# ghy1228/LDPC_Error_Floor

Hardware: AMD Instinct MI355X
Metric: decoded codewords/sec, wman N576 R3/4, 20 NMS iters (higher is better)
Workload: dtype i32

## Files before the change

include/ldpc_nms.h:

```cpp
#ifndef LDPC_NMS_H
#define LDPC_NMS_H

#include <stdint.h>

#ifdef __cplusplus
extern "C" {
#endif

#define LDPC_NMS_ABI_VERSION 3

typedef struct ldpc_graph ldpc_graph;
typedef struct ldpc_ctx ldpc_ctx;

enum ldpc_status {
    LDPC_OK = 0,
    LDPC_ERR_ARG = -1,
    LDPC_ERR_HIP = -2,
    LDPC_ERR_OOM = -3,
    LDPC_ERR_STATE = -4,
    LDPC_ERR_UNSUPPORTED = -5
};

enum ldpc_decoding_type {
    LDPC_DEC_SP = 0,
    LDPC_DEC_MS = 1,
    LDPC_DEC_QMS = 2,
    LDPC_DEC_MS_NONUDGE = 3
};

enum ldpc_kernel {
    LDPC_KERNEL_AUTO = 0,
    LDPC_KERNEL_FLOOD = 1,
    LDPC_KERNEL_FUSED = 2
};

typedef struct ldpc_decode_params {
    int32_t T;
    int32_t decoding_type;
    int32_t q_bit;
    int32_t target_bits;
    float clip_llr;
    int32_t kernel;
    int32_t outputs_size;
    int32_t reserved;
} ldpc_decode_params;

typedef struct ldpc_decode_outputs {
    float* app_all;
    uint32_t* hard_bits;
    uint32_t* synd_bits;
    int64_t* counters;
    uint8_t* frame_flags;
    uint32_t* iter_wrong;
} ldpc_decode_outputs;

int ldpc_abi_version(void);
const char* ldpc_status_string(int status);

int ldpc_graph_create(const int32_t* proto, int32_t M, int32_t N, int32_t z, int32_t device,
                      ldpc_graph** out);
int ldpc_graph_destroy(ldpc_graph* g);
int ldpc_graph_query(const ldpc_graph* g, int32_t* dims);

int ldpc_weights_set(ldpc_graph* g, int32_t T, const float* alpha, const float* alpha_ucn,
                     const float* beta);

int ldpc_ctx_create(ldpc_graph* g, int64_t B_max, int32_t T_max, ldpc_ctx** out);
int ldpc_ctx_destroy(ldpc_ctx* c);

int ldpc_decode(ldpc_ctx* c, const float* llr_dev, int64_t B, const ldpc_decode_params* p,
                const ldpc_decode_outputs* o, void* stream);

int ldpc_kernel_info(const ldpc_ctx* c, const ldpc_decode_params* p, int64_t* bytes_per_cw,
                     char* name, int32_t name_len);

int ldpc_ctx_last_kernel(const ldpc_ctx* c, char* name, int32_t name_len);

int ldpc_ctx_last_frozen(const ldpc_ctx* c);

int ldpc_ctx_last_afix(const ldpc_ctx* c);

int ldpc_channel_awgn(float* llr_dev, int64_t B, int32_t n_vars, double sigma, uint64_t seed,
                      int64_t offset, int32_t decoding_type, int32_t q_bit, int32_t punct_start,
                      int32_t punct_end, int32_t short_start, int32_t short_end, float clip_llr,
                      void* stream);

typedef struct ldpc_channel_params {
    double sigma;
    uint64_t seed;
    int64_t offset;
    int32_t punct_start, punct_end, short_start, short_end;
    int32_t reserved[4];
} ldpc_channel_params;

int ldpc_decode_awgn(ldpc_ctx* ctx, int64_t B, const ldpc_decode_params* params,
                     const ldpc_channel_params* channel, const ldpc_decode_outputs* outputs,
                     void* stream);

int ldpc_awgn_in_kernel(const ldpc_ctx* ctx, const ldpc_decode_params* params, int32_t has_short,
                        int32_t app);

typedef struct ldpc_es_outputs {
    int32_t size;
    int32_t reserved;
    int64_t* counters;
    uint8_t* frame_flags;
    uint8_t* n_iter;
    int64_t* iter_hist;
} ldpc_es_outputs;

int ldpc_decode_es(ldpc_ctx* ctx, const float* llr_dev, int64_t B, const ldpc_decode_params* params,
                   const ldpc_es_outputs* es_outputs, void* stream);
int ldpc_decode_awgn_es(ldpc_ctx* ctx, int64_t B, const ldpc_decode_params* params,
                        const ldpc_channel_params* channel, const ldpc_es_outputs* es_outputs,
                        void* stream);
int ldpc_es_supported(const ldpc_ctx* ctx, const ldpc_decode_params* params);

typedef struct ldpc_word_outputs {
    int32_t size;
    int32_t reserved;
    uint32_t* hard_last;
    uint8_t* word_flags;
    int64_t* counters;
    uint8_t* frame_flags;
} ldpc_word_outputs;

int ldpc_decode_word(ldpc_ctx* ctx, const float* llr_dev, int64_t B, const ldpc_decode_params* params,
                     const ldpc_word_outputs* word_outputs, void* stream);
int ldpc_word_supported(const ldpc_ctx* ctx, const ldpc_decode_params* params);

typedef struct ldpc_es_word_outputs {
    int32_t size;
    int32_t reserved;
    uint32_t* hard_stop;
    uint8_t* word_flags;
    int64_t* counters;
    uint8_t* frame_flags;
    uint8_t* n_iter;
    int64_t* iter_hist;
    uint64_t reserved1;
} ldpc_es_word_outputs;

int ldpc_decode_es_word(ldpc_ctx* ctx, const float* llr_dev, int64_t B, const ldpc_decode_params* params,
                        const ldpc_es_word_outputs* outputs, void* stream);
int ldpc_decode_awgn_es_word(ldpc_ctx* ctx, int64_t B, const ldpc_decode_params* params,
                             const ldpc_channel_params* channel, const ldpc_es_word_outputs* outputs,
                             void* stream);
int ldpc_es_word_supported(const ldpc_ctx* ctx, const ldpc_decode_params* params);

typedef struct ldpc_event_outputs {
    int32_t size;
    int32_t early_stop;
    int64_t frame_base;
    int64_t cap;
    int64_t* ev_count;
    int64_t* ev_frame;
    int32_t* ev_info;
    uint32_t* ev_word;
    int64_t* counters;
    uint8_t* frame_flags;
    uint8_t* n_iter;
    int64_t* iter_hist;
    uint64_t reserved1;
} ldpc_event_outputs;

int ldpc_decode_events(ldpc_ctx* ctx, const float* llr_dev, int64_t B, const ldpc_decode_params* params,
                       const ldpc_event_outputs* outputs, void* stream);
int ldpc_decode_awgn_events(ldpc_ctx* ctx, int64_t B, const ldpc_decode_params* params,
                            const ldpc_channel_params* channel, const ldpc_event_outputs* outputs,
                            void* stream);
int ldpc_events_supported(const ldpc_ctx* ctx, const ldpc_decode_params* params, int32_t early_stop);

int ldpc_decode_q8(ldpc_ctx* ctx, const int8_t* q8_dev, int64_t B, const ldpc_decode_params* params,
                   const ldpc_decode_outputs* outputs, void* stream);
int ldpc_decode_q8_word(ldpc_ctx* ctx, const int8_t* q8_dev, int64_t B, const ldpc_decode_params* params,
                        const ldpc_word_outputs* word_outputs, void* stream);
int ldpc_q8_supported(const ldpc_ctx* ctx, const ldpc_decode_params* params, int32_t has_short,
                      int32_t word);
int ldpc_channel_awgn_q8(int8_t* q8_dev, int64_t B, int32_t n_vars, double sigma, uint64_t seed,
                         int64_t offset, int32_t q_bit, int32_t punct_start, int32_t punct_end,
                         int32_t short_start, int32_t short_end, void* stream);
int ldpc_llr_to_q8(const float* llr_dev, int64_t n, int32_t q_bit, float clip_llr, int8_t* q8_dev,
                   int64_t* n_invalid_dev, void* stream);

int ldpc_channel_awgn_rows(float* rows_dev, const int64_t* idx_dev, int64_t n, int32_t n_vars,
                           double sigma, uint64_t seed, int64_t offset, int32_t decoding_type,
                           int32_t q_bit, int32_t punct_start, int32_t punct_end,
                           int32_t short_start, int32_t short_end, float clip_llr, void* stream);

int ldpc_collect_frames(const uint8_t* flags_dev, int64_t B, uint32_t mask, uint32_t want,
                        int64_t* idx_dev, int64_t cap, int64_t* count_dev, void* stream);

int ldpc_gather_rows(const float* src_dev, int64_t n_cols, const int64_t* idx_dev, int64_t n,
                     float* dst_dev, void* stream);

#define LDPC_UNCOR_ROW_BOUND(n_cols) (13 + 48 * (int64_t)(n_cols))
int ldpc_format_uncor_rows(const float* rows, int64_t n, int64_t n_cols, char* out, int64_t cap,
                           int64_t* len);

#ifdef __cplusplus
}
#endif
#endif
```

include/ldpc_nms_debug.h:

```cpp
#ifndef LDPC_NMS_DEBUG_H
#define LDPC_NMS_DEBUG_H

#include <stdint.h>

#include "ldpc_nms.h"

#ifdef __cplusplus
extern "C" {
#endif

int ldpc_debug_bs_bounds(const int32_t* proto, int32_t M, int32_t N, int32_t z, int32_t T,
                         int32_t mode, int32_t alpha_uniform, int32_t beta_uniform, float clip,
                         int32_t flags, int32_t* violations, char* msg, int32_t msg_len);

int ldpc_debug_bs_frozen(const int32_t* proto, int32_t M, int32_t N, int32_t z, int32_t T, int32_t mode,
                         int32_t alpha_uniform, int32_t beta_uniform, int32_t ucn, int32_t kind,
                         float clip, int32_t* plan, int32_t* frozen, int32_t n, char* names,
                         int32_t names_len);

int ldpc_debug_alpha_tid(float alpha, int32_t mode, int32_t* out_id, uint8_t* table);

int ldpc_debug_alpha_tids(const int32_t* proto, int32_t M, int32_t N, int32_t z, int32_t T,
                          const float* alpha, const float* alpha_ucn, int32_t* ids);

int ldpc_debug_events_out(ldpc_ctx* ctx, const uint32_t* planes_dev, const uint32_t* bad_dev, int64_t B,
                          int32_t target_bits, const uint8_t* n_iter_dev, int32_t T,
                          const ldpc_event_outputs* outputs, void* stream);

#ifdef __cplusplus
}
#endif

#endif
```

ldpc_error_floor_amd/csrc/ldpc_bs.hip:

```cpp
#include <algorithm>
#include <array>
#include <cmath>
#include <cstdio>
#include <cstdlib>
#include <cstring>
#include <functional>
#include <string>
#include <utility>
#include <vector>

#include "ldpc_bs_host.h"

namespace ldpc {
namespace bs {

__global__ void k_bs_tables(const float* __restrict__ alpha, const float* __restrict__ alpha_ucn,
                            const float* __restrict__ beta, const int32_t* __restrict__ row_ptr,
                            int T, int E, int N, int arows, int ar, int bcols, float step, float inv,
                            int qmax, float cu, uint32_t* alut, uint32_t* blut) {
    const int f = blockIdx.x * blockDim.x + threadIdx.x;
    const int na = T * ar, nbt = T * bcols;
    if (f >= na + nbt) return;
    int g[16];
    uint32_t* out;
// ... 71 lines not shown
        if (i > 0) first += (size_t)((((int64_t)lay[2 * (i - 1)] + h.z - (int64_t)cur) % 32 + 32) % 32);
        int A = ((deg + LPC - 1) / LPC) * h.z;
        while (!ok(A)) ++A;
        const int last_rows = (deg - (LPC - 1) + LPC - 1) / LPC;
        cur = first + (size_t)(LPC - 1) * A + (size_t)std::max(last_rows, 0) * h.z;
        lay[2 * i] = (int32_t)first;
        lay[2 * i + 1] = A;
    }
    *nslot = cur;
    return lay;
}
std::vector<int32_t> slot_layout(const host::GraphTables& h, int LPC, size_t* nslot) {
    return slot_layout_rows(h, std::vector<int>((size_t)h.M, LPC), nslot);
}

bool bs_mode(int mode) { return mode == MODE_Q5 || mode == MODE_QM5 || mode == MODE_Q4 || mode == MODE_Q3; }
float bs_step(int mode) { return mode == MODE_Q5 ? 0.5f : mode == MODE_Q3 ? 2.0f : 1.0f; }
int bs_qmax(int mode) { return mode == MODE_Q4 ? 7 : mode == MODE_Q3 ? 3 : QMAX; }
static float mode_step_bs(int mode) { return bs_step(mode); }

static BsPlan plan_inst(const DevGraph& g, int i, bool ucn, float clip, int min_cdeg, int mode, int T) {
    BsPlan p;
    const BsInst& k = kBsInst[i];
    const host::GraphTables& h = *g.host;
    if (h.max_cdeg > k.D || h.max_vdeg > k.DV || (ucn && !k.UCN)) return p;
    p.inst = i;
    p.ucn = ucn;
    const int nv = g.n_vars, nc = g.n_checks;
    p.cn_lanes = 64 * ((k.LPC * nc + 63) / 64);
    int vch = (nv + 63) / 64;
    const int cch = p.cn_lanes / 64;
    if (k.VPL == 1 && k.CPL == 1) {
        static const int eca = [] { const char* e = getenv("LDPC_BS_COLALIGN"); return e ? atoi(e) : 1; }();
        p.colalign = eca != 0 && colalign_fits(h, std::max(vch, cch));
        if (p.colalign) vch = (32 * h.N + 63) / 64;
    }
    if (k.VPL == 1 && k.CPL == 1) p.nw = std::max(vch, cch);
    else p.nw = std::max((vch + k.VPL - 1) / k.VPL, (cch + k.CPL - 1) / k.CPL);
    if (p.nw > 16) return p;
    if (k.VPL > 1 || k.CPL > 1) {
        p.nw = 16;
        if (vch > k.VPL * p.nw || cch > k.CPL * p.nw) return p;
    }
    const char* eap = getenv("LDPC_BS_AROWS");
    p.arows = ((g.w_alpha_uniform && !ucn) || (g.w_alpha_pair_uniform && !(eap && atoi(eap) == 0))) ? 1 : h.M;
    p.bcols = g.w_beta_uniform ? 1 : h.N;
    p.cn_dmin = (p.cn_lanes == k.LPC * nc) ? min_cdeg : 0;
    if (k.BIG) {
        const float cu = clip / mode_step_bs(mode);
        if (cu > (float)bs_qmax(mode)) p.cu = cu;
    }
    size_t nslot = 0;
    p.lay = slot_layout(h, k.LPC, &nslot);
    size_t o = 0;
    if (k.UCN) {
        p.off_hdz = (uint32_t)(4 * (size_t)nv);
        o = ((size_t)4 * (nv + 1) + 127) & ~(size_t)127;
    }
    p.off_slots = (uint32_t)o;
    p.off_pad = (uint32_t)(o + nslot * SLOT_B);
    p.off_zero = p.off_pad + SLOT_B;
    const size_t slot_end = (size_t)p.off_zero + SLOT_B;
    if (k.PK && slot_end > 65535) return p;
    if (k.UCN && p.off_hdz > 65535) return p;
    o = (slot_end + 15) & ~(size_t)15;
    p.off_red = (uint32_t)o;
    o += 64 + (((size_t)4 * T + 15) & ~(size_t)15) + 4 * FLORW;
    if (k.ES) {
        p.off_esu = (uint32_t)o;
        o += ((size_t)4 * T + 15) & ~(size_t)15;
    }
    p.off_alut = (uint32_t)o;
    o += (size_t)2 * (k.UCN ? 2 : 1) * p.arows * LUT_W * 4;
    p.off_blut = (uint32_t)o;
    o += (size_t)2 * p.bcols * BLUT_W * 4;
    const bool first_buffer = k.ES || i == kBsInstUcn1;
    if (k.PK && k.CPL == 1 && (first_buffer ? (size_t)p.off_alut + (size_t)p.arows * LUT_W * 4 : o) > 65535) return p;
    if (k.CPL == 1) {
        p.off_ch = (uint32_t)o;
        o += (size_t)4 * 64 * p.nw;
    }
    if (k.UCN && k.CPL == 1) {
        const int EPL = (k.D + k.LPC - 1) / k.LPC, HDW = (EPL + 1) / 2;
        p.off_hdl = (uint32_t)o;
        o += (size_t)4 * HDW * 64 * p.nw;
    }
    p.lds = (o + 15) & ~(size_t)15;
    if (p.lds > BS_LDS_MAX) return p;
    p.ok = true;
    return p;
}

BsPlan bs_plan(const DevGraph& g, int mode, bool ucn, bool per_edge_w, float clip, int T, bool es = false) {
    BsPlan p;
    const char* e = getenv("LDPC_BS");
    if (e && atoi(e) == 0) return p;
    const char* el = getenv("LDPC_BS_LPC");
    const int want_lpc = el ? atoi(el) : 0;
    const char* ei = getenv("LDPC_BS_INST");
    const int want_inst = ei ? atoi(ei) : -1;
    if (!bs_mode(mode)) return p;
    if (per_edge_w || !g.host || !g.w_beta_nonneg) return p;
    const host::GraphTables& h = *g.host;
    int min_cdeg = 1 << 30;
    for (int i = 0; i < h.M; ++i) min_cdeg = std::min(min_cdeg, h.row_ptr[i + 1] - h.row_ptr[i]);
    if (min_cdeg < 2) return p;
    for (int i = 0; i < kBsNInst; ++i) {
        if (kBsInst[i].ES != es) continue;
        if (es) {
            BsPlan q = plan_inst(g, i, ucn, clip, min_cdeg, mode, T);
            if (q.ok) return q;
            continue;
        }
        if (want_lpc != 0 && want_lpc != kBsInst[i].LPC) continue;
        if (want_inst >= 0 && want_inst != i) continue;
        if (i == kBsInstUcn1 && !ucn) continue;
        BsPlan q = plan_inst(g, i, ucn, clip, min_cdeg, mode, T);
        if (q.ok) return q;
    }
    return p;
}

typedef std::array<int32_t, kBsFrozenFields> BsGeoFields;
static const char* const bs_frozen_names[kBsFrozenFields] = {
    "inst", "n_vars", "n_checks", "z", "N", "cn_lanes", "cn_dmin", "NT", "nw", "arows", "bcols", "AL", "BL",
    "cstride", "off_slots", "off_pad", "off_zero", "off_red", "off_alut", "off_blut", "off_ch", "lds"};
static BsGeoFields bs_plan_fields(const DevGraph& g, const BsPlan& p) {
    const int ar = (p.inst >= 0 && kBsInst[p.inst].UCN ? 2 : 1) * p.arows;
    return {p.inst, g.n_vars, g.n_checks, g.z, g.N, p.cn_lanes, p.cn_dmin, 64 * p.nw, p.nw, p.arows, p.bcols,
            ar * LUT_W, p.bcols * BLUT_W, g.z * SLOT_B, (int32_t)p.off_slots, (int32_t)p.off_pad,
            (int32_t)p.off_zero, (int32_t)p.off_red, (int32_t)p.off_alut, (int32_t)p.off_blut,
            (int32_t)p.off_ch, (int32_t)p.lds};
}
static BsGeoFields bs_frozen_fields() {
    typedef BsFrozenWman W;
    return {W::inst, W::n_vars, W::n_checks, W::z, W::N, W::cn_lanes, W::cn_dmin, W::NT, W::nw, W::arows,
            W::bcols, W::AL, W::BL, (int32_t)W::cstride, (int32_t)W::off_slots, (int32_t)W::off_pad,
            (int32_t)W::off_zero, (int32_t)W::off_red, (int32_t)W::off_alut, (int32_t)W::off_blut,
            (int32_t)W::off_ch, (int32_t)W::lds};
}
static bool bs_frozen_fit(const DevGraph& g, BsPlan& p, const BsReq& r, bool exports) {
    const char* e = getenv("LDPC_BS_FROZEN");
    if (e && atoi(e) == 0) return false;
    if (!p.ok || p.inst != BsFrozenWman::inst || p.ucn || r.es || r.l8 || exports || r.T > BsFrozenWman::T_CAP) return false;
    BsPlan q = p;
    const uint32_t d = (uint32_t)(((4 * BsFrozenWman::T_CAP + 15) & ~15) - ((4 * r.T + 15) & ~15));
    q.off_alut += d;
    q.off_blut += d;
    q.off_ch += d;
    q.lds += d;
    if (bs_plan_fields(g, q) != bs_frozen_fields()) return false;
    p = q;
    return true;
}

#ifndef BS_DEAL_DEFAULT
#define BS_DEAL_DEFAULT 2
#endif
std::vector<int> deal_chunks(const std::vector<int>& cost, int nw, int cap) {
    const int n = (int)cost.size();
    std::vector<int> order(n), slot((size_t)nw * cap, -1);
    for (int c = 0; c < n; ++c) order[c] = c;
    std::stable_sort(order.begin(), order.end(), [&](int x, int y) { return cost[x] > cost[y]; });
    const char* e = getenv("LDPC_BS_DEAL");
    if (e && atoi(e) == 0) {
        std::vector<int> used(nw, 0), load(4, 0);
        for (int c : order) {
            int best = -1, bw = -1;
            for (int sm = 0; sm < 4; ++sm) {
                int w_s = -1;
                for (int w = sm; w < nw; w += 4)
                    if (used[w] < cap && (w_s < 0 || used[w] < used[w_s])) w_s = w;
                if (w_s >= 0 && (best < 0 || load[sm] < load[best])) { best = sm; bw = w_s; }
            }
            slot[(size_t)bw * cap + used[bw]] = c;
            ++used[bw];
            load[best] += cost[c];
        }
        return slot;
    }
    const int deal_mode = e ? atoi(e) : BS_DEAL_DEFAULT;
    if (deal_mode == 2 && cap == 1 && n <= nw && nw <= 16) {
        int slots[4] = {0, 0, 0, 0};
        for (int w = 0; w < nw; ++w) ++slots[w % 4];
        std::vector<int> cur(n, -1), best(n, -1);
        int load[4] = {0, 0, 0, 0}, used[4] = {0, 0, 0, 0};
        long long best_key = -1;
        std::function<void(int)> rec = [&](int i) {
            const int mx = std::max(std::max(load[0], load[1]), std::max(load[2], load[3]));
            if (best_key >= 0 && (long long)mx * 1000000 > best_key) return;
            if (i == n) {
                const long long key = (long long)mx * 1000000 + (long long)load[0] * load[0] + (long long)load[1] * load[1] +
                                      (long long)load[2] * load[2] + (long long)load[3] * load[3];
                if (best_key < 0 || key < best_key) { best_key = key; best = cur; }
                return;
            }
            for (int sm = 0; sm < 4; ++sm) {
                if (used[sm] >= slots[sm]) continue;
                bool dup = false;
                for (int q = 0; q < sm; ++q)
                    if (used[q] < slots[q] && load[q] == load[sm] && slots[q] - used[q] == slots[sm] - used[sm]) dup = true;
                if (dup) continue;
                load[sm] += cost[order[i]];
                ++used[sm];
                cur[i] = sm;
                rec(i + 1);
                load[sm] -= cost[order[i]];
                --used[sm];
            }
        };
        rec(0);
        int next[4] = {0, 1, 2, 3};
        for (int i = 0; i < n; ++i) {
            const int sm = best[i];
            slot[(size_t)next[sm]] = order[i];
            next[sm] += 4;
        }
        return slot;
    }
    std::vector<std::vector<int>> vch(nw);
    std::vector<int> vload(nw, 0);
    for (int c : order) {
        int best = -1;
        for (int w = 0; w < nw; ++w)
            if ((int)vch[w].size() < cap &&
                (best < 0 || vload[w] < vload[best] || (vload[w] == vload[best] && vch[w].size() < vch[best].size())))
                best = w;
        vch[best].push_back(c);
        vload[best] += cost[c];
    }
    std::vector<int> vorder(nw), sload(4, 0), next(4);
    for (int w = 0; w < nw; ++w) vorder[w] = w;
    std::stable_sort(vorder.begin(), vorder.end(), [&](int x, int y) { return vload[x] > vload[y]; });
    for (int sm = 0; sm < 4; ++sm) next[sm] = sm;
    for (int v : vorder) {
        int sm = -1;
        for (int q = 0; q < 4; ++q)
            if (next[q] < nw && (sm < 0 || sload[q] < sload[sm])) sm = q;
        const int w = next[sm];
        next[sm] += 4;
        sload[sm] += vload[v];
        for (size_t u = 0; u < vch[v].size(); ++u) slot[(size_t)w * cap + u] = vch[v][u];
    }
    return slot;
}

std::vector<int32_t> uniform_lanes(const host::GraphTables& h, int LPC, int cn_lanes) {
    std::vector<int32_t> lanes((size_t)cn_lanes, -1);
    const int nc = h.M * h.z;
    for (int ql = 0; ql < cn_lanes; ++ql)
        if (ql / LPC < nc) lanes[(size_t)ql] = (ql / LPC) | ((ql % LPC) << 16) | (LPC << 20);
    return lanes;
}

std::vector<int> check_chunk_cost_lanes(const host::GraphTables& h, const std::vector<int32_t>& lanes) {
    const int cch = (int)(lanes.size() / 64);
    std::vector<int> cost(cch, 2);
    for (int ch = 0; ch < cch; ++ch) {
        int pos = 0;
        for (int l = 0; l < 64; ++l) {
            const int32_t d = lanes[(size_t)64 * ch + l];
            if (d < 0) continue;
            const int i = (d & 0xFFFF) / h.z, L = (d >> 20) & 15;
            pos = std::max(pos, (h.row_ptr[i + 1] - h.row_ptr[i] + L - 1) / L);
        }
        cost[ch] += pos;
    }
    return cost;
}
std::vector<int> check_chunk_cost(const host::GraphTables& h, int LPC, int cch) {
    return check_chunk_cost_lanes(h, uniform_lanes(h, LPC, 64 * cch));
}

std::vector<int> column_rotation_lanes(const host::GraphTables& h, int EPL, const std::vector<int32_t>& lanes) {
    const int z = h.z, cn_lanes = (int)lanes.size();
    std::vector<int> toff(h.N, 0);
    {
        std::vector<std::vector<std::pair<int, int>>> grp;
        std::vector<std::vector<int>> bycol(h.N);
        for (int h0 = 0; h0 < cn_lanes; h0 += 32)
            for (int m = 0; m < EPL; ++m) {
                std::vector<std::pair<int, int>> gl;
                for (int ql = h0; ql < h0 + 32 && ql < cn_lanes; ++ql) {
                    const int32_t d = lanes[(size_t)ql];
                    if (d < 0) continue;
                    const int cc = d & 0xFFFF, cj = (d >> 16) & 15, LPC = (d >> 20) & 15;
                    const int i = cc / z, hc = cc - i * z, kk = LPC * m + cj;
                    if (kk >= h.row_ptr[i + 1] - h.row_ptr[i]) continue;
                    const int pe = h.row_ptr[i] + kk;
                    gl.emplace_back(h.pe_col[pe], (hc + h.pe_shift[pe]) % z);
                }
                if (gl.empty()) continue;
                for (const auto& x : gl)
                    if (bycol[x.first].empty() || bycol[x.first].back() != (int)grp.size())
                        bycol[x.first].push_back((int)grp.size());
                grp.push_back(std::move(gl));
            }
        auto gcost = [&](const std::vector<std::pair<int, int>>& gl) {
            int cnt[32] = {0}, mx = 0, sq = 0;
            uint32_t seen[32];
            int ns = 0;
            for (const auto& x : gl) {
                const uint32_t t = (uint32_t)(x.first * z + (x.second + toff[x.first]) % z);
                bool dup = false;
                for (int q = 0; q < ns && !dup; ++q) dup = seen[q] == t;
                if (dup) continue;
// ... 191 lines not shown
        for (size_t x = 0; x < cs.size(); ++x) cchunk[x] = cs[x];
    }
    std::vector<uint32_t> chd;
    if (k.UCN) {
        chd.assign((size_t)p.cn_lanes * HDW, 0u);
        for (int ql = 0; ql < p.cn_lanes; ++ql) {
            const int cc = ql / LPC, cj = ql % LPC;
            for (int m = 0; m < EPL; ++m) {
                uint32_t addr = p.off_hdz;
                const int kk = LPC * m + cj;
                if (cc < g.n_checks) {
                    const int i = cc / z, hc = cc - i * z;
                    if (kk < h.row_ptr[i + 1] - h.row_ptr[i]) {
                        const int pe = h.row_ptr[i] + kk;
                        const int v = h.pe_col[pe] * z + (hc + h.pe_shift[pe]) % z;
                        addr = 4 * hd_index(v);
                    }
                }
                chd[(size_t)ql * HDW + (m >> 1)] |= addr << (16 * (m & 1));
            }
        }
    }
    BsHostTables t;
    t.vn.swap(vn);
    t.wdeg.swap(wdeg);
    t.cchunk.swap(cchunk);
    t.chd.swap(chd);
    return t;
}
static int bs_graph_tables(const DevGraph& g, const BsPlan& p, void*& graph, int& inst, hipStream_t s) {
    if (graph && inst != p.inst) {
        (void)hipFree(graph);
        graph = nullptr;
    }
    if (graph) return LDPC_OK;
    BsHostTables t = bs_host_tables(g, p);
    const std::vector<uint32_t>& vn = t.vn;
    const std::vector<int32_t>& wdeg = t.wdeg;
    const std::vector<int32_t>& cchunk = t.cchunk;
    const std::vector<uint32_t>& chd = t.chd;
    const size_t nwords = vn.size() + wdeg.size() + p.lay.size() + cchunk.size() + chd.size();
    void* d = nullptr;
    if (hipMalloc(&d, nwords * 4) != hipSuccess) { (void)hipGetLastError(); return LDPC_ERR_OOM; }
    uint32_t* dp = reinterpret_cast<uint32_t*>(d);
    size_t at = 0;
    bool ok = true;
    auto up = [&](const void* src, size_t n) {
        if (n) ok = ok && hipMemcpyAsync(dp + at, src, n * 4, hipMemcpyHostToDevice, s) == hipSuccess;
        at += n;
    };
    up(vn.data(), vn.size());
    up(wdeg.data(), wdeg.size());
    up(p.lay.data(), p.lay.size());
    up(cchunk.data(), cchunk.size());
    up(chd.data(), chd.size());
    if (!ok || hipStreamSynchronize(s) != hipSuccess) {
        (void)hipFree(d);
        return LDPC_ERR_HIP;
    }
    graph = d;
    inst = p.inst;
    return LDPC_OK;
}

static BsPlan bs_route(const DevGraph& g, const BsReq& r, bool* to_bsc) {
    BsPlan p = bs_plan(g, r.mode, r.ucn, r.per_edge_w, r.clip, r.T, r.es);
    *to_bsc = !p.ok && (!r.es || !bs_plan(g, r.mode, r.ucn, r.per_edge_w, r.clip, r.T).ok);
    return p;
}

bool bs_supported(const DevGraph& g, const BsReq& r) {
    bool to_bsc;
    return bs_route(g, r, &to_bsc).ok || (to_bsc && bsc_supported(g, r));
}

bool bs_q8_ok(const DevGraph& g, const BsReq& r, bool has_short) {
    bool to_bsc;
    const BsPlan p = bs_route(g, r, &to_bsc);
    if (!p.ok) return to_bsc && bsc_q8_ok(g, r, has_short);
    return (!has_short || p.cu > 0.f) && q8_tab_fits(p);
}

bool bs_l8_ok(const DevGraph& g, const BsReq& r, bool has_short) {
    bool to_bsc;
    if (r.es) return false;
    const BsPlan p = bs_route(g, r, &to_bsc);
    if (!p.ok) return to_bsc && bsc_l8_ok(g, r, has_short);
    return bs_l8_inst(p.inst) && (!has_short || (kBsInst[p.inst].BIG && p.cu > 0.f));
}

const char* bs_kernel_name(const DevGraph& g, const BsReq& r) {
    static thread_local char buf[64];
    bool to_bsc;
    const BsPlan p = bs_route(g, r, &to_bsc);
    if (!p.ok) return to_bsc ? bsc_kernel_name(g, r) : "";
    const BsInst& k = kBsInst[p.inst];
    char x[16] = "";
    if (k.VPL > 1 || k.CPL > 1) snprintf(x, sizeof(x), ",x%d/%d", k.VPL, k.CPL);
    snprintf(buf, sizeof(buf), "bsl[p32,w%d,d%d,v%d,l%d%s%s%s]", p.nw, k.D, k.DV, k.LPC, x, p.ucn ? ",ucn" : "",
             r.es ? ",es" : "");
    return buf;
}

static int bs_run(const DevGraph& g, const Bufs& b, FusedWorkspace& ws, const BsPlan& p, const float* llr,
                  const BsReq& r, const BsOut& o, bool frozen, hipStream_t s) {
    ws.bs_frozen = frozen;
    void*& graph = r.es ? ws.bs_es_graph : ws.bs_graph;
    int st = bs_graph_tables(g, p, graph, r.es ? ws.bs_es_graph_inst : ws.bs_graph_inst, s);
    if (st != LDPC_OK) return st;
    const BsInst& k = kBsInst[p.inst];
    const float step = mode_step_bs(r.mode);
    const int ar = (k.UCN ? 2 : 1) * p.arows;
    uint32_t *alut = nullptr, *blut = nullptr;
    st = bs_make_tables(b, g, p.arows, ar, p.bcols, step, bs_qmax(r.mode), p.cu, r.ucn, ws, &alut, &blut, s);
    if (st != LDPC_OK) return st;
    const int DV = k.DV;
    const int VNW = (k.PK ? (DV + 1) / 2 : DV) + 1;
    const uint32_t* gt = reinterpret_cast<const uint32_t*>(graph);
    BsLaunch a{};
    a.n_iter = o.n_iter;
    a.iter_hist = o.iter_hist;
    a.hdw = o.hdw;
    a.word = o.word ? 1 : 0;
    a.frozen = frozen;
    a.llr = r.l8 ? reinterpret_cast<const float*>(r.l8) : llr;
    const int src = r.l8 ? BS_SRC_L8 : b.q8 ? BS_SRC_GEN : BS_SRC_LLR;
    a.gen = bs_gen(b, q8_tab_lds(p));
    a.B = b.B;
    a.n_vars = g.n_vars;
    a.n_checks = g.n_checks;
    a.T = b.T;
    a.target_bits = b.target_bits;
    a.cn_lanes = p.cn_lanes;
    a.cn_dmin = p.cn_dmin;
    a.fold_wave = p.cn_lanes < 64 * p.nw ? (uint32_t)(p.nw - 1) : (p.nw > 1 ? 1u : 0u);
    a.inv = 1.0f / step;
    a.cu = p.cu > 0.f ? p.cu : -1.f;
    a.qmax = bs_qmax(r.mode);
    a.ucn = p.ucn ? 1 : 0;
    a.ucn_iter = g.w_ucn_iter;
    a.beta_id = g.w_beta_id_mask;
    a.row_ptr = g.row_ptr;
    a.z = g.z;
    a.vn_tab = gt;
    const size_t nvt = (size_t)k.VPL * 64 * p.nw * VNW;
    a.vn_wdeg = reinterpret_cast<const int32_t*>(gt + nvt);
    a.row_lay = a.vn_wdeg + 3 * (size_t)k.VPL * p.nw;
    a.cn_chunk = a.row_lay + 2 * (size_t)g.M;
    a.cn_hd = reinterpret_cast<const uint32_t*>(a.cn_chunk + (size_t)p.nw * k.CPL);
    a.alut = alut;
    a.blut = blut;
    a.arows = p.arows;
    a.bcols = p.bcols;
    a.btid = (bs_qmax(r.mode) == QMAX && !getenv("LDPC_BS_NOBFIX")) ? g.beta_tid : nullptr;
    a.btid_n = g.N;
    a.atid = nullptr;
    if (bs_loops(k) && !p.ucn && p.arows == 1 && (r.mode == MODE_Q5 || r.mode == MODE_QM5)) {
        const char* e = getenv("LDPC_BS_AFIX");
        if (e ? atoi(e) != 0 : true) a.atid = g.host->w_alpha_tid_dev;
    }
    ws.bs_afix = a.atid != nullptr;
    a.counters = o.counters;
    a.flags = o.flags;
    a.bad = o.bad;
    a.iter_wrong = r.es ? nullptr : b.iter_wrong;
    a.hdx = o.hdx;
    bs_stagger(k.VPL > 1 || k.CPL > 1, &a.stagger, &a.stagger_n);
    a.off_slots = p.off_slots;
    a.off_pad = p.off_pad;
    a.off_zero = p.off_zero;
    a.off_red = p.off_red;
    a.off_alut = p.off_alut;
    a.off_blut = p.off_blut;
    a.off_hdz = p.off_hdz;
    a.off_hdl = p.off_hdl;
    a.off_ch = p.off_ch;
    if (const char* e = getenv("LDPC_DIAG_ABLATE")) a.ablate = atoi(e);
    const int npacks = (int)((b.B + PACK - 1) / PACK);
    int grid = -1;
    if (const char* e = getenv("LDPC_BS_GRID")) grid = std::max(atoi(e), 0);
    a.ticket = nullptr;
    if (bs_loops(k)) {
        const char* e = getenv("LDPC_BS_TICKETS");
        if (e ? atoi(e) != 0 : true) {
            if (!ws.bs_ticket && hipMalloc(reinterpret_cast<void**>(&ws.bs_ticket), sizeof(uint32_t)) != hipSuccess)
                return LDPC_ERR_OOM;
            a.ticket = ws.bs_ticket;
        }
    }
    static const auto kLaunch = launch_table(std::make_integer_sequence<int, kBsNInst>{});
    static const size_t lds_min = [] { const char* e = getenv("LDPC_BS_LDS_MIN"); return e ? (size_t)atol(e) : 0; }();
    const size_t lds = std::min(std::max(p.lds, lds_min), (size_t)BS_LDS_MAX);
    const uint64_t rkey = (uint64_t)p.inst << 48 | (uint64_t)p.nw << 32 | (uint64_t)lds;
    if (ws.bs_resident_key != rkey) {
        ws.bs_resident_key = rkey;
        std::fill(ws.bs_resident, ws.bs_resident + 7, 0);
    }
#ifdef BS_STAMP
    static unsigned long long* dst = nullptr;
    static size_t dst_words = 0;
    const size_t st_words = BS_WG_BASE + (size_t)BS_WG_REC * npacks;
    if (dst_words < st_words) {
        if (dst && (hipStreamSynchronize(s) != hipSuccess || hipFree(dst) != hipSuccess)) return LDPC_ERR_HIP;
        dst = nullptr;
        dst_words = 0;
        if (hipMalloc(reinterpret_cast<void**>(&dst), st_words * 8) != hipSuccess) return LDPC_ERR_OOM;
        dst_words = st_words;
    }
    if (hipMemsetAsync(dst, 0, st_words * 8, s) != hipSuccess) return LDPC_ERR_HIP;
    a.stamps = dst;
    st = kLaunch[p.inst](a, npacks, p.nw, lds, s, src, grid, ws.bs_resident);
    unsigned long long hst[256];
    if (st != LDPC_OK || hipMemcpyAsync(hst, dst, sizeof(hst), hipMemcpyDeviceToHost, s) != hipSuccess ||
        hipStreamSynchronize(s) != hipSuccess)
        return st != LDPC_OK ? st : LDPC_ERR_HIP;
    fprintf(stderr, "bs_stamp inst %d T %d q8 %d frozen %d: per pack, shader clocks [check, check-barrier, var, var-barrier | "
            "entry, channel, ch-barrier, tables, first-var, check-setup | epilogue]\n", p.inst, b.T, b.q8 != nullptr,
            (int)frozen);
    static const int order[] = {0, 1, 2, 3, 8, 9, 10, 11, 12, 4, 5};
    for (int w = 0; w < p.nw && w < 16; ++w) {
        const double n = (double)(hst[16 * w + 15] ? hst[16 * w + 15] : 1);
        fprintf(stderr, "  wave %2d:", w);
        for (const int i : order) fprintf(stderr, " %8.0f", hst[16 * w + i] / n);
        fprintf(stderr, "  | SIMD %5.3f %5.3f %5.3f %5.3f\n", (hst[16 * w + 13] & 0xFFFFFFFFull) / n,
                (hst[16 * w + 13] >> 32) / n, (hst[16 * w + 14] & 0xFFFFFFFFull) / n, (hst[16 * w + 14] >> 32) / n);
    }
    if (const char* path = getenv("LDPC_BS_WG_DUMP")) {
        std::vector<unsigned long long> rec((size_t)BS_WG_REC * npacks);
        if (hipMemcpy(rec.data(), dst + BS_WG_BASE, rec.size() * 8, hipMemcpyDeviceToHost) != hipSuccess)
            return LDPC_ERR_HIP;
        int nwg = 0;
        for (int w = 0; w < npacks; ++w) nwg += rec[(size_t)BS_WG_REC * w] != 0;
        const int tickets = a.ticket != nullptr && nwg < npacks;
        if (FILE* f = fopen(path, "a")) {
            fprintf(f, "bs_wg_launch inst %d T %d B %lld packs %d q8 %d frozen %d tickets %d\n"
                    "# bs_wg wg packs rt_entry rt_exit clk_entry clk_exit hw_id xcc_id   (rt: 100 MHz ticks, clk: shader clocks)\n",
                    p.inst, b.T, (long long)b.B, npacks, b.q8 != nullptr, (int)frozen, tickets);
            for (int w = 0; w < npacks; ++w) {
                const unsigned long long* r = rec.data() + (size_t)BS_WG_REC * w;
                if (!r[0]) continue;
                fprintf(f, "bs_wg %d %llu %llu %llu %llu %llu %08llx %llu\n", w, r[0], r[1], r[2], r[3], r[4],
                        r[5] & 0xFFFFFFFFull, r[5] >> 32);
            }
            fclose(f);
        }
    }
    return st;
#else
    return kLaunch[p.inst](a, npacks, p.nw, lds, s, src, grid, ws.bs_resident);
#endif
}

int bs_decode(const DevGraph& g, const Bufs& b, FusedWorkspace& ws, const float* llr, const BsReq& r,
              const BsOut& o, hipStream_t s) {
    bool to_bsc;
    BsPlan p = bs_route(g, r, &to_bsc);
    ws.bs_frozen = false;
    ws.bs_afix = false;
    if (!p.ok) return to_bsc ? bsc_decode(g, b, ws, llr, r, o, s) : LDPC_ERR_UNSUPPORTED;
    const bool frozen = bs_frozen_fit(g, p, r, o.hdx != nullptr || o.hdw != nullptr);
    return bs_run(g, b, ws, p, llr, r, o, frozen, s);
}

}

namespace ldpc {
namespace bs {
struct BoundsReport {
    int violations = 0;
    std::string first;
    void fail(const char* what, long long idx, long long lim) {
        if (violations++ == 0) {
            char buf[160];
            snprintf(buf, sizeof(buf), "%s: index %lld outside [0, %lld)", what, idx, lim);
            first = buf;
        }
    }
    void in(const char* what, long long idx, long long lim) {
        if (idx < 0 || idx >= lim) fail(what, idx, lim);
    }
    void lds(const char* what, long long a, long long n, long long lo, long long hi) {
        if (a < lo || a + n > hi) fail(what, a, hi);
    }
    void apart(const char* what, long long a, long long n, long long b, long long m) {
        if (a < b + m && b < a + n) fail(what, a + n, b);
    }
};

static int bs_bounds_check(const DevGraph& g, const BsPlan& p, const BsHostTables& t, int T, int flags,
                           BoundsReport& r) {
    const BsInst& k = kBsInst[p.inst];
    const host::GraphTables& h = *g.host;
    const int LPC = k.LPC, VPL = k.VPL, CPL = k.CPL, DV = k.DV;
    const int EPL = (k.D + LPC - 1) / LPC, HDW = (EPL + 1) / 2, OB = 4 / LPC;
    const int VNA = k.PK ? (DV + 1) / 2 : DV, VNW = VNA + 1;
    const int NT = 64 * p.nw, nwv = p.nw, nv = g.n_vars, z = h.z;
    const bool UCN = k.UCN, ucn = UCN && (p.ucn || k.ES);
    const int AR = UCN ? 2 * p.arows : p.arows;
    const long long AL = (long long)AR * LUT_W, BL = (long long)p.bcols * BLUT_W;
    const long long lds = (long long)p.lds;
    const bool SKIPM = CPL > 1;
    const bool GBL = CPL == 1;
    const bool HDL = UCN && CPL == 1;
    if (getenv("LDPC_BOUNDS_VERBOSE"))
        fprintf(stderr, "bs plan: inst %d nw %d ucn %d lds %lld (slots %u..%u, alut %u, blut %u, ch %u, hdl %u)\n",
                p.inst, p.nw, (int)p.ucn, lds, p.off_slots, p.off_pad, p.off_alut, p.off_blut, p.off_ch, p.off_hdl);
    r.in("lds size", lds, (long long)BS_LDS_MAX + 1);
    if ((long long)t.vn.size() != (long long)VPL * NT * VNW) r.fail("vn_tab size", (long long)t.vn.size(), (long long)VPL * NT * VNW);
    r.lds("RED", p.off_red, 4LL * (16 + ((T + 3) & ~3) + FLORW), 0, k.ES ? p.off_esu : p.off_alut);
    if (k.ES) {
        r.lds("syndrome words", p.off_esu, 4LL * T, p.off_red, p.off_alut);
        r.apart("syndrome words / RED", p.off_esu, 4LL * T, p.off_red, 4LL * (16 + ((T + 3) & ~3) + FLORW));
        if (p.off_esu != p.off_red + 4u * (uint32_t)(16 + ((T + 3) & ~3) + FLORW)) r.fail("syndrome words' offset", p.off_esu, p.off_red);
        if (p.off_alut & 15) r.fail("alpha tables off 16 B", p.off_alut & 15, 1);
    }
    r.lds("ALUT", p.off_alut, 4 * 2 * AL, 0, p.off_blut);
    r.lds("BLUT", p.off_blut, 4 * 2 * BL, 0, lds);
    r.lds("PAD+ZERO", p.off_pad, 2 * SLOT_B, p.off_slots, p.off_red);
    if (UCN) r.lds("HD", 0, 4LL * (nv + 1), 0, p.off_slots);
    if (q8_tab_fits(p)) {
        const long long tb = q8_tab_lds(p);
        const long long tn = (flags & LDPC_BOUNDS_BIG_TABLES) ? (long long)(p.off_pad - p.off_slots) + 4
                                                              : 4LL * AWGN_TAB_W;
        r.lds("channel tables", tb, tn, p.off_slots, p.off_pad);
        if (UCN) r.apart("channel tables / HD", tb, tn, 0, 4LL * (nv + 1));
        r.apart("channel tables / PAD+ZERO", tb, tn, p.off_pad, 2 * SLOT_B);
        r.apart("channel tables / RED", tb, tn, p.off_red, (long long)p.off_alut - p.off_red);
        r.apart("channel tables / ALUT", tb, tn, p.off_alut, 4 * 2 * AL);
        r.apart("channel tables / BLUT", tb, tn, p.off_blut, 4 * 2 * BL);
    }
    for (int u = 0; u < VPL; ++u)
        for (int w = 0; w < nwv; ++w) {
            const long long wi = 3LL * (u * nwv + w);
            r.in("vn_wdeg", wi + 2, (long long)t.wdeg.size());
            if (wi + 2 >= (long long)t.wdeg.size()) continue;
            const int dw = t.wdeg[(size_t)wi], pcol = t.wdeg[(size_t)wi + 2];
            if (pcol >= 0) r.in("btid column", pcol, h.N);
            if (dw >= 0 && T > 1) {
                const long long col = p.bcols == 1 ? 0 : pcol;
                if (col >= 0) r.in("btid", (long long)(T - 1) * h.N + col, (long long)T * h.N);
            }
            for (int l = 0; l < 64; ++l) {
                const long long ti = ((long long)u * NT + 64LL * w + l) * VNW;
                r.in("vn_tab", ti + VNA, (long long)t.vn.size());
                if (ti + VNA >= (long long)t.vn.size()) continue;
                const uint32_t* q = &t.vn[(size_t)ti];
                const int vv = (int)q[VNA];
                const int v = (UCN && vv >= 0) ? (vv & 0xFFFF) : vv;
                if (v >= nv) r.fail("variable", v, nv);
                if (vv >= 0 && UCN) r.in("HD index", (long long)((uint32_t)vv >> 16), nv);
                if (vv >= 0 && p.bcols > 1) r.in("beta table", v / (nv / p.bcols), p.bcols);
                for (int f = 0; f < DV && f < dw; ++f) {
                    const uint32_t a = k.PK ? ((f & 1) ? (q[f >> 1] >> 16) : (q[f >> 1] & 0xFFFFu)) : q[f];
                    if (a != p.off_zero) r.lds("variable slot", a, SLOT_B, p.off_slots, p.off_pad);
                }
            }
        }
    for (int w = 0; w < nwv; ++w)
        for (int c = 0; c < CPL; ++c) {
            r.in("cn_chunk", (long long)w * CPL + c, (long long)t.cchunk.size());
            const int gchunk = CPL == 1 ? w : t.cchunk[(size_t)w * CPL + c];
            const bool active = CPL == 1 ? w * 64 < p.cn_lanes : gchunk >= 0;
            int gm = EPL;
            if (SKIPM) {
                uint32_t any = 0u;
                for (int l = 0; l < 64; ++l) {
                    const int ql = std::max(gchunk, 0) * 64 + l, cc = ql / LPC;
                    const int ci = std::min(cc / z, g.n_checks / z - 1);
                    const int gdeg = cc < g.n_checks ? h.row_ptr[ci + 1] - h.row_ptr[ci] : 0;
                    any |= (1u << ((gdeg + LPC - 1) / LPC)) - 1u;
                }
                gm = __builtin_popcount(any);
                if (active) r.in("real positions - 1 (the min2 switch)", gm - 1, EPL);
            }
            for (int l = 0; l < 64; ++l) {
                const int ql = std::max(gchunk, 0) * 64 + l, cc = ql / LPC, cj = l % LPC;
                const int ci = std::min(cc / z, g.n_checks / z - 1);
                r.in("row_ptr", ci + 1, h.M + 1);
                r.in("row_lay", 2LL * ci + 1, (long long)p.lay.size());
                const int gdeg = cc < g.n_checks ? h.row_ptr[ci + 1] - h.row_ptr[ci] : 0;
                if (UCN) {
                    const bool guard = (flags & LDPC_BOUNDS_PRE_GUARD) ? true : ql < p.cn_lanes;
                    if (ucn && gchunk >= 0 && guard)
                        for (int pp = 0; pp < HDW; ++pp) r.in("cn_hd", (long long)ql * HDW + pp, (long long)t.chd.size());
                }
                if (GBL) r.lds("per-lane words", p.off_ch + 4LL * (64 * w + l), 4, p.off_ch, lds);
                if (HDL)
                    for (int pp = 0; pp < HDW; ++pp) r.lds("HD addresses", p.off_hdl + 4LL * (pp * NT + 64 * w + l), 4, p.off_hdl, lds);
                if (!active) continue;
                const long long gbase = p.off_slots +
                    ((long long)p.lay[2 * ci] + (long long)cj * p.lay[2 * ci + 1] + (cc - ci * z)) * SLOT_B;
                for (int m = 0; m < EPL; ++m) {
                    if (SKIPM && m >= gm) continue;
                    const bool re = LPC * m + LPC - 1 < p.cn_dmin || LPC * m + cj < gdeg;
                    const long long a = re ? gbase + (long long)m * z * SLOT_B : p.off_pad;
                    r.lds("check slot", a, SLOT_B, p.off_slots, p.off_red);
                    if (re && a + SLOT_B > p.off_pad) r.fail("check slot past the slot region", a, p.off_pad);
                    if (ucn && cc < g.n_checks && ql < p.cn_lanes && (size_t)ql * HDW + (m >> 1) < t.chd.size()) {
                        const uint32_t hw = t.chd[(size_t)ql * HDW + (m >> 1)];
                        const uint32_t ha = (m & 1) ? (hw >> 16) : (hw & 0xFFFFu);
                        r.lds("HD read", ha, 4, 0, (long long)p.off_hdz + 4);
                    }
                }
                const long long ctab = p.off_alut + (long long)(p.arows > 1 ? ci : 0) * LUT_W * 4 + (long long)cj * OB * 64;
                const long long last = ctab + 4LL * AL + (UCN ? (long long)p.arows * LUT_W * 4 : 0) + (OB - 1) * 64 + 3 * 16;
                r.lds("alpha table", ctab, 16, p.off_alut, p.off_alut + 4 * 2 * AL);
                if (k.PK && CPL == 1) r.in("packed alpha-table address", ctab, 65536);
                r.lds("alpha table (odd t, alpha')", last, 16, p.off_alut, p.off_alut + 4 * 2 * AL);
            }
        }
    return r.violations;
}
}
}

extern "C" int ldpc_debug_bs_frozen(const int32_t* proto, int32_t M, int32_t N, int32_t z, int32_t T,
                                    int32_t mode, int32_t alpha_uniform, int32_t beta_uniform, int32_t ucn,
                                    int32_t kind, float clip, int32_t* plan, int32_t* frozen, int32_t n,
                                    char* names, int32_t names_len) {
    using namespace ldpc;
    using namespace ldpc::bs;
    if (!proto || T <= 0 || kind < 0 || kind > 2 || n < 0) return LDPC_ERR_ARG;
    host::GraphTables h;
    const int st = host::build_graph(proto, M, N, z, h);
    if (st != LDPC_OK) return st;
    DevGraph g{};
    g.M = h.M; g.N = h.N; g.z = h.z; g.E = h.E;
    g.n_checks = h.M * h.z; g.n_vars = h.N * h.z; g.n_edges = h.E * h.z; g.max_cdeg = h.max_cdeg;
    g.h_row_ptr = h.row_ptr.data();
    g.host = &h;
    g.w_alpha_uniform = alpha_uniform;
    g.w_alpha_pair_uniform = alpha_uniform;
    g.w_beta_uniform = beta_uniform;
    g.w_beta_nonneg = 1;
    const BsReq r{mode, ucn != 0, false, clip, T, kind == 1};
    bool to_bsc;
    BsPlan p = bs_route(g, r, &to_bsc);
    const bool fz = bs_frozen_fit(g, p, r, kind == 2);
    const BsGeoFields pf = bs_plan_fields(g, p), ff = bs_frozen_fields();
    for (int i = 0; i < n && i < kBsFrozenFields; ++i) {
        if (plan) plan[i] = p.ok ? pf[(size_t)i] : -1;
        if (frozen) frozen[i] = ff[(size_t)i];
    }
    if (names && names_len > 0) {
        std::string all;
        for (int i = 0; i < kBsFrozenFields; ++i) all += std::string(i ? "," : "") + bs_frozen_names[i];
        std::strncpy(names, all.c_str(), (size_t)names_len - 1);
        names[names_len - 1] = 0;
    }
    return fz ? 1 : 0;
}

extern "C" int ldpc_debug_bs_bounds(const int32_t* proto, int32_t M, int32_t N, int32_t z, int32_t T,
                                    int32_t mode, int32_t alpha_uniform, int32_t beta_uniform,
                                    float clip, int32_t flags, int32_t* violations, char* msg,
                                    int32_t msg_len) {
    using namespace ldpc;
    using namespace ldpc::bs;
    if (!proto || !violations || T <= 0) return LDPC_ERR_ARG;
    host::GraphTables h;
    const int st = host::build_graph(proto, M, N, z, h);
    if (st != LDPC_OK) return st;
    DevGraph g{};
    g.M = h.M; g.N = h.N; g.z = h.z; g.E = h.E;
    g.n_checks = h.M * h.z; g.n_vars = h.N * h.z; g.n_edges = h.E * h.z; g.max_cdeg = h.max_cdeg;
    g.h_row_ptr = h.row_ptr.data();
    g.host = &h;
    g.w_alpha_uniform = alpha_uniform;
    g.w_alpha_pair_uniform = alpha_uniform;
    g.w_beta_uniform = beta_uniform;
    g.w_beta_nonneg = 1;
    int min_cdeg = 1 << 30;
    for (int i = 0; i < h.M; ++i) min_cdeg = std::min(min_cdeg, h.row_ptr[i + 1] - h.row_ptr[i]);
    int checked = 0;
    *violations = 0;
    std::string first;
    for (int i = 0; i < kBsNInst; ++i)
        for (int u = 0; u < 2; ++u) {
            if (kBsInst[i].ES && !(flags & LDPC_BOUNDS_ES)) continue;
            if (i == kBsInstUcn1 && (!(flags & LDPC_BOUNDS_UCN1) || u == 0)) continue;
            const BsPlan p = plan_inst(g, i, u != 0, clip, min_cdeg, mode, T);
            if (!p.ok) continue;
            const BsHostTables t = bs_host_tables(g, p);
            BoundsReport r;
            bs_bounds_check(g, p, t, T, flags, r);
            ++checked;
            if (r.violations && first.empty()) {
                char buf[64];
                snprintf(buf, sizeof(buf), "instance %d%s: ", i, u ? " ucn" : "");
                first = std::string(buf) + r.first;
            }
            *violations += r.violations;
        }
    for (int b1 = 0; b1 < 2; ++b1) {
        if (b1 && !beta_uniform) continue;
        g.w_beta_one = b1;
        BoundsReport r;
        const int n = bsc_debug_bounds(g, mode, clip, T, flags, r.violations, r.first);
        if (n <= 0) continue;
        ++checked;
        if (r.violations && first.empty()) first = std::string(b1 ? "bsc beta=1: " : "bsc: ") + r.first;
        *violations += r.violations;
    }
    g.w_beta_one = 1;
    if ((flags & LDPC_BOUNDS_ES_BSC) && beta_uniform && !bs_plan(g, mode, false, false, clip, T).ok) {
        BoundsReport r;
        if (bsc_debug_bounds(g, mode, clip, T, flags, r.violations, r.first, true) > 0) {
            ++checked;
            if (r.violations && first.empty()) first = std::string("bsc early stop: ") + r.first;
            *violations += r.violations;
        }
    }
    if (msg && msg_len > 0) {
        std::strncpy(msg, first.c_str(), (size_t)msg_len - 1);
        msg[msg_len - 1] = 0;
    }
    return checked;
}
```

ldpc_error_floor_amd/csrc/ldpc_bs_kernel.h:

```cpp
#pragma once
#include <type_traits>
#include <cstdint>

#include "ldpc_beta_tabs.h"
#include "ldpc_fused.h"
#include "ldpc_fused5_kernel.h"
#include "ldpc_bitplane.h"
#include "ldpc_bs_frozen.h"

namespace ldpc {
namespace bs {

constexpr int PACK = 32;
constexpr int SLOT_W = 5;
constexpr int SLOT_B = SLOT_W * 4;
constexpr int LUT_W = 64;
constexpr int BLUT_W = LUT_W + 4;
constexpr int QMAX = 15;
constexpr size_t BS_LDS_MAX = 160 * 1024;

struct BsInst { int D, DV, LPC, VPL, CPL; bool UCN, BIG, PK; int WPE; bool ES = false; };
constexpr BsInst kBsInst[] = {
    {15, 6, 4, 1, 1, false, false, true, 8},
    {16, 8, 4, 1, 1, false, false, true, 8},
// ... 280 lines not shown
    a = grp_and<LPC>(a);
    m2[3] = a;
#pragma unroll
    for (int m = 0; m < K; ++m) c2[m] = B3(T_NANDEQ, cand[m], X[m][3], a);
#pragma unroll
    for (int i = 2; i >= 0; --i) {
        a = X[0][i] | ~c2[0];
#pragma unroll
        for (int m = 1; m < K; ++m) a = B3(T_ANDORN, a, X[m][i], c2[m]);
        a = grp_and<LPC>(a);
        m2[i] = a;
        if (i > 0) {
#pragma unroll
            for (int m = 0; m < K; ++m) c2[m] = B3(T_ANDEQ, c2[m], X[m][i], a);
        }
    }
#pragma unroll
    for (int i = 0; i < 4; ++i) m2[i] = mux(two, m1[i], m2[i]);
}

#ifdef BS_DIAG
#define ABL(bit) (a.ablate & (bit))
#else
#define ABL(bit) 0
#endif
#ifdef BS_MARK
#define PH(name, k) asm volatile(";@ph " name ".%0" ::"i"(k))
#define PH4(name, k, x) asm volatile(";@ph " name ".%4" : "+v"(x[0]), "+v"(x[1]), "+v"(x[2]), "+v"(x[3]) : "i"(k))
#define PH8(name, k, x, y)                                                                        \
    asm volatile(";@ph " name ".%8" : "+v"(x[0]), "+v"(x[1]), "+v"(x[2]), "+v"(x[3]), "+v"(y[0]),  \
                 "+v"(y[1]), "+v"(y[2]), "+v"(y[3]) : "i"(k))
#define PH9(name, k, x, y, z)                                                                     \
    asm volatile(";@ph " name ".%9" : "+v"(x[0]), "+v"(x[1]), "+v"(x[2]), "+v"(x[3]), "+v"(y[0]),  \
                 "+v"(y[1]), "+v"(y[2]), "+v"(y[3]), "+v"(z) : "i"(k))
#else
#define PH(name, k) ((void)0)
#define PH4(name, k, x) ((void)0)
#define PH8(name, k, x, y) ((void)0)
#define PH9(name, k, x, y, z) ((void)0)
#endif
__device__ __forceinline__ void t8x8(uint32_t& lo, uint32_t& hi) {
    uint32_t t;
    t = B3((TA ^ TB) & TC, lo, lo >> 7, 0x00AA00AAu);
    lo = B3(T_XOR3, lo, t, t << 7);
    t = B3((TA ^ TB) & TC, hi, hi >> 7, 0x00AA00AAu);
    hi = B3(T_XOR3, hi, t, t << 7);
    t = B3((TA ^ TB) & TC, lo, lo >> 14, 0x0000CCCCu);
    lo = B3(T_XOR3, lo, t, t << 14);
    t = B3((TA ^ TB) & TC, hi, hi >> 14, 0x0000CCCCu);
    hi = B3(T_XOR3, hi, t, t << 14);
    t = B3((TA ^ TB) & TC, lo, hi << 4, 0xF0F0F0F0u);
    lo ^= t;
    hi ^= t >> 4;
}
template <bool BIG>
__device__ __forceinline__ void pack_bytes(const uint32_t (&D)[8], uint32_t valid, uint32_t& cs,
                                           uint32_t (&cm)[4], uint32_t& bg) {
    uint32_t lo[4], hi[4];
#pragma unroll
    for (int g = 0; g < 4; ++g) {
        lo[g] = D[2 * g];
        hi[g] = D[2 * g + 1];
        t8x8(lo[g], hi[g]);
    }
    const uint32_t a = __builtin_amdgcn_perm(lo[1], lo[0], 0x06020400u), b = __builtin_amdgcn_perm(lo[1], lo[0], 0x07030501u);
    const uint32_t c = __builtin_amdgcn_perm(lo[3], lo[2], 0x06020400u), d = __builtin_amdgcn_perm(lo[3], lo[2], 0x07030501u);
    const uint32_t L0 = __builtin_amdgcn_perm(c, a, 0x05040100u) & valid, L2 = __builtin_amdgcn_perm(c, a, 0x07060302u) & valid;
    const uint32_t L1 = __builtin_amdgcn_perm(d, b, 0x05040100u) & valid, L3 = __builtin_amdgcn_perm(d, b, 0x07060302u) & valid;
    const uint32_t e = __builtin_amdgcn_perm(hi[1], hi[0], 0x05010400u), f = __builtin_amdgcn_perm(hi[3], hi[2], 0x05010400u);
    const uint32_t n = ~__builtin_amdgcn_perm(f, e, 0x05040100u) & valid;
    bg = BIG ? (__builtin_amdgcn_perm(f, e, 0x07060302u) & valid) : 0u;
    cs = n;
    cm[0] = L0;
    cm[1] = B3(T_XAND, L1, n, L0);
    cm[2] = B3(T_XAND, L2, n, L0 | L1);
    cm[3] = B3(T_XAND, L3, n, L0 | L1 | L2);
}
template <bool BIG>
__device__ __forceinline__ int pack_channel(const float (&xv)[PACK], float inv, int qmax, float cu,
                                            uint32_t valid, uint32_t& cs, uint32_t (&cm)[4], uint32_t& bg) {
    const float qf = (float)qmax;
    uint32_t D[8];
    int off = 0;
#pragma unroll
    for (int k = 0; k < 8; ++k) D[k] = 0u;
#pragma unroll
    for (int r = 0; r < PACK; ++r) {
        const float x = xv[r] * inv;
        const float q = __builtin_amdgcn_fmed3f(rintf(x), -qf, qf);
        const bool big = BIG && fabsf(x) == cu;
        off |= (q != x && !big) ? 1 : 0;
        D[r >> 2] = __builtin_amdgcn_cvt_pk_u8_f32(q + (big ? 48.f : 16.f), r & 3, D[r >> 2]);
    }
    pack_bytes<BIG>(D, valid, cs, cm, bg);
    return off;
}
typedef unsigned int v2u_g __attribute__((ext_vector_type(2)));
typedef __attribute__((address_space(3))) const v2u_g LdsU2;
__device__ __forceinline__ void gen_bytes(const BsGen& g, int64_t pk, int v, int qmax, uint32_t (&D)[8]) {
    const int bit = v + 1;
    if (g.ss > 0 && bit >= g.ss && bit <= g.se) {
#pragma unroll
        for (int i = 0; i < 8; ++i) D[i] = (uint32_t)(48 - qmax) * 0x01010101u;
        return;
    }
    if (g.ps > 0 && bit >= g.ps && bit <= g.pe) {
#pragma unroll
        for (int i = 0; i < 8; ++i) D[i] = 0x10101010u;
        return;
    }
    LdsU2* bucket = reinterpret_cast<LdsU2*>((uintptr_t)g.lds);
    const LdsW* thi = reinterpret_cast<const LdsW*>((uintptr_t)(g.lds + 8u * (1u << AWGN_KB)));
    const LdsW* tlo = thi + AWGN_NB_MAX;
    const uint64_t g0 = (uint64_t)g.offset + (uint64_t)pk * 32u;
    const int sh = (int)(g.offset & 3);
    const uint32_t boff = (uint32_t)(16 + g.kmin);
    auto word = [&](const int (&l)[4]) __attribute__((always_inline)) -> uint32_t {
        return ((uint32_t)l[0] + boff) | ((uint32_t)l[1] + boff) << 8 | ((uint32_t)l[2] + boff) << 16 |
               ((uint32_t)l[3] + boff) << 24;
    };
#pragma unroll
    for (int i = 0; i < 8; ++i) {
        const uint64_t gq = (g0 + 4u * (uint32_t)i) >> 2;
        int la[4];
        awgn_levels4b(g, bucket, thi, tlo, (uint32_t)v, gq, la);
        uint32_t w = word(la);
        if (sh) {
            int lb[4];
            awgn_levels4b(g, bucket, thi, tlo, (uint32_t)v, gq + 1, lb);
            w = __builtin_amdgcn_alignbyte(word(lb), w, (uint32_t)sh);
        }
        D[i] = w;
    }
}
__device__ __forceinline__ void gen_tables(const BsGen& g, int tid, int NT) {
    copy_async(g.lds, g.tab, AWGN_TAB_W, __builtin_amdgcn_readfirstlane(tid >> 6), NT);
}

constexpr double STAGGER_US = 60.0;
constexpr int FLORW = 32;
constexpr bool bs_loops(const BsInst& k) { return k.VPL == 1 && k.CPL == 1 && !k.UCN; }
#if defined(BS_INST) && BS_INST <= 2
#define BS_LOOP_TU 1
#else
#define BS_LOOP_TU 0
#endif
template <class K>
struct BsArgsAf : K {
    const int32_t* atid;
};
template <class K>
using BsKernArgs = std::conditional_t<BS_LOOP_TU != 0, BsArgsAf<K>, K>;
constexpr int BS_RED_NEXT = 8;
#define BS_PACK_SETUP(pk)                                                                          \
    const int64_t b0 = (int64_t)(pk) * PACK;                                                       \
    const int nvalid = (int)min<int64_t>(PACK, a.B - b0);                                          \
    const uint32_t valid = (nvalid >= 32) ? 0xFFFFFFFFu : ((1u << nvalid) - 1u);                   \
    uint32_t* RED = reinterpret_cast<uint32_t*>(smem + (FZ ? W::off_red : a.off_red));             \
    const int flor = 16 + ((a.T + 3) & ~3);                                                        \
    const int AR = UCN ? 2 * (FZ ? W::arows : a.arows) : (FZ ? W::arows : a.arows);                \
    const int AL = AR * LUT_W, BL = (FZ ? W::bcols : a.bcols) * BLUT_W;                            \
    uint32_t* ALUT = reinterpret_cast<uint32_t*>(smem + (FZ ? W::off_alut : a.off_alut));          \
    uint32_t* BLUT = reinterpret_cast<uint32_t*>(smem + (FZ ? W::off_blut : a.off_blut));          \
    const bool ucn = UCN && a.ucn;                                                                 \
    auto ucn_on = [&](int t) __attribute__((always_inline)) -> bool {                              \
        return ucn && (t >= 64 || ((a.ucn_iter >> t) & 1));                                        \
    };

template <int D, int DV, int LPC, int VPL, int CPL, bool UCN, bool BIG, bool PK, int WPE, bool XP, int LB, bool Q8,
          bool ES = false, bool EW = false, bool FZ = false, bool L8 = false>
__global__ void __launch_bounds__(LB) __attribute__((amdgpu_waves_per_eu(WPE)))
k_bs(BsKernArgs<std::conditional_t<ES, std::conditional_t<EW, BsArgsEw, BsArgsEs>, std::conditional_t<XP, BsArgsXp, BsArgs>>> a) {
    static_assert(LPC == 2 || LPC == 4, "lanes per check");
    using KArgs = std::conditional_t<ES, std::conditional_t<EW, BsArgsEw, BsArgsEs>, std::conditional_t<XP, BsArgsXp, BsArgs>>;
    static_assert(!ES || (UCN && VPL == 1 && CPL == 1 && !XP), "early stop: one-chunk UCN-compiled instances");
    static_assert(!EW || ES, "the stop-iteration word: early-stop builds");
    static_assert(!L8 || (!Q8 && !ES && !FZ), "int8 LLRs: the decode and export builds");
    static_assert(!FZ || (BS_LOOP_TU && !UCN && !XP && !ES && VPL == 1 && CPL == 1 && D == 15 && DV == 6 && LPC == 4),
                  "frozen geometry: the wman pack-loop builds");
    using W = BsFrozenWman;
    static_assert(W::cstride == W::z * SLOT_B && W::AL == W::arows * LUT_W && W::BL == W::bcols * BLUT_W &&
                  W::NT == 64 * W::nw && W::off_zero == W::off_pad + SLOT_B, "BsFrozenWman is consistent");
    constexpr int SB = (DV * QMAX + QMAX <= 127) ? 8 : 9;
    constexpr int EPL = (D + LPC - 1) / LPC;
    constexpr bool SKIPM = CPL > 1;
    constexpr int OB = 4 / LPC;
    constexpr int VNA = PK ? (DV + 1) / 2 : DV;
    constexpr int VNW = VNA + 1;
    constexpr int HDW = (EPL + 1) / 2;
    constexpr bool PKG = PK && CPL == 1;
    constexpr bool ONE = VPL == 1 && CPL == 1;
    constexpr int PRIO = ONE ? (DV >= 6 ? 4 : 2) : 0;
    constexpr int PROPRIO = PRIO == 4 ? 3 : 0;
    constexpr bool T0A = ONE;
    constexpr bool EBR = T0A;
    constexpr int SBSET = ONE ? 3 : 2;
    constexpr int KEEP0 = ONE ? 3 : (UCN ? 4 : 7);
    constexpr int KEEP = DV <= 4 ? DV : (KEEP0 < DV ? KEEP0 : DV - 1);
    constexpr bool BKPF = !XP && VPL > 1;
    constexpr bool AFX = BS_LOOP_TU != 0;
    static_assert(!AFX || (ONE && !UCN), "fixed-set check tables: the one-chunk instances without UCN");
    extern __shared__ __attribute__((aligned(16))) unsigned char smem[];
    if ((uint32_t)(uintptr_t)smem != 0u) __builtin_trap();
#ifdef BS_STAMP
    uint64_t sacc[13] = {};
    uint64_t sts = __builtin_amdgcn_s_memtime();
    if (a.stamps && threadIdx.x == 0) {
        unsigned long long* rec = a.stamps + BS_WG_BASE + (size_t)BS_WG_REC * blockIdx.x;
        rec[1] = __builtin_amdgcn_s_memrealtime();
        rec[3] = sts;
    }
#define BS_ST(i)                                                                                   \
    do {                                                                                           \
        const uint64_t tn_ = __builtin_amdgcn_s_memtime();                                         \
        sacc[i] += tn_ - sts;                                                                      \
        sts = tn_;                                                                                 \
    } while (0)
#else
#define BS_ST(i) ((void)0)
#endif
    const int tid = threadIdx.x;
    const int NT = FZ ? W::NT : (int)blockDim.x;
    const int lane = tid & 63;
    const int wave = __builtin_amdgcn_readfirstlane(tid >> 6);
    const int nwv = NT >> 6;
    const int nv = (FZ ? W::n_vars : a.n_vars);
#if !BS_LOOP_TU
    BS_PACK_SETUP(blockIdx.x)
#endif

    if (PROPRIO > 0) __builtin_amdgcn_s_setprio(PROPRIO);
    uint32_t va[VPL][VNA];
    int vv[VPL], dw[VPL], dwmin[VPL], pcol[VPL];
    uint32_t tab_b[VPL];
#pragma unroll
    for (int u = 0; u < VPL; ++u) {
        const uint32_t* vt = a.vn_tab + ((size_t)u * NT + tid) * VNW;
#pragma unroll
        for (int p = 0; p < VNA; ++p) va[u][p] = vt[p];
        vv[u] = (int)vt[VNA];
        dw[u] = __builtin_amdgcn_readfirstlane(a.vn_wdeg[3 * (u * nwv + wave)]);
        dwmin[u] = __builtin_amdgcn_readfirstlane(a.vn_wdeg[3 * (u * nwv + wave) + 1]);
        pcol[u] = __builtin_amdgcn_readfirstlane(a.vn_wdeg[3 * (u * nwv + wave) + 2]);
        tab_b[u] = ((FZ ? W::bcols : a.bcols) > 1 && vv[u] >= 0) ? (uint32_t)(((UCN ? (vv[u] & 0xFFFF) : vv[u]) / (nv / (FZ ? W::bcols : a.bcols))) * BLUT_W * 4) : 0u;
    }
    constexpr int FOLDB = BS_LOOP_TU ? 0x100 : 0;
    int cn_dmin = (FZ ? W::cn_dmin : a.cn_dmin) | ((FOLDB && (uint32_t)wave == a.fold_wave) ? FOLDB : 0);

    if (a.stagger > 0 && (int)blockIdx.x < a.stagger_n) {
        const int n = (int)(((uint32_t)blockIdx.x * 97u % (uint32_t)a.stagger_n) * (uint32_t)a.stagger /
                            (uint32_t)a.stagger_n);
        for (int i = 0; i < n; ++i) __builtin_amdgcn_s_sleep(8);
    }
#if BS_LOOP_TU
    auto lane_now = [&]() __attribute__((always_inline)) -> int {
        uint32_t all = ~0u;
        asm volatile("" : "+s"(all));
        return (int)__builtin_amdgcn_mbcnt_hi(all, __builtin_amdgcn_mbcnt_lo(all, 0u));
    };
    unsigned pack = blockIdx.x;
#ifdef BS_STAMP
    unsigned long long npk = 0ull;
#endif
    do {
    if (pack != blockIdx.x) {
        __syncthreads();
        if (PROPRIO > 0) __builtin_amdgcn_s_setprio(PROPRIO);
    }
    typedef __attribute__((address_space(4))) const BsArgs PackArgs;
    PackArgs* kap = (PackArgs*)__builtin_amdgcn_kernarg_segment_ptr();
    asm volatile("" : "+s"(kap));
    PackArgs& a = *kap;
    const int tid = wave * 64 + lane_now(), lane = tid & 63;
    BS_PACK_SETUP(pack)
    [[maybe_unused]] const int pack_tbits = FZ ? a.target_bits : 0;
#define BS_TBITS (FZ ? pack_tbits : a.target_bits)
#define BS_PK pack
#define BS_NEXT_PACK continue
#define BS_LANE_IS0 (lane_now() == 0)
#else
#define BS_TBITS a.target_bits
#define BS_PK blockIdx.x
#define BS_NEXT_PACK return
#define BS_LANE_IS0 (lane == 0)
#endif
    if (tid < SLOT_W) {
        reinterpret_cast<uint32_t*>(smem + (FZ ? W::off_pad : a.off_pad))[tid] = 0xFFFFFFFFu;
        reinterpret_cast<uint32_t*>(smem + (FZ ? W::off_zero : a.off_zero))[tid] = 0u;
    }
    if (UCN && tid == 0) lds_put(a.off_hdz, 0u);
    if (tid < 8) RED[tid] = (tid == 1) ? 0xFFFFFFFFu : 0u;
#ifdef BS_STAMP
    if (tid == 0) {
        uint32_t hw0;
        asm volatile("s_getreg_b32 %0, hwreg(HW_REG_HW_ID)" : "=s"(hw0));
        RED[12] = (hw0 >> 4) & 3u;
    }
#endif
    if (tid < FLORW) RED[flor + tid] = 0u;
    [[maybe_unused]] uint32_t es_done = ~valid;
    if constexpr (ES) {
        for (int w = tid; w < a.T; w += NT) RED[flor + FLORW + w] = 0u;
    }
    [[maybe_unused]] uint32_t es_hd = 0u;
#if BS_LOOP_TU
    BsGen gen{};
    if constexpr (Q8) {
        gen.tab = a.gen.tab;
        gen.k0 = a.gen.k0;
        gen.k1 = a.gen.k1;
        gen.offset = a.gen.offset;
        gen.nb = a.gen.nb;
        gen.kmin = a.gen.kmin;
        gen.ps = a.gen.ps;
        gen.pe = a.gen.pe;
        gen.ss = a.gen.ss;
        gen.se = a.gen.se;
        gen.lds = a.gen.lds;
    }
#define BS_GEN gen
#else
#define BS_GEN a.gen
#endif
#if BS_LOOP_TU
    unsigned next_pack = pack + gridDim.x;
    auto take_ticket = [&]() __attribute__((always_inline)) {
        typedef __attribute__((address_space(1))) uint32_t GlobalW;
        GlobalW* tk = (GlobalW*)(uintptr_t)a.cn_hd;
        if (tid == 0 && tk)
            next_pack = gridDim.x + __hip_atomic_fetch_add(tk, 1u, __ATOMIC_RELAXED, __HIP_MEMORY_SCOPE_AGENT);
    };
    if constexpr (Q8) take_ticket();
#endif
    if constexpr (Q8) gen_tables(BS_GEN, tid, NT);
    if (Q8 || !EBR) __syncthreads();
#if BS_LOOP_TU
    if constexpr (Q8) {
        if (tid == 0) RED[BS_RED_NEXT] = next_pack;
    }
#endif
    BS_ST(8);
    uint32_t cs[VPL], cm[VPL][4], bg[VPL];
    int off = 0;
    if (T0A) {
        copy_async((FZ ? W::off_alut : a.off_alut), a.alut, AL, wave, NT);
        copy_async((FZ ? W::off_blut : a.off_blut), a.blut, BL, wave, NT);
    }
    const __amdgpu_buffer_rsrc_t llr_rs = __builtin_amdgcn_make_buffer_rsrc(
        (void*)(a.llr + b0 * nv), 0, nvalid * nv * 4, 0x00020000);
    auto llr_at = [&](int r, int v) __attribute__((always_inline)) -> float {
        return __builtin_bit_cast(float, __builtin_amdgcn_raw_buffer_load_b32(llr_rs, 4 * v, 4 * r * nv, 0));
    };
    auto var_of = [&](int u) __attribute__((always_inline)) -> int {
        return (UCN && vv[u] >= 0) ? (vv[u] & 0xFFFF) : vv[u];
    };
    float xv[VPL][PACK];
#if BS_LOOP_TU
#pragma unroll
    for (int r = 0; r < PACK; ++r) xv[0][r] = 0.f;
#endif
    if constexpr (Q8) {
#pragma unroll
        for (int u = 0; u < VPL; ++u) {
            cs[u] = 0u;
            bg[u] = 0u;
#pragma unroll
            for (int p = 0; p < 4; ++p) cm[u][p] = 0u;
            const int v = var_of(u);
            if (v >= 0 && !ABL(32)) {
                uint32_t Dq[8];
                gen_bytes(BS_GEN, BS_PK, v, a.qmax, Dq);
                pack_bytes<BIG>(Dq, valid, cs[u], cm[u], bg[u]);
            }
        }
    } else if constexpr (L8) {
#if BS_LOOP_TU
        take_ticket();
#endif
        const __amdgpu_buffer_rsrc_t l8_rs = __builtin_amdgcn_make_buffer_rsrc(
            (void*)(reinterpret_cast<const uint8_t*>(a.llr) + b0 * nv), 0, nvalid * nv, 0x00020000);
        auto l8_load = [&](uint32_t (&Dw)[8], int v) __attribute__((always_inline)) {
            uint32_t by[PACK];
#pragma unroll
            for (int r = 0; r < PACK; ++r)
                by[r] = (uint32_t)__builtin_amdgcn_raw_buffer_load_b8(l8_rs, v, min(r, nvalid - 1) * nv, 0);
#pragma unroll
            for (int i = 0; i < 8; ++i)
                Dw[i] = by[4 * i] | by[4 * i + 1] << 8 | by[4 * i + 2] << 16 | by[4 * i + 3] << 24;
        };
        uint32_t Dw[VPL][8];
#pragma unroll
        for (int i = 0; i < 8; ++i) Dw[0][i] = 0u;
        if (var_of(0) >= 0 && !ABL(32)) l8_load(Dw[0], var_of(0));
        if (EBR) {
            asm volatile("" ::: "memory");
            __builtin_amdgcn_s_waitcnt(0xC07F);
            __builtin_amdgcn_s_barrier();
            asm volatile("" ::: "memory");
        }
        const bool l8_big = BIG && a.cu > 0.f;
        uint32_t l8_bad = 0u;
#pragma unroll
        for (int u = 0; u < VPL; ++u) {
            cs[u] = 0u;
            bg[u] = 0u;
#pragma unroll
            for (int p = 0; p < 4; ++p) cm[u][p] = 0u;
            const int v = var_of(u);
            const int u1 = u + 1 < VPL ? u + 1 : u;
            const int vn = (u + 1 < VPL && !ABL(32)) ? var_of(u1) : -1;
            if (v >= 0 && !ABL(32)) {
                uint32_t Dk[8];
#pragma unroll
                for (int i = 0; i < 8; ++i) {
                    uint32_t iv;
                    Dk[i] = l8_bytes(Dw[u][i], a.qmax, l8_big, iv);
                    l8_bad |= l8_invalid(iv, valid >> (4 * i));
                }
                pack_bytes<BIG>(Dk, valid, cs[u], cm[u], bg[u]);
            }
            if (vn >= 0) l8_load(Dw[u1], vn);
        }
        off = l8_bad != 0u;
#if BS_LOOP_TU
        if (tid == 0) RED[BS_RED_NEXT] = next_pack;
#endif
    } else {
#if BS_LOOP_TU
    take_ticket();
#endif
    if (var_of(0) >= 0 && !ABL(32)) {
#pragma unroll
        for (int r = 0; r < PACK; ++r) xv[0][r] = llr_at(r, var_of(0));
    }
    if (EBR) {
        asm volatile("" ::: "memory");
        __builtin_amdgcn_s_waitcnt(0xC07F);
        __builtin_amdgcn_s_barrier();
        asm volatile("" ::: "memory");
    }
#pragma unroll
    for (int u = 0; u < VPL; ++u) {
        cs[u] = 0u;
        bg[u] = 0u;
#pragma unroll
        for (int p = 0; p < 4; ++p) cm[u][p] = 0u;
        const int v = var_of(u);
        const int u1 = u + 1 < VPL ? u + 1 : u;
        const int vn = (u + 1 < VPL && !ABL(32)) ? var_of(u1) : -1;
        if (v >= 0 && !ABL(32))
            off |= pack_channel<BIG>(xv[u], a.inv, a.qmax, a.cu, valid, cs[u], cm[u], bg[u]);
        if (vn >= 0) {
#pragma unroll
            for (int r = 0; r < PACK; ++r) xv[u1][r] = llr_at(r, vn);
        }
    }
#if BS_LOOP_TU
    if (tid == 0) RED[BS_RED_NEXT] = next_pack;
#endif
    }
    if (off) atomicOr(&RED[7], 1u);
    BS_ST(9);
    __syncthreads();
    BS_ST(10);
    if (RED[7]) {
        if constexpr (ES) {
            if (tid < nvalid) {
                if (a.flags) a.flags[b0 + tid] = 0x80;
                if (kern_args<KArgs>().n_iter) kern_args<KArgs>().n_iter[b0 + tid] = 0;
            }
        }
        if constexpr (L8) {
            if (tid < nvalid && a.flags) a.flags[b0 + tid] = 0x80;
        }
        if (tid == 0) a.bad[BS_PK] = 1u;
        BS_NEXT_PACK;
    }
    if (tid == 0) a.bad[BS_PK] = 0u;
    if (!T0A) {
        for (int w = tid; w < AL; w += NT) ALUT[w] = a.alut[w];
        for (int w = tid; w < BL; w += NT) BLUT[w] = a.blut[w];
        __syncthreads();
    }
    BS_ST(11);

    int bkp[VPL];
#pragma unroll
    for (int u = 0; u < VPL; ++u) bkp[u] = -1;
    auto beta_lw = [&](const int u, const uint32_t bslice, const int tb, const uint32_t (&cmu)[4],
                       uint32_t (&lw)[4], const bool use_bk) __attribute__((always_inline)) {
        int bk = -1;
        if constexpr (!XP) {
            if (use_bk && a.btid) {
                const int col = ((FZ ? W::bcols : a.bcols) == 1) ? 0 : pcol[u];
                if (BKPF) bk = __builtin_amdgcn_readfirstlane(bkp[u]);
                else if (col >= 0)
                    bk = __builtin_amdgcn_readfirstlane((int)((const ConstW*)a.btid)[(size_t)tb * (FZ ? W::btid_n : a.btid_n) + col]);
            }
        }
        if (ABL(2) || (tb < 64 && ((a.beta_id >> tb) & 1))) {
            PH("vn_beta_id", u);
#pragma unroll
            for (int i = 0; i < 4; ++i) lw[i] = cmu[i];
        } else if (bk >= 0 && bk < kNBetaTab) {
            PH("vn_beta_fix", u);
            beta_asm(lw, cmu, bk);
            if constexpr (BIG) {
                if ((FZ ? W::bcols : a.bcols) == 1) {
                    const ConstW* tg = (const ConstW*)(a.blut) + (size_t)tb * BLUT_W;
#pragma unroll
                    for (int i = 0; i < 4; ++i) lw[i] = mux(bg[u], tg[LUT_W + i], lw[i]);
                } else {
                    const v4u gb = lds_q(bslice + tab_b[u] + LUT_W * 4);
                    lw[0] = mux(bg[u], gb.x, lw[0]);
                    lw[1] = mux(bg[u], gb.y, lw[1]);
                    lw[2] = mux(bg[u], gb.z, lw[2]);
                    lw[3] = mux(bg[u], gb.w, lw[3]);
                }
            }
        } else if ((FZ ? W::bcols : a.bcols) == 1) {
            PH("vn_beta_sg", u);
            const ConstW* tg = (const ConstW*)(a.blut) + (size_t)tb * BLUT_W;
            lut_s(lw, cmu, tg);
            if constexpr (BIG) {
#pragma unroll
                for (int i = 0; i < 4; ++i) lw[i] = mux(bg[u], tg[LUT_W + i], lw[i]);
            }
        } else {
            PH("vn_beta_lds", u);
            const uint32_t btab = bslice + tab_b[u];
            const uint32_t cmi[1][4] = {{cmu[0], cmu[1], cmu[2], cmu[3]}};
            uint32_t lo[1][4];
            lut<1>(lo, cmi, btab);
#pragma unroll
            for (int i = 0; i < 4; ++i) lw[i] = lo[0][i];
            if constexpr (BIG) {
                const v4u gb = lds_q(btab + LUT_W * 4);
                lw[0] = mux(bg[u], gb.x, lw[0]);
                lw[1] = mux(bg[u], gb.y, lw[1]);
                lw[2] = mux(bg[u], gb.z, lw[2]);
                lw[3] = mux(bg[u], gb.w, lw[3]);
            }
        }
    };
    auto vn_phase = [&](const bool first, const bool last, const uint32_t bslice, const int tb)
                        __attribute__((always_inline)) {
        (void)tid;
        uint32_t wr = 0u, apos = 0u, nb = 0u;
#pragma unroll
        for (int u = 0; u < VPL; ++u) {
            if (VPL > 1 && dw[u] < 0) continue;
            PH("vn_setup", (last ? 100 : 0) + u);
#pragma unroll
            for (int p = 0; p < VNA; ++p) asm volatile("" : "+v"(va[u][p]));
            auto vaddr = [&](int f) __attribute__((always_inline)) -> uint32_t {
                if constexpr (PK) return (f & 1) ? (va[u][f >> 1] >> 16) : (va[u][f >> 1] & 0xFFFFu);
                else return va[u][f];
            };
            const int v = (UCN && vv[u] >= 0) ? (vv[u] & 0xFFFF) : vv[u];
            const uint32_t hda = UCN ? 4u * ((uint32_t)vv[u] >> 16) : 0u;
            const uint32_t cmu[4] = {cm[u][0], cm[u][1], cm[u][2], cm[u][3]};
            const bool counted = v >= 0 && v < BS_TBITS;
            uint32_t lw[1][4];
            PH("vn_beta", (last ? 100 : 0) + u);
            if (!last) beta_lw(u, bslice, tb, cmu, lw[0], !first);
            const int dwu = dw[u];
            auto vbody = [&](auto sbc) __attribute__((always_inline)) {
                constexpr int SB = decltype(sbc)::value;
                uint32_t mn[KEEP > 0 ? KEEP : 1], mb[KEEP > 0 ? KEEP : 1][4];
                uint32_t S[SB];
#pragma unroll
                for (int i = 0; i < SB; ++i) S[i] = 0u;
                if (!first) {
#pragma unroll
                    for (int f = 0; f < DV; ++f) {
                        if (f < dwu) {
                            PH("vn_sum", 1000 * (SB - 6) + (last ? 100 : 0) + 10 * u + f);
                            uint32_t M[4], n, b[4];
                            read_slot(n, M, vaddr(f));
#pragma unroll
                            for (int i = 0; i < 4; ++i) b[i] = M[i] ^ n;
                            if (f == 0) set_b<SB>(S, b, n);
                            else add_b<SB>(S, b, n);
                            if (f < KEEP) {
                                mn[f < KEEP ? f : 0] = n;
#pragma unroll
                                for (int i = 0; i < 4; ++i) mb[f < KEEP ? f : 0][i] = b[i];
                            }
                        }
                    }
                    if constexpr (SB == 8) PH8("vn_app", 1000 * (SB - 6) + (last ? 100 : 0) + u, S, (S + 4));
                    else PH("vn_app", 1000 * (SB - 6) + (last ? 100 : 0) + u);
                    uint32_t hd, nz = 0u;
                    const uint32_t c_s = cs[u];
                    if (last) {
                        uint32_t A[SB];
#pragma unroll
                        for (int i = 0; i < SB; ++i) A[i] = S[i];
                        const uint32_t cb[4] = {cmu[0] ^ c_s, cmu[1] ^ c_s, cmu[2] ^ c_s, cmu[3] ^ c_s};
                        add_b<SB>(A, cb, c_s);
                        hd = ~A[SB - 1];
#pragma unroll
                        for (int i = 0; i < SB; ++i) nz |= A[i];
                    } else {
                        uint32_t c = c_s;
#pragma unroll
                        for (int i = 0; i < SB - 1; ++i) c = B3(T_MAJ, S[i], i < 4 ? (cmu[i] ^ c_s) : c_s, c);
                        hd = B3(T_XNOR3, S[SB - 1], c_s, c);
                    }
                    if (UCN && !last && v >= 0 && (ES || ucn_on(tb))) lds_put(hda, hd);
                    hd &= valid;
                    if constexpr (XP) {
                        const bool word = kern_args<KArgs>().word != 0;
                        const size_t row = word ? (size_t)BS_PK : (size_t)(tb - 1) * (size_t)((a.B + 31) >> 5) + BS_PK;
                        if (v >= 0 && (last || !word)) a.hdx[row * nv + v] = hd;
                    }
                    if (ABL(8)) hd = 0u;
                    if (counted) {
                        wr |= hd;
                        if (last) {
                            apos |= hd & nz;
                            if constexpr (ES) nb += (uint32_t)__popc(hd & ~es_done);
                            else
                            nb += (uint32_t)__popc(hd);
                        }
                    }
                    if constexpr (EW) {
                        if (last) es_hd |= hd & ~es_done;
                    }
                }
                if (last) return;
                if constexpr (SB == 8) PH8("vn_tv", 1000 * (SB - 6) + (last ? 100 : 0) + u, S, (S + 4));
                else PH("vn_tv", 1000 * (SB - 6) + (last ? 100 : 0) + u);
                uint32_t lb[4];
#pragma unroll
                for (int i = 0; i < 4; ++i) lb[i] = lw[0][i] ^ cs[u];
                add_b<SB>(S, lb, cs[u]);
                uint32_t Tv[6];
                clamp6<SB>(Tv, S);
                const int dwm = dwmin[u];
                if (first) {
                    if (UCN && v >= 0 && ucn_on(0)) lds_put(hda, ~Tv[5]);
                    uint32_t x[7], X[4];
#pragma unroll
                    for (int i = 0; i < 7; ++i) x[i] = Tv[i < 6 ? i : 5];
                    abs_sat(X, x);
#pragma unroll
                    for (int f = 0; f < DV; ++f)
                        if (f < dwu && (f < dwm || vaddr(f) != (FZ ? W::off_zero : a.off_zero))) write_slot(vaddr(f), x[6], X);
                } else {
#pragma unroll
                    for (int f = 0; f < DV; ++f) {
                        if (f < dwu) {
                            if (ABL(4)) continue;
                            PH("vn_vc", 1000 * (SB - 6) + (last ? 100 : 0) + 10 * u + f);
                            uint32_t x[7], X[4], n, b[4];
                            if (f < KEEP) {
                                n = mn[f < KEEP ? f : 0];
#pragma unroll
                                for (int i = 0; i < 4; ++i) b[i] = mb[f < KEEP ? f : 0][i];
                            } else {
                                uint32_t M[4];
                                read_slot(n, M, vaddr(f));
#pragma unroll
                                for (int i = 0; i < 4; ++i) b[i] = M[i] ^ n;
                            }
                            sub_tv(x, Tv, b, n);
                            abs_sat(X, x);
                            if (f < dwm || vaddr(f) != (FZ ? W::off_zero : a.off_zero)) write_slot(vaddr(f), x[6], X);
                        }
                    }
                }
            };
            if constexpr (SB >= 8) {
                if ((SBSET & 1) && dwu * QMAX + QMAX <= 63) vbody(std::integral_constant<int, 7>{});
                else if ((SBSET & 2) && SB == 9 && dwu * QMAX + QMAX <= 127) vbody(std::integral_constant<int, (SB == 9 ? 8 : SB)>{});
                else vbody(std::integral_constant<int, SB>{});
            } else {
                vbody(std::integral_constant<int, SB>{});
            }
        }
        if (!first && !last) {
            PH("vn_flags", 0);
            if (!ABL(8)) {
                const uint32_t la = __builtin_amdgcn_mbcnt_hi(~0u, __builtin_amdgcn_mbcnt_lo(~0u, 0u)) & 31u;
                __hip_atomic_fetch_or(RED + flor + la, wr, __ATOMIC_RELAXED, __HIP_MEMORY_SCOPE_WORKGROUP);
            }
        } else if (!first) {
            PH("vn_flags", last ? 100 : 0);
            if (!ABL(8)) wr = wave_or(wr);
            if (last) {
                apos = wave_or(apos);
                nb = wave_add(nb);
            }
            if (BS_LANE_IS0) {
                if (wr) atomicOr(&RED[0], wr);
                if (last) {
                    if (apos) atomicOr(&RED[2], apos);
                    if (nb) atomicAdd(&RED[3], nb);
                }
            }
        }
    };

    vn_phase(true, false, (FZ ? W::off_blut : a.off_blut), 0);
    BS_ST(12);
    const int cj = lane % LPC;
    int gchunk[CPL], gdeg[CPL], gm[CPL];
    uint32_t gbase[CPL], gtab[CPL], ghd[CPL][UCN ? HDW : 1];
#pragma unroll
    for (int c = 0; c < CPL; ++c) {
        gchunk[c] = (CPL == 1) ? wave : __builtin_amdgcn_readfirstlane(a.cn_chunk[wave * CPL + c]);
        const int ql = max(gchunk[c], 0) * 64 + lane;
        const int cc = ql / LPC;
        const int ci = min(cc / (FZ ? W::z : a.z), (FZ ? W::n_checks : a.n_checks) / (FZ ? W::z : a.z) - 1);
        gdeg[c] = (cc < (FZ ? W::n_checks : a.n_checks)) ? a.row_ptr[ci + 1] - a.row_ptr[ci] : 0;
        gm[c] = SKIPM ? (int)__popc(wave_or((1u << ((gdeg[c] + LPC - 1) / LPC)) - 1u)) : EPL;
        gbase[c] = (FZ ? W::off_slots : a.off_slots) + (uint32_t)((a.row_lay[2 * ci] + cj * a.row_lay[2 * ci + 1] + (cc - ci * (FZ ? W::z : a.z))) * SLOT_B);
        gtab[c] = (FZ ? W::off_alut : a.off_alut) + (uint32_t)(((FZ ? W::arows : a.arows) > 1 ? ci : 0) * LUT_W * 4) + (uint32_t)(cj * OB * 64);
        if constexpr (PKG) gbase[c] |= gtab[c] << 16;
        if constexpr (UCN) {
#pragma unroll
            for (int p = 0; p < HDW; ++p) ghd[c][p] = ((ES || ucn) && gchunk[c] >= 0 && ql < (FZ ? W::cn_lanes : a.cn_lanes)) ? a.cn_hd[(size_t)ql * HDW + p] : 0u;
        }
    }
    constexpr bool RPW = CPL > 1;
    constexpr int RB = EPL;
    static_assert(CPL * RB <= 32, "real-position word");
    static_assert(!SKIPM || EPL <= 8, "BS_MIN2_CASE covers 1..8");
    uint32_t rpk = 0u;
#pragma unroll
    for (int c = 0; c < CPL; ++c)
#pragma unroll
        for (int m = 0; m < EPL; ++m)
            if (RPW && (LPC * m + LPC - 1 < cn_dmin || LPC * m + cj < gdeg[c])) rpk |= 1u << (RB * c + m);
    const uint32_t cstride = (uint32_t)((FZ ? W::z : a.z) * SLOT_B);
    const uint32_t tabu = (uint32_t)((FZ ? W::arows : a.arows) * LUT_W * 4);
    constexpr bool GBL = CPL == 1;
    if constexpr (GBL) lds_put((FZ ? W::off_ch : a.off_ch) + 4u * (uint32_t)tid, gbase[0]);
    constexpr bool HDL = UCN && CPL == 1;
    if constexpr (HDL) {
#pragma unroll
        for (int p = 0; p < HDW; ++p) lds_put(a.off_hdl + 4u * (uint32_t)(p * NT + tid), ghd[0][p]);
    }
    __syncthreads();

    BS_ST(4);
    for (int t = 0; t < (ABL(16) ? 0 : a.T); ++t) {
        PH("top", 0);
        if (!ONE && wave == 0 && t > 0) {
            const uint32_t ln = __builtin_amdgcn_mbcnt_hi(~0u, __builtin_amdgcn_mbcnt_lo(~0u, 0u));
            uint32_t x = ln < 32u ? RED[flor + ln] : 0u;
            if (ln < 32u) RED[flor + ln] = 0u;
            const uint32_t w0 = wave_or(x);
            RED[16 + t - 1] = w0;
            RED[1] &= w0;
        }
        const int nx = (t + 1) & 1;
        int ak = 0;
        bool afx = false;
        if constexpr (AFX) {
            typedef __attribute__((address_space(4))) const BsArgsAf<KArgs> ConstAf;
            ConstAf* kq = (ConstAf*)__builtin_amdgcn_kernarg_segment_ptr();
            asm volatile("" : "+s"(kq));
            const ConstW* at = (const ConstW*)kq->atid;
            afx = at != nullptr;
            if (afx) ak = (int)at[t];
        }
#pragma unroll
        for (int u = 0; u < VPL; ++u) asm volatile("" : "+s"(dw[u]), "+s"(dwmin[u]));
        if (!RPW) asm volatile("" : "+s"(cn_dmin));
        const int cdm = FZ ? W::cn_dmin : FOLDB ? (cn_dmin & (FOLDB - 1)) : cn_dmin;
        if (RPW) {
#pragma unroll
            for (int u = 0; u < VPL; ++u) asm volatile("" : "+v"(vv[u]));
        }
        if (t + 1 < a.T) {
            int cw = wave, al = AL, bl = BL, bcl = (FZ ? W::bcols : a.bcols);
            if (!FZ && !(Q8 && VPL == 1 && CPL == 1 && !UCN))
                asm volatile("" : "+s"(cw), "+s"(al), "+s"(bl), "+s"(bcl));
            const uint32_t* alut_p = a.alut;
            const uint32_t* blut_p = a.blut;
            uint32_t off_al = (FZ ? W::off_alut : a.off_alut), off_bl = (FZ ? W::off_blut : a.off_blut);
            if constexpr (VPL == 1 && CPL == 1 && !(Q8 && !UCN)) {
                typedef __attribute__((address_space(4))) const BsArgs ConstArgs;
                ConstArgs* ka = (ConstArgs*)__builtin_amdgcn_kernarg_segment_ptr();
                asm volatile("" : "+s"(ka));
                alut_p = ka->alut;
                blut_p = ka->blut;
                if constexpr (!FZ) {
                    off_al = ka->off_alut;
                    off_bl = ka->off_blut;
                }
            }
            if (!(AFX && afx))
                copy_async(off_al + 4u * (uint32_t)(nx * al), alut_p + (size_t)(t + 1) * al, al, cw, NT);
            if (bcl > 1)
                copy_async(off_bl + 4u * (uint32_t)(nx * bl), blut_p + (size_t)(t + 1) * bl, bl, cw, NT);
        }
        if constexpr (BKPF) {
            if (t + 1 < a.T && a.btid) {
#pragma unroll
                for (int u = 0; u < VPL; ++u) {
                    const int col = ((FZ ? W::bcols : a.bcols) == 1) ? 0 : pcol[u];
                    bkp[u] = col >= 0 ? a.btid[(size_t)(t + 1) * (FZ ? W::btid_n : a.btid_n) + col] : -1;
                }
            }
        }
        if (PRIO == 2) __builtin_amdgcn_s_setprio(1);
        if (PRIO == 4) __builtin_amdgcn_s_setprio(2);
#pragma unroll
        for (int c = 0; c < CPL; ++c) {
            const bool active = (CPL == 1) ? (FZ && W::cn_lanes >= W::NT) || wave * 64 < (FZ ? W::cn_lanes : a.cn_lanes) : (gchunk[c] >= 0);
            if (!active || ABL(1)) continue;
            PH("ck_addr", c);
            uint32_t cbase;
            if constexpr (GBL) {
                uint32_t all = ~0u;
                asm volatile("" : "+s"(all));
                const uint32_t ln = __builtin_amdgcn_mbcnt_hi(all, __builtin_amdgcn_mbcnt_lo(all, 0u));
                cbase = lds_w((FZ ? W::off_ch : a.off_ch) + ((uint32_t)wave << 8) + 4u * ln);
            } else {
                cbase = gbase[c];
                asm volatile("" : "+v"(cbase));
            }
            uint32_t ctab = PKG ? (cbase >> 16) : gtab[c];
            if constexpr (PKG) cbase &= 0xFFFFu;
            int gmc = gm[c];
            asm volatile("" : "+s"(gmc));
            uint32_t rp = rpk;
            if (RPW) asm volatile("" : "+v"(rp));
            const int cdeg = gdeg[c];
            auto real = [&](int m) __attribute__((always_inline)) -> bool {
                if constexpr (RPW) return ((rp >> (RB * c + m)) & 1u) != 0u;
                else return LPC * m + LPC - 1 < cdm || LPC * m + cj < cdeg;
            };
            auto caddr = [&](int m) __attribute__((always_inline)) -> uint32_t {
                return real(m) ? cbase + m * cstride : (FZ ? W::off_pad : a.off_pad);
            };
            uint32_t Xs[EPL][4], ns[EPL];
            PH("ck_read", c);
#pragma unroll
            for (int m = 0; m < EPL; ++m) read_slot(ns[m], Xs[m], caddr(m));
            uint32_t syn = 0u;
            PH("ck_syn", c);
            const bool ucn_t = ucn_on(t);
            if constexpr (UCN) {
                if (ucn_t || (ES && t > 0)) {
                    uint32_t hwv[HDW];
                    if constexpr (HDL) {
                        uint32_t all = ~0u;
                        asm volatile("" : "+s"(all));
                        const uint32_t ln = __builtin_amdgcn_mbcnt_hi(all, __builtin_amdgcn_mbcnt_lo(all, 0u));
#pragma unroll
                        for (int p = 0; p < HDW; ++p)
                            hwv[p] = lds_w(a.off_hdl + 4u * (uint32_t)(p * NT) + ((uint32_t)wave << 8) + 4u * ln);
                    } else {
#pragma unroll
                        for (int p = 0; p < HDW; ++p) {
                            asm volatile("" : "+v"(ghd[c][p]));
                            hwv[p] = ghd[c][p];
                        }
                    }
#pragma unroll
                    for (int m = 0; m < EPL; ++m) {
                        if (SKIPM && m >= gmc) continue;
                        const uint32_t hw = hwv[m >> 1];
                        syn ^= lds_w((m & 1) ? (hw >> 16) : (hw & 0xFFFFu));
                    }
                    syn ^= qperm<QP_X1>(syn);
                    if (LPC == 4) syn ^= qperm<QP_X2>(syn);
                    if constexpr (ES) {
                        if (t > 0) {
                            const uint32_t wu = wave_or(syn);
                            if (wu && BS_LANE_IS0)
                                __hip_atomic_fetch_or(RED + flor + FLORW + (t - 1), wu,
                                                      __ATOMIC_RELAXED, __HIP_MEMORY_SCOPE_WORKGROUP);
                        }
                    }
                }
            }
            PH4("ck_min", c, Xs[EPL - 1]);
            uint32_t m1[4] = {Xs[0][0], Xs[0][1], Xs[0][2], Xs[0][3]}, m2[4] = {~0u, ~0u, ~0u, ~0u};
            uint32_t par = ns[0];
            uint32_t cand[EPL];
#pragma unroll
            for (int m = 1; m < EPL; ++m) par ^= ns[m];
            if constexpr (SKIPM) {
                switch (gmc) {
#define BS_MIN2_CASE(k)                                                                            \
    case k:                                                                                        \
        if constexpr (k <= EPL) {                                                                  \
            PH("ck_mink", 16 * c + k);                                                             \
            min2_bits<k, LPC>(m1, m2, cand, Xs);                                                   \
            _Pragma("unroll") for (int m = k; m < EPL; ++m) cand[m] = 0u;                          \
        } else {                                                                                   \
            __builtin_unreachable();                                                               \
        }                                                                                          \
        break;
                    BS_MIN2_CASE(1) BS_MIN2_CASE(2) BS_MIN2_CASE(3) BS_MIN2_CASE(4) BS_MIN2_CASE(5)
                    BS_MIN2_CASE(6) BS_MIN2_CASE(7) BS_MIN2_CASE(8)
#undef BS_MIN2_CASE
                    default:
                        __builtin_unreachable();
                }
            } else {
                min2_bits<EPL, LPC>(m1, m2, cand, Xs);
            }
            PH9("ck_merge", c, m1, m2, par);
            par ^= qperm<QP_X1>(par);
            if (LPC == 4) par ^= qperm<QP_X2>(par);
            uint32_t q1[4], q2[4];
            PH9("ck_tab", c, m1, m2, par);
            if (AFX && afx) {
                beta_asm(q1, m1, ak);
                beta_asm(q2, m2, ak);
            } else {
                const uint32_t mm[2][4] = {{m1[0], m1[1], m1[2], m1[3]}, {m2[0], m2[1], m2[2], m2[3]}};
                const uint32_t tab = ctab + (uint32_t)((t & 1) * AL * 4);
                uint32_t qb[OB][2];
                bool any_unsat = false;
                if constexpr (UCN) any_unsat = ucn_t && (CPL == 1 || __builtin_amdgcn_ballot_w64(syn != 0u) != 0ull);
#pragma unroll
                for (int b = 0; b < OB; ++b) {
                    uint32_t o[2];
                    lut_bit<2>(o, mm, tab + (uint32_t)(b * 64));
                    if constexpr (UCN) {
                        if (any_unsat) {
                            uint32_t ou[2];
                            lut_bit<2>(ou, mm, tab + tabu + (uint32_t)(b * 64));
                            o[0] = mux(syn, ou[0], o[0]);
                            o[1] = mux(syn, ou[1], o[1]);
                        }
                    }
                    qb[b][0] = o[0];
                    qb[b][1] = o[1];
                }
                if (LPC == 4) {
                    q1[0] = qperm<0x00>(qb[0][0]); q1[1] = qperm<0x55>(qb[0][0]);
                    q1[2] = qperm<0xAA>(qb[0][0]); q1[3] = qperm<0xFF>(qb[0][0]);
                    q2[0] = qperm<0x00>(qb[0][1]); q2[1] = qperm<0x55>(qb[0][1]);
                    q2[2] = qperm<0xAA>(qb[0][1]); q2[3] = qperm<0xFF>(qb[0][1]);
                } else {
                    q1[0] = qperm<0xA0>(qb[0][0]); q1[1] = qperm<0xA0>(qb[OB - 1][0]);
                    q1[2] = qperm<0xF5>(qb[0][0]); q1[3] = qperm<0xF5>(qb[OB - 1][0]);
                    q2[0] = qperm<0xA0>(qb[0][1]); q2[1] = qperm<0xA0>(qb[OB - 1][1]);
                    q2[2] = qperm<0xF5>(qb[0][1]); q2[3] = qperm<0xF5>(qb[OB - 1][1]);
                }
            }
#pragma unroll
            for (int m = 0; m < EPL; ++m) {
                if (m == 0) PH8("ck_pass2", 16 * c, q1, q2);
                if (real(m)) {
                    if (m > 0) PH("ck_pass2", 16 * c + m);
                    uint32_t Mg[4];
#pragma unroll
                    for (int i = 0; i < 4; ++i) Mg[i] = mux(cand[m], q2[i], q1[i]);
                    write_slot(cbase + m * cstride, par ^ ns[m], Mg);
                }
            }
        }
        if constexpr (ONE) {
            const bool folds = FOLDB ? (cn_dmin & FOLDB) != 0 : (uint32_t)wave == a.fold_wave;
            if (folds && t > 0) {
                const uint32_t ln = __builtin_amdgcn_mbcnt_hi(~0u, __builtin_amdgcn_mbcnt_lo(~0u, 0u));
                uint32_t x = ln < 32u ? RED[flor + ln] : 0u;
                if (ln < 32u) RED[flor + ln] = 0u;
                const uint32_t w0 = wave_or(x);
                RED[16 + t - 1] = w0;
                RED[1] &= w0;
            }
        }
        BS_ST(0);
        __syncthreads();
        BS_ST(1);
        if constexpr (ES) {
            if (t > 0) {
                const uint32_t un = (uint32_t)__builtin_amdgcn_readfirstlane((int)RED[flor + FLORW + t - 1]);
                const uint32_t nn = ~un & ~es_done;
                es_done |= nn;
                if (nn) {
                    const int v = vv[0] >= 0 ? (vv[0] & 0xFFFF) : -1;
                    uint32_t nb = 0u;
                    if constexpr (EW) {
                        if (v >= 0) {
                            const uint32_t h = lds_w(4u * ((uint32_t)vv[0] >> 16)) & nn;
                            es_hd |= h;
                            if (v < a.target_bits) nb = (uint32_t)__popc(h);
                        }
                    } else
                    if (v >= 0 && v < a.target_bits)
                        nb = (uint32_t)__popc(lds_w(4u * ((uint32_t)vv[0] >> 16)) & nn);
                    nb = wave_add(nb);
                    if (nb && BS_LANE_IS0) atomicAdd(&RED[3], nb);
                }
                if (es_done == 0xFFFFFFFFu) break;
            }
        }
        if (PRIO == 2) __builtin_amdgcn_s_setprio(0);
        if (PRIO == 4) {
            if (dw[0] >= DV - 1) __builtin_amdgcn_s_setprio(1);
            else __builtin_amdgcn_s_setprio(0);
        }
        const uint32_t bslice = (FZ ? W::off_blut : a.off_blut) + (uint32_t)(nx * BL * 4);
        if (t == a.T - 1) vn_phase(false, true, bslice, t + 1);
        else vn_phase(false, false, bslice, t + 1);
        BS_ST(2);
        __syncthreads();
        BS_ST(3);
    }
    int64_t* e_counters = a.counters;
    uint8_t* e_flags = a.flags;
    uint32_t* e_iter_wrong = a.iter_wrong;
    int64_t e_B = a.B;
    if constexpr (Q8 || (VPL == 1 && CPL == 1 && UCN)) {
        typedef __attribute__((address_space(4))) const BsArgs ConstArgs;
        ConstArgs* ka = (ConstArgs*)__builtin_amdgcn_kernarg_segment_ptr();
        asm volatile("" : "+s"(ka));
        e_counters = ka->counters;
        e_flags = ka->flags;
        e_iter_wrong = ka->iter_wrong;
        e_B = ka->B;
    }
#if BS_LOOP_TU
    const int te = wave * 64 + lane_now();
#else
    const int te = tid;
#endif
    if constexpr (EW) {
        uint32_t* hdw = kern_args<KArgs>().hdw;
        const int v = vv[0] >= 0 ? (vv[0] & 0xFFFF) : -1;
        if (hdw && v >= 0) hdw[(size_t)BS_PK * nv + v] = es_hd;
    }
    if constexpr (ES) {
        __syncthreads();
        if (wave == 0) {
            const uint32_t* ESU = RED + flor + FLORW;
            const int r = te & 31;
            const bool on = te < nvalid;
            int stop = a.T - 1;
            uint32_t all = 1u, wl = 0u;
            bool open = true;
            for (int t = 0; t < a.T; ++t) {
                const bool lastt = t == a.T - 1;
                const uint32_t w = lastt ? RED[0] : RED[16 + t];
                const uint32_t u = lastt ? 0u : ESU[t];
                if (open) {
                    wl = (w >> r) & 1u;
                    all &= wl;
                    if (!((u >> r) & 1u)) {
                        stop = t;
                        open = false;
                    }
                }
            }
            const unsigned long long mw = __builtin_amdgcn_ballot_w64(on && wl != 0u);
            const unsigned long long ma = __builtin_amdgcn_ballot_w64(on && all != 0u);
            if (on) {
                if (e_flags) e_flags[b0 + te] = (uint8_t)(all | (wl << 1));
                if (kern_args<KArgs>().n_iter) kern_args<KArgs>().n_iter[b0 + te] = (uint8_t)(stop + 1);
            }
            if (te == 0 && e_counters) {
                unsigned long long* cc = reinterpret_cast<unsigned long long*>(e_counters);
                const unsigned long long c0 = RED[3], c1 = __popcll(mw), c2 = __popcll(ma);
                if (c0) atomicAdd(cc + 0, c0);
                if (c1) atomicAdd(cc + 1, c1);
                if (c2) atomicAdd(cc + 2, c2);
            }
            if (kern_args<KArgs>().iter_hist) {
                unsigned long long rem = __builtin_amdgcn_ballot_w64(on);
                while (rem) {
                    const int l = __builtin_ctzll(rem);
                    const int ts = __builtin_amdgcn_readlane(stop, l);
                    const unsigned long long m = __builtin_amdgcn_ballot_w64(on && stop == ts);
                    if (te == l)
                        atomicAdd(reinterpret_cast<unsigned long long*>(kern_args<KArgs>().iter_hist) + ts,
                                  (unsigned long long)__popcll(m));
                    rem &= ~m;
                }
            }
        }
    }
    if constexpr (!ES) {
    if (te == 0) {
        const uint32_t wl = RED[0] & valid;
        const uint32_t all = RED[1] & RED[0] & valid;
        const uint32_t ap = RED[2] & valid;
        RED[16 + a.T - 1] = RED[0];
        if (e_counters) {
            unsigned long long* cc = reinterpret_cast<unsigned long long*>(e_counters);
            const unsigned long long c0 = RED[3], c1 = __popc(wl), c2 = __popc(all),
                                     c3 = 2ull * __popc(ap) + __popc(wl & ~ap);
            if (c0) atomicAdd(cc + 0, c0);
            if (c1) atomicAdd(cc + 1, c1);
            if (c2) atomicAdd(cc + 2, c2);
            if (c3) atomicAdd(cc + 3, c3);
        }
        RED[5] = all;
        RED[6] = wl;
    }
    if (e_flags || e_iter_wrong) {
        __syncthreads();
        if (e_flags && te < nvalid)
            e_flags[b0 + te] = (uint8_t)(((RED[5] >> te) & 1) | (((RED[6] >> te) & 1) << 1));
        if (e_iter_wrong)
            for (int t = te; t < a.T; t += NT)
                e_iter_wrong[(size_t)t * (size_t)((e_B + 31) >> 5) + BS_PK] = RED[16 + t] & valid;
    }
    }
    BS_ST(5);
#if BS_LOOP_TU
#ifdef BS_STAMP
    ++npk;
#endif
    } while ((pack = (unsigned)__builtin_amdgcn_readfirstlane(
                  (int)reinterpret_cast<volatile uint32_t*>(smem + (FZ ? W::off_red : a.off_red))[BS_RED_NEXT])) <
             (unsigned)((a.B + PACK - 1) / PACK));
#elif defined(BS_STAMP)
    const unsigned long long npk = 1ull;
#endif
#undef BS_TBITS
#undef BS_PK
#undef BS_NEXT_PACK
#undef BS_LANE_IS0
#undef BS_GEN
#ifdef BS_STAMP
    if (a.stamps && lane == 0 && wave < 16) {
#pragma unroll
        for (int i = 0; i < 13; ++i) atomicAdd(a.stamps + 16 * wave + i, (unsigned long long)sacc[i]);
        atomicAdd(a.stamps + 16 * wave + 15, npk);
        uint32_t hw;
        asm volatile("s_getreg_b32 %0, hwreg(HW_REG_HW_ID)" : "=s"(hw));
        const uint32_t simd = (((hw >> 4) & 3u) - reinterpret_cast<uint32_t*>(smem + (FZ ? W::off_red : a.off_red))[12]) & 3u;
        atomicAdd(a.stamps + 16 * wave + 13 + (simd >> 1), npk << (32 * (simd & 1)));
        if (wave == 0) {
            uint32_t xcc;
            asm volatile("s_getreg_b32 %0, hwreg(HW_REG_XCC_ID)" : "=s"(xcc));
            unsigned long long* rec = a.stamps + BS_WG_BASE + (size_t)BS_WG_REC * blockIdx.x;
            rec[0] = npk;
            rec[2] = __builtin_amdgcn_s_memrealtime();
            rec[4] = __builtin_amdgcn_s_memtime();
            rec[5] = (unsigned long long)xcc << 32 | hw;
        }
    }
#endif
#undef BS_ST
}

struct BsLaunch : BsArgsEw {
    int word;
    const int32_t* atid;
    bool frozen;
    uint32_t* ticket;
};

template <class K>
K kernel_arg_of(void (*)(K));
template <class K>
struct BsAfBase { using type = void; };
template <class K>
struct BsAfBase<BsArgsAf<K>> { using type = K; };
template <class K, class L>
K bs_kernel_args(const L& a) {
    if constexpr (std::is_base_of_v<K, L>) return a;
    else if constexpr (!std::is_void_v<typename BsAfBase<K>::type>)
        return K{bs_kernel_args<typename BsAfBase<K>::type>(a), a.atid};
    else return K{a, a.word};
}
template <auto Fn>
void bs_max_lds() {
    static const hipError_t once = hipFuncSetAttribute(reinterpret_cast<const void*>(Fn),
                                                       hipFuncAttributeMaxDynamicSharedMemorySize, (int)BS_LDS_MAX);
    (void)once;
}
template <auto Fn, class L>
int bs_launch_kernel(const L& a, int nblocks, int nw, size_t lds, hipStream_t s) {
    bs_max_lds<Fn>();
    hipLaunchKernelGGL(Fn, dim3(nblocks), dim3(64 * nw), lds, s, bs_kernel_args<decltype(kernel_arg_of(Fn))>(a));
    return hipGetLastError() == hipSuccess ? LDPC_OK : LDPC_ERR_HIP;
}

template <int I, bool XP, bool Q8, bool FZ = false, bool L8 = false>
int launch_bs_x(const BsLaunch& a, int npacks, int nw, size_t lds, hipStream_t s, int grid, int* resident) {
    constexpr BsInst k = kBsInst[I];
    static_assert(bs_loops(k) == (BS_LOOP_TU != 0), "BS_LOOP_TU lists the instances of bs_loops");
    constexpr auto fn = &k_bs<k.D, k.DV, k.LPC, k.VPL, k.CPL, k.UCN, k.BIG, k.PK, k.WPE, XP, 1024, Q8, false, false, FZ, L8>;
    int nblocks = npacks;
    if constexpr (bs_loops(k)) {
        if (grid < 0) {
            if (*resident <= 0) {
                bs_max_lds<fn>();
                int dev = 0, ncu = 0, per_cu = 0;
                if (hipGetDevice(&dev) != hipSuccess ||
                    hipDeviceGetAttribute(&ncu, hipDeviceAttributeMultiprocessorCount, dev) != hipSuccess ||
                    hipOccupancyMaxActiveBlocksPerMultiprocessor(&per_cu, reinterpret_cast<const void*>(fn),
                                                                 64 * nw, lds) != hipSuccess ||
                    ncu <= 0 || per_cu <= 0) {
                    (void)hipGetLastError();
                    return LDPC_ERR_HIP;
                }
                *resident = ncu * per_cu;
            }
            grid = *resident;
        }
        if (grid > 0 && grid < npacks) nblocks = grid;
        BsLaunch t = a;
        t.cn_hd = nblocks < npacks ? a.ticket : nullptr;
        if (t.cn_hd && hipMemsetAsync(a.ticket, 0, sizeof(uint32_t), s) != hipSuccess) return LDPC_ERR_HIP;
        return bs_launch_kernel<fn>(t, nblocks, nw, lds, s);
    }
    return bs_launch_kernel<fn>(a, nblocks, nw, lds, s);
}

template <int I, bool Q8, bool EW>
int launch_bs_es_x(const BsLaunch& a, int npacks, int nw, size_t lds, hipStream_t s) {
    constexpr BsInst k = kBsInst[I];
    static_assert(k.ES && !bs_loops(k), "an early-stop instance");
    return bs_launch_kernel<&k_bs<k.D, k.DV, k.LPC, k.VPL, k.CPL, k.UCN, k.BIG, k.PK, k.WPE, false, 1024, Q8, true, EW>>(
        a, npacks, nw, lds, s);
}
constexpr bool bs_l8_inst(int i) { return i == 0 || i == 1 || i == 3 || i == 4 || i == 5 || i == kBsInstUcn1; }
enum BsSrc { BS_SRC_LLR = 0, BS_SRC_GEN = 1, BS_SRC_L8 = 2 };
template <int I>
int launch_bs_any(const BsLaunch& a, int npacks, int nw, size_t lds, hipStream_t s, int src, int grid, int* resident) {
    const bool q8 = src == BS_SRC_GEN;
    if (src == BS_SRC_L8) {
        if constexpr (bs_l8_inst(I)) {
            if (a.hdw || (a.hdx && !a.word)) return LDPC_ERR_UNSUPPORTED;
            return a.hdx ? launch_bs_x<I, true, false, false, true>(a, npacks, nw, lds, s, grid, resident + 6)
                         : launch_bs_x<I, false, false, false, true>(a, npacks, nw, lds, s, grid, resident + 5);
        }
        return LDPC_ERR_UNSUPPORTED;
    }
    if constexpr (kBsInst[I].ES) {
        if (a.hdx) return LDPC_ERR_UNSUPPORTED;
        if (a.hdw)
            return q8 ? launch_bs_es_x<I, true, true>(a, npacks, nw, lds, s)
                      : launch_bs_es_x<I, false, true>(a, npacks, nw, lds, s);
        return q8 ? launch_bs_es_x<I, true, false>(a, npacks, nw, lds, s)
                  : launch_bs_es_x<I, false, false>(a, npacks, nw, lds, s);
    } else {
        if constexpr (I == BsFrozenWman::inst) {
            if (a.frozen && !a.hdx)
                return q8 ? launch_bs_x<I, false, true, true>(a, npacks, nw, lds, s, grid, resident + 4)
                          : launch_bs_x<I, false, false, true>(a, npacks, nw, lds, s, grid, resident + 3);
        }
        if (a.hdx) return q8 ? LDPC_ERR_UNSUPPORTED : launch_bs_x<I, true, false>(a, npacks, nw, lds, s, grid, resident + 1);
        return q8 ? launch_bs_x<I, false, true>(a, npacks, nw, lds, s, grid, resident + 2)
                  : launch_bs_x<I, false, false>(a, npacks, nw, lds, s, grid, resident);
    }
}

template <int I>
int bs_launch(const BsLaunch& a, int npacks, int nw, size_t lds, hipStream_t s, int src, int grid, int* resident);

}
}
```

ldpc_error_floor_amd/csrc/ldpc_capi.hip:

```cpp
#include <algorithm>
#include <cstdio>
#include <cstring>
#include <functional>
#include <new>
#include <vector>

#include "ldpc_awgn.h"
#include "ldpc_beta_tabs.h"
#include "ldpc_internal.h"
#include "ldpc_fused.h"

using namespace ldpc;

struct ldpc_graph {
    int device = 0;
    host::GraphTables h;
    int32_t* d_tables = nullptr;
    DevGraph dev{};
    int T_w = 0;
    int per_edge_w = 0;
    std::vector<int32_t> row_merge;
    int32_t* d_row_merge = nullptr;
    float* d_alpha = nullptr;
    float* d_alpha_ucn = nullptr;
// ... 147 lines not shown
            for (int t = 0; t < p.T; ++t) a &= p.wrong[((size_t)t * p.ntiles + tile) * 4 + q];
            all[q] = a;
            ap[q] = p.anypos[(size_t)tile * 4 + q] & valid;
            c[1] += __popcll(wl[q]);
            c[2] += __popcll(all[q]);
            c[3] += 2 * __popcll(ap[q]) + __popcll(wl[q] & ~ap[q]);
        }
        c[0] += (unsigned long long)p.biterr[tile];
        if (flags) {
            for (int bl = 0; bl < TILE; ++bl) {
                const int64_t b = tile * TILE + bl;
                if (b >= p.B) break;
                const int lane = bl >> 2, q = bl & 3;
                flags[b] = (uint8_t)(((all[q] >> lane) & 1) | (((wl[q] >> lane) & 1) << 1));
            }
        }
    }
    for (int k = 0; k < 4; ++k) red[k][threadIdx.x] = c[k];
    __syncthreads();
    for (int s = 128; s > 0; s >>= 1) {
        if ((int)threadIdx.x < s)
            for (int k = 0; k < 4; ++k) red[k][threadIdx.x] += red[k][threadIdx.x + s];
        __syncthreads();
    }
    if (threadIdx.x == 0 && counters)
        for (int k = 0; k < 4; ++k)
            if (red[k][0]) atomicAdd(reinterpret_cast<unsigned long long*>(counters + k), red[k][0]);
}

int ensure_counters(ldpc_ctx* c) {
    if (c->wrong) return LDPC_OK;
    const size_t nt = (size_t)c->ntiles_max;
    int st = dev_alloc(&c->wrong, (size_t)c->T_max * nt * 4);
    if (st == LDPC_OK) st = dev_alloc(&c->anypos, nt * 4);
    if (st == LDPC_OK) st = dev_alloc(&c->biterr, nt);
    return st;
}

int ensure_flood(ldpc_ctx* c) {
    if (c->ch) return LDPC_OK;
    const ldpc_graph* g = c->g;
    const size_t nt = (size_t)c->ntiles_max;
    const size_t nv = (size_t)g->h.N * g->h.z, ne = (size_t)g->h.E * g->h.z;
    int st = dev_alloc(&c->ch, nt * nv * TILE);
    if (st == LDPC_OK) st = dev_alloc(&c->Tv, nt * nv * TILE);
    if (st == LDPC_OK) st = dev_alloc(&c->c2v, nt * ne * TILE);
    if (st == LDPC_OK) st = dev_alloc(&c->hd, (size_t)(c->T_max + 1) * nt * nv * 4);
    if (st != LDPC_OK) {
        dev_free(c->ch); dev_free(c->Tv); dev_free(c->c2v); dev_free(c->hd);
    }
    return st;
}

}

extern "C" {

int ldpc_abi_version(void) { return LDPC_NMS_ABI_VERSION; }

const char* ldpc_status_string(int status) {
    switch (status) {
        case LDPC_OK: return "ok";
        case LDPC_ERR_ARG: return "invalid argument";
        case LDPC_ERR_HIP: return "HIP runtime error";
        case LDPC_ERR_OOM: return "device out of memory";
        case LDPC_ERR_STATE: return "invalid state (weights not set or limits exceeded)";
        case LDPC_ERR_UNSUPPORTED: return "unsupported configuration";
        default: return "unknown status";
    }
}

int ldpc_graph_create(const int32_t* proto, int32_t M, int32_t N, int32_t z, int32_t device,
                      ldpc_graph** out) {
    if (!out) return LDPC_ERR_ARG;
    *out = nullptr;
    ldpc_graph* g = new (std::nothrow) ldpc_graph();
    if (!g) return LDPC_ERR_OOM;
    const int st = host::build_graph(proto, M, N, z, g->h);
    if (st != LDPC_OK) { delete g; return st; }
    g->device = device;
    const host::GraphTables& h = g->h;
    {
        DeviceGuard dg(device);
        if (dev_alloc(&g->d_tables, h.device_block.size()) != LDPC_OK) { delete g; return LDPC_ERR_OOM; }
        if (hipMemcpy(g->d_tables, h.device_block.data(), h.device_block.size() * sizeof(int32_t),
                      hipMemcpyHostToDevice) != hipSuccess) {
            dev_free(g->d_tables);
            delete g;
            return LDPC_ERR_HIP;
        }
    }
    DevGraph& d = g->dev;
    d.M = M; d.N = N; d.z = z; d.E = h.E;
    d.n_checks = M * z; d.n_vars = N * z; d.n_edges = h.E * z; d.max_cdeg = h.max_cdeg;
    const int32_t* p = g->d_tables;
    d.row_ptr = p; p += M + 1;
    d.pe_row = p; p += h.E;
    d.pe_col = p; p += h.E;
    d.pe_shift = p; p += h.E;
    d.col_ptr = p; p += N + 1;
    d.col_pe = p;
    d.vn_edge = reinterpret_cast<const int4*>(g->d_tables + h.off_vn);
    d.h_row_ptr = h.row_ptr.data();
    d.host = &g->h;
    *out = g;
    return LDPC_OK;
}

int ldpc_graph_destroy(ldpc_graph* g) {
    if (!g) return LDPC_ERR_ARG;
    DeviceGuard dg(g->device);
    dev_free(g->d_tables);
    dev_free(g->d_alpha);
    dev_free(g->d_alpha_ucn);
    dev_free(g->d_beta);
    dev_free(g->d_beta_tid);
    dev_free(g->d_alpha_tid);
    dev_free(g->d_row_merge);
    delete g;
    return LDPC_OK;
}

int ldpc_graph_query(const ldpc_graph* g, int32_t* dims) {
    if (!g || !dims) return LDPC_ERR_ARG;
    const host::GraphTables& h = g->h;
    const int32_t v[8] = {h.M, h.N, h.z, h.E, h.M * h.z, h.N * h.z, h.E * h.z, h.max_cdeg};
    std::memcpy(dims, v, sizeof(v));
    return LDPC_OK;
}

int ldpc_weights_set(ldpc_graph* g, int32_t T, const float* alpha, const float* alpha_ucn,
                     const float* beta) {
    if (!g) return LDPC_ERR_ARG;
    if (alpha && alpha_ucn && T > 0 && g->h.E > 0 &&
        std::memcmp(alpha, alpha_ucn, (size_t)T * g->h.E * sizeof(float)) == 0)
        alpha_ucn = nullptr;
    host::WeightInfo wi;
    const int sta = host::analyze_weights(g->h, T, alpha, alpha_ucn, beta, wi);
    if (sta != LDPC_OK) return sta;
    DeviceGuard dg(g->device);
    dev_free(g->d_alpha);
    dev_free(g->d_alpha_ucn);
    dev_free(g->d_beta);
    dev_free(g->d_beta_tid);
    dev_free(g->d_alpha_tid);
    g->dev.beta_tid = nullptr;
    g->h.w_alpha_tid_dev = nullptr;
    g->T_w = 0;
    const size_t ne = (size_t)T * g->h.E, nn = (size_t)T * g->h.N;
    int st = dev_alloc(&g->d_alpha, ne);
    if (st == LDPC_OK && alpha_ucn) st = dev_alloc(&g->d_alpha_ucn, ne);
    if (st == LDPC_OK) st = dev_alloc(&g->d_beta, nn);
    if (st == LDPC_OK) st = dev_alloc(&g->d_beta_tid, nn);
    const bool afix = !wi.alpha_tid.empty() &&
                      std::all_of(wi.alpha_tid.begin(), wi.alpha_tid.end(), [](int32_t k) { return k >= 0; });
    if (st == LDPC_OK && afix) st = dev_alloc(&g->d_alpha_tid, (size_t)T);
    if (st != LDPC_OK) return st;
    bool ok = hipMemcpy(g->d_alpha, alpha, ne * sizeof(float), hipMemcpyHostToDevice) == hipSuccess;
    if (alpha_ucn)
        ok = ok && hipMemcpy(g->d_alpha_ucn, alpha_ucn, ne * sizeof(float),
                             hipMemcpyHostToDevice) == hipSuccess;
    ok = ok && hipMemcpy(g->d_beta, beta, nn * sizeof(float), hipMemcpyHostToDevice) == hipSuccess;
    ok = ok && hipMemcpy(g->d_beta_tid, wi.beta_tid.data(), nn * sizeof(int32_t), hipMemcpyHostToDevice) == hipSuccess;
    if (afix)
        ok = ok && hipMemcpy(g->d_alpha_tid, wi.alpha_tid.data(), (size_t)T * sizeof(int32_t), hipMemcpyHostToDevice) == hipSuccess;
    if (!ok) return LDPC_ERR_HIP;
    g->dev.beta_tid = g->d_beta_tid;
    g->h.w_alpha_tid_dev = afix ? g->d_alpha_tid : nullptr;
    g->T_w = T;
    g->per_edge_w = wi.per_edge_w;
    g->row_merge = wi.row_merge;
    g->dev.h_row_merge = nullptr;
    g->dev.row_merge = nullptr;
    if (!g->d_row_merge) {
        const int st2 = dev_alloc(&g->d_row_merge, (size_t)g->h.M);
        if (st2 != LDPC_OK) return st2;
    }
    if (hipMemcpy(g->d_row_merge, g->row_merge.data(), (size_t)g->h.M * sizeof(int32_t),
                  hipMemcpyHostToDevice) != hipSuccess)
        return LDPC_ERR_HIP;
    g->dev.h_row_merge = g->row_merge.data();
    g->dev.row_merge = g->d_row_merge;
    g->dev.w_alpha_uniform = wi.alpha_uniform;
    g->dev.w_alpha_pair_uniform = wi.alpha_pair_uniform;
    g->dev.w_beta_uniform = wi.beta_uniform;
    g->dev.w_beta_nonneg = wi.beta_nonneg;
    g->dev.w_beta_one = wi.beta_one;
    g->dev.w_beta_id_mask = wi.beta_id_mask;
    g->dev.w_ucn_iter = wi.ucn_iter_mask;
    g->dev.w_version++;
    return LDPC_OK;
}

int ldpc_ctx_create(ldpc_graph* g, int64_t B_max, int32_t T_max, ldpc_ctx** out) {
    if (!out) return LDPC_ERR_ARG;
    *out = nullptr;
    if (!g || B_max <= 0 || T_max <= 0) return LDPC_ERR_ARG;
    ldpc_ctx* c = new (std::nothrow) ldpc_ctx();
    if (!c) return LDPC_ERR_OOM;
    c->g = g;
    c->B_max = B_max;
    c->T_max = T_max;
    c->ntiles_max = (int)((B_max + TILE - 1) / TILE);
    DeviceGuard dg(g->device);
    const int st = ensure_counters(c);
    if (st != LDPC_OK) { ldpc_ctx_destroy(c); return st; }
    *out = c;
    return LDPC_OK;
}

int ldpc_ctx_destroy(ldpc_ctx* c) {
    if (!c) return LDPC_ERR_ARG;
    DeviceGuard dg(c->g->device);
    dev_free(c->ch); dev_free(c->Tv); dev_free(c->c2v); dev_free(c->hd);
    dev_free(c->wrong); dev_free(c->anypos); dev_free(c->biterr);
    fused_free(c->fused);
    if (c->llr_scratch) (void)hipFree(c->llr_scratch);
    if (c->gen_done) (void)hipEventSynchronize(c->gen_done);
    if (c->gen_tab) (void)hipFree(c->gen_tab);
    if (c->gen_done) (void)hipEventDestroy(c->gen_done);
    delete c;
    return LDPC_OK;
}

static int decode_impl(ldpc_ctx* c, const float* llr_dev, int64_t B, const ldpc_decode_params* p,
                       const ldpc_decode_outputs* o, void* stream, const AwgnParams* gen,
                       const uint32_t* q8 = nullptr, const AwgnParams* gen8 = nullptr);

static bool auto_fused(int mode) { return mode != MODE_SP; }

int ldpc_decode(ldpc_ctx* c, const float* llr_dev, int64_t B, const ldpc_decode_params* p,
                const ldpc_decode_outputs* o, void* stream) {
    if (!llr_dev) return LDPC_ERR_ARG;
    return decode_impl(c, llr_dev, B, p, o, stream, nullptr);
}

static bool awgn_q8_on() {
    static const bool on = [] { const char* e = getenv("LDPC_AWGN_Q8"); return !(e && atoi(e) == 0); }();
    return on;
}

static bool q8_serves(const ldpc_ctx* c, const ldpc_decode_params* p, bool has_short) {
    const ldpc_graph* g = c->g;
    return awgn_q8_on() && p->decoding_type == LDPC_DEC_QMS && p->kernel != LDPC_KERNEL_FLOOD &&
           fused_q8_ok(g->dev, mode_of(p->decoding_type, p->q_bit), p->T, p->clip_llr,
                       g->d_alpha_ucn != nullptr, g->per_edge_w != 0, has_short);
}

static int ensure_gen_tab(ldpc_ctx* c, const AwgnParams& a, void* stream) {
    if (!c->gen_tab) {
        if (hipMalloc(reinterpret_cast<void**>(&c->gen_tab), sizeof(c->gen_host)) != hipSuccess) {
            (void)hipGetLastError();
            return LDPC_ERR_OOM;
        }
        c->gen_valid = false;
    }
    uint32_t tab[AWGN_TAB_W];
    awgn_gen_table(a, tab);
    if (!c->gen_done && hipEventCreateWithFlags(&c->gen_done, hipEventDisableTiming) != hipSuccess) {
        (void)hipGetLastError();
        c->gen_done = nullptr;
        return LDPC_ERR_HIP;
    }
    if (!c->gen_valid || std::memcmp(tab, c->gen_host, sizeof(tab)) != 0) {
        if (c->gen_pending && hipEventSynchronize(c->gen_done) != hipSuccess) return LDPC_ERR_HIP;
        c->gen_pending = false;
        std::memcpy(c->gen_host, tab, sizeof(tab));
        c->gen_valid = false;
        if (hipMemcpyAsync(c->gen_tab, c->gen_host, sizeof(tab), hipMemcpyHostToDevice,
                           reinterpret_cast<hipStream_t>(stream)) != hipSuccess ||
            hipStreamSynchronize(reinterpret_cast<hipStream_t>(stream)) != hipSuccess)
            return LDPC_ERR_HIP;
        c->gen_valid = true;
    }
    return LDPC_OK;
}
static int ensure_llr_scratch(ldpc_ctx* c) {
    const ldpc_graph* g = c->g;
    const int64_t n = c->B_max * (int64_t)g->h.N * g->h.z;
    if (c->llr_scratch_n >= n) return LDPC_OK;
    DeviceGuard dg(g->device);
    return dev_grow(c->llr_scratch, c->llr_scratch_n, (size_t)n);
}

static Bufs make_bufs(const ldpc_ctx* c, int64_t B, const ldpc_decode_params* p) {
    const ldpc_graph* g = c->g;
    Bufs b{};
    b.B = B;
    b.ntiles = (int)((B + TILE - 1) / TILE);
    b.T = p->T;
    b.n_vars = g->h.N * g->h.z;
    b.target_bits = p->target_bits;
    b.clip = p->clip_llr;
    b.alpha = g->d_alpha;
    b.alpha_ucn = g->d_alpha_ucn;
    b.beta = g->d_beta;
    b.count = 1;
    return b;
}

static void set_last_kernel(ldpc_ctx* c, const char* kernel, const char* mode, bool gen) {
    const size_t n = std::strlen(kernel);
    std::snprintf(c->last_kernel, sizeof(c->last_kernel), "%.*s%s%s%s", (int)(mode && n ? n - 1 : n), kernel,
                  mode ? mode : "", mode ? "]" : "", gen ? "+gen" : "");
}

int ldpc_awgn_in_kernel(const ldpc_ctx* c, const ldpc_decode_params* p, int32_t has_short, int32_t app) {
    if (!c || !p) return LDPC_ERR_ARG;
// ... 312 lines not shown
    if (!c || !llr_dev || !p) return LDPC_ERR_ARG;
    return decode_bs_impl(c, llr_dev, B, p, true, bs_outs(o), stream, nullptr, nullptr);
}

int ldpc_decode_awgn_es_word(ldpc_ctx* c, int64_t B, const ldpc_decode_params* p, const ldpc_channel_params* ch,
                             const ldpc_es_word_outputs* o, void* stream) {
    if (!o || o->size != (int32_t)sizeof(ldpc_es_word_outputs) || !o->hard_stop) return LDPC_ERR_ARG;
    if (!c || !p || !ch || !(ch->sigma > 0.0) || ch->offset < 0) return LDPC_ERR_ARG;
    return decode_awgn_es_impl(c, B, p, ch, bs_outs(o), stream);
}

int ldpc_decode_word(ldpc_ctx* c, const float* llr_dev, int64_t B, const ldpc_decode_params* p,
                     const ldpc_word_outputs* o, void* stream) {
    if (!c || !llr_dev || !p || !o || o->size != (int32_t)sizeof(ldpc_word_outputs) || !o->hard_last)
        return LDPC_ERR_ARG;
    return decode_bs_impl(c, llr_dev, B, p, false, bs_outs(o), stream, nullptr, nullptr);
}

static int q8_request(const ldpc_ctx* c, int64_t B, const ldpc_decode_params* p, bool has_short, BsReq* r) {
    const int rq = bs_request(c, B, p, false, r);
    if (rq != LDPC_OK) return rq;
    return bs_l8_ok(c->g->dev, *r, has_short) ? LDPC_OK : LDPC_ERR_UNSUPPORTED;
}

int ldpc_q8_supported(const ldpc_ctx* c, const ldpc_decode_params* p, int32_t has_short, int32_t word) {
    if (!c || !p) return LDPC_ERR_ARG;
    (void)word;
    BsReq r{};
    const int st = q8_request(c, 1, p, has_short != 0, &r);
    return st == LDPC_OK ? 1 : st == LDPC_ERR_UNSUPPORTED ? 0 : st;
}

static int decode_q8_impl(ldpc_ctx* c, const int8_t* q8_dev, int64_t B, const ldpc_decode_params* p, const BsOuts& o,
                          uint32_t* iter_wrong, void* stream) {
    BsReq r{};
    const int rq = q8_request(c, B, p, false, &r);
    if (rq != LDPC_OK) return rq;
    r.l8 = q8_dev;
    ldpc_graph* g = c->g;
    hipStream_t s = reinterpret_cast<hipStream_t>(stream);
    DeviceGuard dg(g->device);
    Bufs b = make_bufs(c, B, p);
    b.iter_wrong = iter_wrong;
    if (iter_wrong && hipMemsetAsync(iter_wrong, 0, (size_t)p->T * ((B + 31) / 32) * sizeof(uint32_t), s) != hipSuccess)
        return LDPC_ERR_HIP;
    BsOut bo{};
    bo.counters = o.counters;
    bo.flags = o.frame_flags;
    const int st = fused_decode_bs(g->dev, b, c->fused, nullptr, r, c->B_max, c->ntiles_max, bo, o.rows, o.word_flags, s);
    if (st != LDPC_OK) return st;
    set_last_kernel(c, bs_kernel_name(g->dev, r), o.rows ? ",word" : nullptr, false);
    std::strncat(c->last_kernel, "+q8", sizeof(c->last_kernel) - std::strlen(c->last_kernel) - 1);
    return hipGetLastError() == hipSuccess ? LDPC_OK : LDPC_ERR_HIP;
}

int ldpc_decode_q8(ldpc_ctx* c, const int8_t* q8_dev, int64_t B, const ldpc_decode_params* p,
                   const ldpc_decode_outputs* o, void* stream) {
    if (!q8_dev || !p) return LDPC_ERR_ARG;
    if (p->outputs_size != 0 && p->outputs_size != (int32_t)sizeof(ldpc_decode_outputs)) return LDPC_ERR_ARG;
    if (o && (o->app_all || o->hard_bits || o->synd_bits)) return LDPC_ERR_ARG;
    if (!c) return LDPC_ERR_ARG;
    const bool full = o && p->outputs_size == (int32_t)sizeof(ldpc_decode_outputs);
    const BsOuts bo{o ? o->counters : nullptr, o ? o->frame_flags : nullptr, nullptr, nullptr, nullptr, nullptr, nullptr};
    return decode_q8_impl(c, q8_dev, B, p, bo, full ? o->iter_wrong : nullptr, stream);
}

int ldpc_decode_q8_word(ldpc_ctx* c, const int8_t* q8_dev, int64_t B, const ldpc_decode_params* p,
                        const ldpc_word_outputs* o, void* stream) {
    if (!q8_dev || !o || o->size != (int32_t)sizeof(ldpc_word_outputs) || !o->hard_last) return LDPC_ERR_ARG;
    if (!c || !p) return LDPC_ERR_ARG;
    return decode_q8_impl(c, q8_dev, B, p, bs_outs(o), nullptr, stream);
}

static_assert(sizeof(ldpc_event_outputs) == 96, "ldpc_event_outputs is part of ABI 3");
static bool event_outputs_ok(const ldpc_event_outputs* o) {
    return o && o->size == (int32_t)sizeof(ldpc_event_outputs) && o->ev_count && o->ev_frame && o->ev_info &&
           o->cap >= 0;
}
static EventSink event_sink(const ldpc_event_outputs* o, int64_t frame_base, const ldpc_decode_params* p) {
    return EventSink{frame_base, o->cap, o->ev_count, o->ev_frame, o->ev_info, o->ev_word, p->target_bits};
}
static BsOuts bs_outs(const ldpc_event_outputs* o, const EventSink* ev) {
    const bool es = o->early_stop != 0;
    return BsOuts{o->counters, o->frame_flags, es ? o->n_iter : nullptr, es ? o->iter_hist : nullptr, nullptr, nullptr, ev};
}

int ldpc_events_supported(const ldpc_ctx* c, const ldpc_decode_params* p, int32_t early_stop) {
    return bs_request_supported(c, p, early_stop != 0);
}

int ldpc_decode_events(ldpc_ctx* c, const float* llr_dev, int64_t B, const ldpc_decode_params* p,
                       const ldpc_event_outputs* o, void* stream) {
    if (!event_outputs_ok(o)) return LDPC_ERR_ARG;
    if (!c || !llr_dev || !p) return LDPC_ERR_ARG;
    const EventSink ev = event_sink(o, o->frame_base, p);
    return decode_bs_impl(c, llr_dev, B, p, o->early_stop != 0, bs_outs(o, &ev), stream, nullptr, nullptr);
}

int ldpc_decode_awgn_events(ldpc_ctx* c, int64_t B, const ldpc_decode_params* p, const ldpc_channel_params* ch,
                            const ldpc_event_outputs* o, void* stream) {
    if (!event_outputs_ok(o)) return LDPC_ERR_ARG;
    if (!c || !p || !ch || !(ch->sigma > 0.0) || ch->offset < 0) return LDPC_ERR_ARG;
    if (!o->early_stop) return LDPC_ERR_UNSUPPORTED;
    const EventSink ev = event_sink(o, ch->offset, p);
    return decode_awgn_es_impl(c, B, p, ch, bs_outs(o, &ev), stream);
}

int ldpc_debug_events_out(ldpc_ctx* c, const uint32_t* planes_dev, const uint32_t* bad_dev, int64_t B,
                          int32_t target_bits, const uint8_t* n_iter_dev, int32_t T, const ldpc_event_outputs* o,
                          void* stream) {
    if (!event_outputs_ok(o)) return LDPC_ERR_ARG;
    if (!c || !planes_dev || !bad_dev || B <= 0 || target_bits < 0) return LDPC_ERR_ARG;
    ldpc_graph* g = c->g;
    if (target_bits > g->h.N * g->h.z) return LDPC_ERR_ARG;
    DeviceGuard dg(g->device);
    const EventSink ev{o->frame_base, o->cap, o->ev_count, o->ev_frame, o->ev_info, o->ev_word, target_bits};
    return events_out(g->dev, planes_dev, bad_dev, B, n_iter_dev, T, ev, o->frame_flags,
                      reinterpret_cast<hipStream_t>(stream));
}

int ldpc_ctx_last_frozen(const ldpc_ctx* c) {
    if (!c) return LDPC_ERR_ARG;
    return (c->fused.bs_frozen && std::strncmp(c->last_kernel, "bsl[", 4) == 0) ? 1 : 0;
}

extern "C" int ldpc_debug_alpha_tid(float alpha, int32_t mode, int32_t* out_id, uint8_t* table) {
    if (!out_id) return LDPC_ERR_ARG;
    const int k = host::alpha_table_id(alpha, mode);
    *out_id = k;
    if (k >= 0 && table) std::memcpy(table, kBetaTab[k], 16);
    return LDPC_OK;
}

extern "C" int ldpc_debug_alpha_tids(const int32_t* proto, int32_t M, int32_t N, int32_t z, int32_t T, const float* alpha,
                          const float* alpha_ucn, int32_t* ids) {
    if (!proto || !alpha || !ids || T <= 0) return LDPC_ERR_ARG;
    host::GraphTables h;
    int st = host::build_graph(proto, M, N, z, h);
    if (st != LDPC_OK) return st;
    const std::vector<float> beta((size_t)T * h.N, 1.0f);
    host::WeightInfo wi;
    st = host::analyze_weights(h, T, alpha, alpha_ucn, beta.data(), wi);
    if (st != LDPC_OK) return st;
    if (wi.alpha_tid.empty()) return 0;
    std::copy(wi.alpha_tid.begin(), wi.alpha_tid.end(), ids);
    return 1;
}

int ldpc_ctx_last_afix(const ldpc_ctx* c) {
    if (!c) return LDPC_ERR_ARG;
    return (c->fused.bs_afix && std::strncmp(c->last_kernel, "bsl[", 4) == 0) ? 1 : 0;
}

int ldpc_ctx_last_kernel(const ldpc_ctx* c, char* name, int32_t name_len) {
    if (!c || !name || name_len <= 0) return LDPC_ERR_ARG;
    std::strncpy(name, c->last_kernel, (size_t)name_len - 1);
    name[name_len - 1] = 0;
    return LDPC_OK;
}

}
```

ldpc_error_floor_amd/csrc/ldpc_fused.h:

```cpp
#pragma once
#include <string>

#include "ldpc_internal.h"

namespace ldpc {

struct FusedWorkspace {
    uint64_t* hd = nullptr;
    int64_t hd_elems = 0;
    void* tables = nullptr;
    size_t tables_bytes = 0;
    void* bs_graph = nullptr;
    int bs_graph_inst = -1;
    void* bs_es_graph = nullptr;
    int bs_es_graph_inst = -1;
    void* bs_lut = nullptr;
    size_t bs_lut_bytes = 0;
    uint32_t* bs_bad = nullptr;
    int64_t bs_bad_n = 0;
    int bs_resident[7] = {0, 0, 0, 0, 0, 0, 0};
    uint64_t bs_resident_key = ~0ull;
    uint32_t* bs_ticket = nullptr;
    bool bs_frozen = false;
    bool bs_afix = false;
    uint32_t* hdx = nullptr;
    int64_t hdx_elems = 0;
    bool bits_packed = false;
    uint32_t* hdw = nullptr;
    int64_t hdw_elems = 0;
    uint8_t* ev_niter = nullptr;
    int64_t ev_niter_n = 0;
    const char* last_kernel = "";
    uint64_t key_gad[4] = {~0ull, 0, 0, 0}, key_qtab[4] = {~0ull, 0, 0, 0}, key_bslut[4] = {~0ull, 0, 0, 0};
};

template <class T, class N>
int dev_grow(T*& p, N& have, size_t n, size_t elem) {
    if ((size_t)have >= n) return LDPC_OK;
    if (p) (void)hipFree(p);
    p = nullptr;
    have = 0;
    if (hipMalloc(reinterpret_cast<void**>(&p), n * elem) != hipSuccess) {
        (void)hipGetLastError();
        return LDPC_ERR_OOM;
    }
    have = (N)n;
    return LDPC_OK;
}
template <class T, class N>
int dev_grow(T*& p, N& have, size_t n) { return dev_grow(p, have, n, sizeof(T)); }

bool fused_supported(const DevGraph& g, int mode, int T, float clip_llr);
int64_t fused_bytes_per_cw(const DevGraph& g, int T);
int fused_decode(const DevGraph& g, Bufs& b, FusedWorkspace& ws, const float* llr, int mode,
                 bool ucn, bool want_bits, int ntiles_max, int T_max, int per_edge_w,
                 int64_t* counters, uint8_t* flags, hipStream_t s);
struct HdView {
    const uint64_t* tile;
    const uint32_t* pack;
    const uint32_t* bad;
};
HdView fused_bits_view(const FusedWorkspace& ws);
const char* fused_kernel_name(const DevGraph& g, int mode, int T, float clip_llr, bool ucn,
                              bool per_edge_w);

bool fused5_supported(const DevGraph& g, int T);
const char* fused5_shape_name(const DevGraph& g, int T);
int fused5_decode(const DevGraph& g, const Bufs& b, FusedWorkspace& ws, const float* llr,
                  int qmax, float step, int clip_u, bool per_edge_w, uint64_t* hd_out,
                  int64_t* counters, uint8_t* flags, hipStream_t s, const uint32_t* only = nullptr);
int fused5_cw(const DevGraph& g, int T);

struct BsReq {
    int mode;
    bool ucn, per_edge_w;
    float clip;
    int T;
    bool es;
    const int8_t* l8 = nullptr;
};
struct BsOut {
    int64_t* counters;
    uint8_t* flags;
    uint32_t* bad;
    uint32_t* hdx;
    bool word;
    uint8_t* n_iter;
    int64_t* iter_hist;
    uint32_t* hdw;
};
bool bs_supported(const DevGraph& g, const BsReq& r);
bool bs_q8_ok(const DevGraph& g, const BsReq& r, bool has_short);
bool bs_l8_ok(const DevGraph& g, const BsReq& r, bool has_short);
bool bsc_l8_ok(const DevGraph& g, const BsReq& r, bool has_short);
const char* bs_kernel_name(const DevGraph& g, const BsReq& r);
bool bsc_supported(const DevGraph& g, const BsReq& r);
bool bsc_q8_ok(const DevGraph& g, const BsReq& r, bool has_short);
const char* bsc_kernel_name(const DevGraph& g, const BsReq& r);
int bs_decode(const DevGraph& g, const Bufs& b, FusedWorkspace& ws, const float* llr, const BsReq& r,
              const BsOut& o, hipStream_t s);
int bsc_decode(const DevGraph& g, const Bufs& b, FusedWorkspace& ws, const float* llr, const BsReq& r,
               const BsOut& o, hipStream_t s);
enum { LDPC_BOUNDS_PRE_GUARD = 1, LDPC_BOUNDS_BIG_TABLES = 2, LDPC_BOUNDS_ES = 4, LDPC_BOUNDS_ES_BSC = 8,
       LDPC_BOUNDS_UCN1 = 16 };
int bsc_debug_bounds(const DevGraph& g, int mode, float clip, int T, int flags, int& violations,
                     std::string& first, bool es = false);
bool fused_q8_ok(const DevGraph& g, int mode, int T, float clip, bool ucn, bool per_edge_w, bool has_short);
bool fused_awgn_v5(const DevGraph& g, int mode, int T, float clip, bool ucn, bool per_edge_w, bool app);
constexpr int WORD_MAX_VARS = 4096;
struct EventSink {
    int64_t frame_base, cap;
    int64_t* count;
    int64_t* frame;
    int32_t* info;
    uint32_t* word;
    int target_bits;
};
bool fused_bs_supported(const DevGraph& g, const BsReq& r);
int fused_decode_bs(const DevGraph& g, const Bufs& b, FusedWorkspace& ws, const float* llr, const BsReq& r,
                    int64_t B_max, int ntiles_max, BsOut o, uint32_t* rows, uint8_t* word_flags, hipStream_t s,
                    const EventSink* ev = nullptr);
int events_out(const DevGraph& g, const uint32_t* planes, const uint32_t* bad, int64_t B, const uint8_t* n_iter,
               int T, const EventSink& ev, uint8_t* frame_flags, hipStream_t s);
int word_out(const DevGraph& g, const uint32_t* planes, const uint32_t* bad, int64_t B, uint32_t* hard_last,
             uint8_t* word_flags, uint8_t* frame_flags, hipStream_t s);
void fused_free(FusedWorkspace& ws);

bool ffl_mode(int mode);
bool ffl_supported(const DevGraph& g, int mode, bool ucn, bool per_edge_w);
const char* ffl_kernel_name(const DevGraph& g, int mode, bool ucn, bool per_edge_w);
int ffl_decode(const DevGraph& g, const Bufs& b, const float* llr, int mode, bool ucn, bool per_edge_w,
               int64_t* counters, uint8_t* flags, hipStream_t s);

}
```

ldpc_error_floor_amd/csrc/ldpc_host.cpp:

```cpp
#include "ldpc_host.h"
#include "ldpc_beta_tabs.h"

#include <algorithm>
#include <climits>
#include <cmath>

namespace ldpc {
namespace host {

int build_graph(const int32_t* proto, int32_t M, int32_t N, int32_t z, GraphTables& g) {
    g = GraphTables{};
    if (!proto || M <= 0 || N <= 0 || z <= 0) return LDPC_ERR_ARG;
    if ((int64_t)M * N * z > INT32_MAX) return LDPC_ERR_ARG;
    g.M = M;
    g.N = N;
    g.z = z;
    g.row_ptr.assign((size_t)M + 1, 0);
    for (int i = 0; i < M; ++i)
        for (int j = 0; j < N; ++j) {
            const int32_t s = proto[(size_t)i * N + j];
            if (s < -1) return LDPC_ERR_ARG;
            if (s != -1) {
                g.pe_row.push_back(i);
                g.pe_col.push_back(j);
                g.pe_shift.push_back(s % z);
            }
        }
    g.E = (int)g.pe_row.size();
    if (g.E == 0) return LDPC_ERR_ARG;
    for (int e = 0; e < g.E; ++e) g.row_ptr[(size_t)g.pe_row[e] + 1]++;
    for (int i = 0; i < M; ++i) {
        g.max_cdeg = std::max(g.max_cdeg, g.row_ptr[(size_t)i + 1]);
        g.row_ptr[(size_t)i + 1] += g.row_ptr[i];
    }
    if (g.max_cdeg > kMaxCheckDegree) return LDPC_ERR_UNSUPPORTED;
    g.col_ptr.assign((size_t)N + 1, 0);
    for (int e = 0; e < g.E; ++e) g.col_ptr[(size_t)g.pe_col[e] + 1]++;
    for (int j = 0; j < N; ++j) {
        g.max_vdeg = std::max(g.max_vdeg, g.col_ptr[(size_t)j + 1]);
        g.col_ptr[(size_t)j + 1] += g.col_ptr[j];
    }
    g.col_pe.assign((size_t)g.E, 0);
    {
        std::vector<int32_t> fill(g.col_ptr.begin(), g.col_ptr.end() - 1);
        for (int e = 0; e < g.E; ++e) g.col_pe[(size_t)fill[(size_t)g.pe_col[e]]++] = e;
    }
    std::vector<int32_t>& h = g.device_block;
    h.insert(h.end(), g.row_ptr.begin(), g.row_ptr.end());
    h.insert(h.end(), g.pe_row.begin(), g.pe_row.end());
    h.insert(h.end(), g.pe_col.begin(), g.pe_col.end());
    h.insert(h.end(), g.pe_shift.begin(), g.pe_shift.end());
    h.insert(h.end(), g.col_ptr.begin(), g.col_ptr.end());
    h.insert(h.end(), g.col_pe.begin(), g.col_pe.end());
    while (h.size() % 4) h.push_back(0);
    g.off_vn = h.size();
    for (int e = 0; e < g.E; ++e) {
        const int pe = g.col_pe[(size_t)e], i = g.pe_row[(size_t)pe], r0 = g.row_ptr[(size_t)i];
        h.push_back(r0 * z + (pe - r0));
        h.push_back(g.row_ptr[(size_t)i + 1] - r0);
        h.push_back(g.pe_shift[(size_t)pe]);
        h.push_back(((i * z) << 6) | (pe - r0));
    }
    return LDPC_OK;
}

int beta_table_id(float b) {
    if (!(b >= 0.f)) return -1;
    uint8_t t[16];
    for (int m = 0; m < 16; ++m)
        t[m] = (uint8_t)std::min(15.f, std::fabs(std::nearbyint((float)m * b)));
    int lo = 0, hi = kNBetaTab;
    int sum = 0;
    for (int m = 0; m < 16; ++m) sum += t[m];
    for (int k = lo; k < hi; ++k) {
        int s = 0;
        for (int m = 0; m < 16; ++m) s += kBetaTab[k][m];
        if (s != sum) continue;
        if (std::equal(t, t + 16, kBetaTab[k])) return k;
    }
    return -1;
}

static void alpha_table(float alpha, float step, uint8_t (&t)[16]) {
    const float inv = 1.0f / step;
    for (int m = 0; m < 16; ++m) {
        const float mv = (float)m * step;
        float x = mv * alpha;
        x = (x > 0.f) ? x : 0.f;
        const float r = std::nearbyint(x * inv);
        t[m] = (uint8_t)std::min(std::max(r, -15.f), 15.f);
    }
}

int alpha_table_id(float alpha, int mode) {
    if (mode != MODE_Q5 && mode != MODE_QM5) return -1;
    uint8_t t[16];
    alpha_table(alpha, mode == MODE_Q5 ? 0.5f : 1.0f, t);
    for (int k = 0; k < kNBetaTab; ++k)
        if (std::equal(t, t + 16, kBetaTab[k])) return k;
    return -1;
}

int analyze_weights(const GraphTables& g, int32_t T, const float* alpha, const float* alpha_ucn,
                    const float* beta, WeightInfo& w) {
    w = WeightInfo{};
    if (T <= 0 || !alpha || !beta || g.E <= 0) return LDPC_ERR_ARG;
    if ((int64_t)T * g.E > INT32_MAX || (int64_t)T * g.N > INT32_MAX) return LDPC_ERR_ARG;
    for (int t = 0; t < T && !w.per_edge_w; ++t)
        for (int i = 0; i < g.M && !w.per_edge_w; ++i)
            for (int e = g.row_ptr[(size_t)i] + 1; e < g.row_ptr[(size_t)i + 1]; ++e) {
                const size_t a0 = (size_t)t * g.E + g.row_ptr[(size_t)i], a1 = (size_t)t * g.E + e;
                if (alpha[a1] != alpha[a0] || (alpha_ucn && alpha_ucn[a1] != alpha_ucn[a0])) {
                    w.per_edge_w = 1;
                    break;
                }
            }
    w.row_merge.assign((size_t)g.M, 0);
    for (int i = 1; i < g.M && !w.per_edge_w; ++i) {
        const int deg = g.row_ptr[(size_t)i + 1] - g.row_ptr[(size_t)i];
        bool same = deg == g.row_ptr[(size_t)i] - g.row_ptr[(size_t)i - 1];
        for (int t = 0; t < T && same && deg > 0; ++t) {
            const size_t a0 = (size_t)t * g.E + g.row_ptr[(size_t)i - 1];
            const size_t a1 = (size_t)t * g.E + g.row_ptr[(size_t)i];
            same = alpha[a1] == alpha[a0] && (!alpha_ucn || alpha_ucn[a1] == alpha_ucn[a0]);
        }
        w.row_merge[(size_t)i] = same ? 1 : 0;
    }
    w.alpha_uniform = (!w.per_edge_w && !alpha_ucn) ? 1 : 0;
    w.alpha_pair_uniform = !w.per_edge_w ? 1 : 0;
    for (int t = 0; t < T && w.alpha_pair_uniform; ++t) {
        const size_t a0 = (size_t)t * g.E;
        for (int e = 1; e < g.E && w.alpha_pair_uniform; ++e)
            if (alpha[a0 + e] != alpha[a0] || (alpha_ucn && alpha_ucn[a0 + e] != alpha_ucn[a0]))
                w.alpha_pair_uniform = 0;
    }
    w.beta_uniform = 1;
    w.beta_nonneg = 1;
    w.beta_one = 1;
    for (int t = 0; t < T && t < 64; ++t) {
        bool id = true;
        for (int j = 0; j < g.N && id; ++j) {
            const float b = beta[(size_t)t * g.N + j];
            for (int m = 0; m <= 15 && id; ++m) {
                const float q = std::nearbyint((float)m * b);
                id = std::min(15.f, std::fabs(q)) == (float)m && !(b < 0.f);
            }
        }
        if (id) w.beta_id_mask |= (uint64_t)1 << t;
    }
    if (alpha_ucn)
        for (int t = 0; t < T && t < 64; ++t)
            for (int e = 0; e < g.E; ++e)
                if (alpha_ucn[(size_t)t * g.E + e] != alpha[(size_t)t * g.E + e]) {
                    w.ucn_iter_mask |= (uint64_t)1 << t;
                    break;
                }
    w.beta_tid.resize((size_t)T * g.N);
    for (size_t x = 0; x < (size_t)T * g.N; ++x) w.beta_tid[x] = beta_table_id(beta[x]);
    for (int t = 0; t < T; ++t) {
        const float a0 = alpha[(size_t)t * g.E], b0 = beta[(size_t)t * g.N];
        for (int e = 1; e < g.E && w.alpha_uniform; ++e)
            if (alpha[(size_t)t * g.E + e] != a0) w.alpha_uniform = 0;
        for (int j = 0; j < g.N; ++j) {
            const float b = beta[(size_t)t * g.N + j];
            if (b != b0) w.beta_uniform = 0;
            if (!(b >= 0.f)) w.beta_nonneg = 0;
            if (b != 1.f) w.beta_one = 0;
        }
    }
    if (w.alpha_uniform) {
        w.alpha_tid.resize((size_t)T);
        for (int t = 0; t < T; ++t) {
            const float a0 = alpha[(size_t)t * g.E];
            const int k = alpha_table_id(a0, MODE_Q5);
            w.alpha_tid[(size_t)t] = (k == alpha_table_id(a0, MODE_QM5)) ? k : -1;
        }
    }
    return LDPC_OK;
}

int check_decode(const GraphTables& g, int64_t B, int64_t B_max, int32_t T_max, int32_t T_w,
                 const ldpc_decode_params* p, int* mode) {
    if (!p) return LDPC_ERR_ARG;
    if (B <= 0 || B > B_max || p->T <= 0 || p->T > T_max) return LDPC_ERR_STATE;
    if (T_w < p->T) return LDPC_ERR_STATE;
    const int m = mode_of(p->decoding_type, p->q_bit);
    if (m < 0) return LDPC_ERR_ARG;
    if (p->target_bits <= 0 || p->target_bits > g.N * g.z) return LDPC_ERR_ARG;
    if (!(p->clip_llr > 0.f) || !std::isfinite(p->clip_llr)) return LDPC_ERR_ARG;
    if (p->kernel != LDPC_KERNEL_AUTO && p->kernel != LDPC_KERNEL_FLOOD &&
        p->kernel != LDPC_KERNEL_FUSED)
        return LDPC_ERR_ARG;
    if (mode) *mode = m;
    return LDPC_OK;
}

int check_channel(int64_t B, int32_t n_vars, double sigma, int64_t offset, int32_t decoding_type,
                  int32_t q_bit, int32_t punct_start, int32_t punct_end, int32_t short_start,
                  int32_t short_end, float clip_llr) {
    if (B <= 0 || n_vars <= 0 || !(sigma > 0.0) || !std::isfinite(sigma) || offset < 0)
        return LDPC_ERR_ARG;
    if (mode_of(decoding_type, q_bit) < 0) return LDPC_ERR_ARG;
    if (punct_start < 0 || short_start < 0) return LDPC_ERR_ARG;
    if (punct_start > 0 && punct_end < punct_start) return LDPC_ERR_ARG;
    if (short_start > 0 && short_end < short_start) return LDPC_ERR_ARG;
    if (!(clip_llr > 0.f) || !std::isfinite(clip_llr)) return LDPC_ERR_ARG;
    return LDPC_OK;
}

std::pair<int, int> order_variable_edges(std::vector<uint32_t>& A, const std::vector<int>& deg, int DV,
                                         int rounds) {
    auto round_cost = [&](int h0, int f) {
        uint32_t seen[32];
        int ns = 0, cnt[32] = {0}, mx = 0, sq = 0;
        for (int l = h0; l < h0 + 32; ++l) {
            const uint32_t ad = A[(size_t)l * DV + f];
            bool dup = false;
            for (int i = 0; i < ns && !dup; ++i) dup = seen[i] == ad;
            if (dup) continue;
            seen[ns++] = ad;
            const int c = ++cnt[(ad >> 2) & 31];
            mx = std::max(mx, c);
            sq += 2 * c - 1;
        }
        return mx * 4096 + sq;
    };
    int before = 0, after = 0;
    uint64_t rng = 0x9E3779B97F4A7C15ull;
    for (int h0 = 0; h0 < 64; h0 += 32) {
        std::vector<int> cost(rounds);
        std::vector<int> movable;
        for (int l = h0; l < h0 + 32; ++l)
            if (deg[l] >= 2) movable.push_back(l);
        for (int f = 0; f < rounds; ++f) {
            cost[f] = round_cost(h0, f);
            before += cost[f] / 4096;
        }
        for (int it = 0; it < 4000 && !movable.empty(); ++it) {
            rng = rng * 6364136223846793005ull + 1442695040888963407ull;
            const int l = movable[(rng >> 33) % movable.size()];
            const int f1 = (int)((rng >> 17) % (uint64_t)deg[l]);
            int f2 = (int)((rng >> 45) % (uint64_t)(deg[l] - 1));
            if (f2 >= f1) ++f2;
            std::swap(A[(size_t)l * DV + f1], A[(size_t)l * DV + f2]);
            const int c1 = round_cost(h0, f1), c2 = round_cost(h0, f2);
            if (c1 + c2 <= cost[f1] + cost[f2]) {
                cost[f1] = c1;
                cost[f2] = c2;
            } else {
                std::swap(A[(size_t)l * DV + f1], A[(size_t)l * DV + f2]);
            }
        }
        for (int f = 0; f < rounds; ++f) after += cost[f] / 4096;
    }
    return {before, after};
}

void awgn_qms_levels(double sigma, int q_bit, int* nb, int* kmin, uint32_t* thr_hi, uint32_t* thr_lo,
                     float* val) {
    double u, cmax;
    switch (q_bit) {
        case 6: u = 1.0; cmax = 15.5; break;
        case 5: u = 0.5; cmax = 7.5; break;
        case -5: u = 1.0; cmax = 15.0; break;
        case 4: u = 1.0; cmax = 7.0; break;
        default: u = 2.0; cmax = 6.0; break;
    }
    const int K = (int)std::ceil(cmax / u) + 1;
    auto Q = [&](int k) { return std::min(std::max(k * u, -cmax), cmax); };
    int n = 0;
    val[0] = (float)Q(-K);
    const double s2 = sigma * sigma;
    for (int k = -K + 1; k <= K; ++k) {
        if (Q(k) == Q(k - 1)) continue;
        const double x = (k - 0.5) * u;
        const double nz = (x * s2 * 0.5 + 1.0) / sigma;
        uint64_t T;
        if (nz < 0.0) {
            T = (uint64_t)std::ldexp(0.5 * std::erfc(-nz * 0.7071067811865476), 64);
        } else {
            const uint64_t tail = (uint64_t)std::ldexp(0.5 * std::erfc(nz * 0.7071067811865476), 64);
            T = tail == 0 ? ~(uint64_t)0 : (uint64_t)0 - tail;
        }
        thr_hi[n] = (uint32_t)(T >> 32);
        thr_lo[n] = (uint32_t)T;
        ++n;
        val[n] = (float)Q(k);
    }
    *nb = n;
    *kmin = q_bit == 6 ? 0 : (int)std::lround(-cmax / u);
}

}
}
```

ldpc_error_floor_amd/csrc/ldpc_host.h:

```cpp
#pragma once
#include <cstddef>
#include <cstdint>
#include <utility>
#include <vector>

#include "ldpc_nms.h"

namespace ldpc {

enum Mode : int { MODE_Q6 = 0, MODE_Q5, MODE_QM5, MODE_Q4, MODE_Q3, MODE_MS, MODE_MSNN, MODE_SP };
constexpr bool mode_is_qms(int m) { return m >= 0 && m <= MODE_Q3; }

inline int mode_of(int decoding_type, int q_bit) {
    if (decoding_type == LDPC_DEC_SP) return MODE_SP;
    if (decoding_type == LDPC_DEC_MS) return MODE_MS;
    if (decoding_type == LDPC_DEC_MS_NONUDGE) return MODE_MSNN;
    if (decoding_type != LDPC_DEC_QMS) return -1;
    switch (q_bit) {
        case 6: return MODE_Q6;
        case 5: return MODE_Q5;
        case -5: return MODE_QM5;
        case 4: return MODE_Q4;
        case 3: return MODE_Q3;
        default: return -1;
    }
}

namespace host {

constexpr int kMaxCheckDegree = 64;

struct GraphTables {
    int M = 0, N = 0, z = 0, E = 0;
    int max_cdeg = 0, max_vdeg = 0;
    std::vector<int32_t> row_ptr;
    std::vector<int32_t> pe_row;
    std::vector<int32_t> pe_col;
    std::vector<int32_t> pe_shift;
    std::vector<int32_t> col_ptr;
    std::vector<int32_t> col_pe;
    std::vector<int32_t> device_block;
    size_t off_vn = 0;
    const int32_t* w_alpha_tid_dev = nullptr;
};

int build_graph(const int32_t* proto, int32_t M, int32_t N, int32_t z, GraphTables& out);

struct WeightInfo {
    int per_edge_w = 0;
    int alpha_uniform = 0, beta_uniform = 0, beta_nonneg = 0, beta_one = 0;
    int alpha_pair_uniform = 0;
    uint64_t beta_id_mask = 0;
    uint64_t ucn_iter_mask = 0;
    std::vector<int32_t> row_merge;
    std::vector<int32_t> beta_tid;
    std::vector<int32_t> alpha_tid;
};
int beta_table_id(float beta);
int alpha_table_id(float alpha, int mode);
int analyze_weights(const GraphTables& g, int32_t T, const float* alpha, const float* alpha_ucn,
                    const float* beta, WeightInfo& out);

int check_decode(const GraphTables& g, int64_t B, int64_t B_max, int32_t T_max, int32_t T_w,
                 const ldpc_decode_params* p, int* mode);

int check_channel(int64_t B, int32_t n_vars, double sigma, int64_t offset, int32_t decoding_type,
                  int32_t q_bit, int32_t punct_start, int32_t punct_end, int32_t short_start,
                  int32_t short_end, float clip_llr);

std::pair<int, int> order_variable_edges(std::vector<uint32_t>& A, const std::vector<int>& deg, int DV,
                                         int rounds);

void awgn_qms_levels(double sigma, int q_bit, int* nb, int* kmin, uint32_t* thr_hi, uint32_t* thr_lo,
                     float* val);

}
}
```

ldpc_error_floor_amd/csrc/pybind_module.cpp:

```cpp
#include <pybind11/numpy.h>
#include <pybind11/pybind11.h>

#include <algorithm>
#include <stdexcept>
#include <string>

#include "ldpc_nms.h"
#include "ldpc_nms_debug.h"

namespace py = pybind11;

static void check(int st, const char* what) {
    if (st < 0)
        throw std::runtime_error(std::string(what) + ": " + ldpc_status_string(st) + " (" +
                                 std::to_string(st) + ")");
}

struct Graph {
    ldpc_graph* h = nullptr;
    explicit Graph(py::array_t<int32_t, py::array::c_style | py::array::forcecast> proto, int z,
                   int device) {
        if (proto.ndim() != 2) throw std::invalid_argument("proto must be 2-D");
        check(ldpc_graph_create(proto.data(), (int32_t)proto.shape(0), (int32_t)proto.shape(1), z,
                                device, &h),
// ... 408 lines not shown
        "decode_awgn_events",
        [](Ctx& c, int64_t B, int T, int decoding_type, int q_bit, int target_bits, float clip,
           int kernel, double sigma, uint64_t seed, int64_t offset, int ps, int pe, int ss, int se,
           bool early_stop, int64_t cap, uintptr_t ev_count, uintptr_t ev_frame, uintptr_t ev_info,
           uintptr_t ev_word, uintptr_t counters, uintptr_t flags, uintptr_t n_iter, uintptr_t iter_hist,
           uintptr_t stream) {
            ldpc_decode_params p = make_params(T, decoding_type, q_bit, target_bits, clip, kernel);
            ldpc_channel_params ch = make_channel(sigma, seed, offset, ps, pe, ss, se);
            ldpc_event_outputs o = make_event_outputs(early_stop, 0, cap, ev_count, ev_frame, ev_info, ev_word,
                                                      counters, flags, n_iter, iter_hist);
            int st;
            {
                py::gil_scoped_release nogil;
                st = ldpc_decode_awgn_events(c.h, B, &p, &ch, &o, reinterpret_cast<void*>(stream));
            }
            check(st, "ldpc_decode_awgn_events");
        },
        py::arg("ctx"), py::arg("B"), py::arg("T"), py::arg("decoding_type"), py::arg("q_bit"),
        py::arg("target_bits"), py::arg("clip"), py::arg("kernel"), py::arg("sigma"),
        py::arg("seed"), py::arg("offset"), py::arg("punct_start"), py::arg("punct_end"),
        py::arg("short_start"), py::arg("short_end"), py::arg("early_stop"), py::arg("cap"),
        py::arg("ev_count"), py::arg("ev_frame"), py::arg("ev_info"), py::arg("ev_word") = 0,
        py::arg("counters") = 0, py::arg("flags") = 0, py::arg("n_iter") = 0, py::arg("iter_hist") = 0,
        py::arg("stream") = 0);
    m.def(
        "events_supported",
        [](Ctx& c, int T, int decoding_type, int q_bit, int target_bits, int kernel, float clip, bool early_stop) {
            ldpc_decode_params p = make_params(T, decoding_type, q_bit, target_bits, clip, kernel);
            const int st = ldpc_events_supported(c.h, &p, early_stop ? 1 : 0);
            check(st, "ldpc_events_supported");
            return st == 1;
        },
        py::arg("ctx"), py::arg("T"), py::arg("decoding_type"), py::arg("q_bit"),
        py::arg("target_bits"), py::arg("kernel"), py::arg("clip_llr") = 20.0f, py::arg("early_stop") = false);
    m.def(
        "debug_events_out",
        [](Ctx& c, uintptr_t planes, uintptr_t bad, int64_t B, int target_bits, uintptr_t n_iter, int T,
           int64_t frame_base, int64_t cap, uintptr_t ev_count, uintptr_t ev_frame, uintptr_t ev_info,
           uintptr_t ev_word, uintptr_t flags, uintptr_t stream) {
            ldpc_event_outputs o = make_event_outputs(false, frame_base, cap, ev_count, ev_frame, ev_info, ev_word,
                                                      0, flags, 0, 0);
            check(ldpc_debug_events_out(c.h, reinterpret_cast<const uint32_t*>(planes),
                                        reinterpret_cast<const uint32_t*>(bad), B, target_bits,
                                        reinterpret_cast<const uint8_t*>(n_iter), T, &o,
                                        reinterpret_cast<void*>(stream)),
                  "ldpc_debug_events_out");
        },
        py::arg("ctx"), py::arg("planes"), py::arg("bad"), py::arg("B"), py::arg("target_bits"),
        py::arg("n_iter"), py::arg("T"), py::arg("frame_base"), py::arg("cap"), py::arg("ev_count"),
        py::arg("ev_frame"), py::arg("ev_info"), py::arg("ev_word") = 0, py::arg("flags") = 0,
        py::arg("stream") = 0);
    m.def(
        "channel_awgn",
        [](uintptr_t llr, int64_t B, int n_vars, double sigma, uint64_t seed, int64_t offset,
           int decoding_type, int q_bit, int ps, int pe, int ss, int se, float clip,
           uintptr_t stream) {
            int st;
            {
                py::gil_scoped_release nogil;
                st = ldpc_channel_awgn(reinterpret_cast<float*>(llr), B, n_vars, sigma, seed, offset,
                                       decoding_type, q_bit, ps, pe, ss, se, clip,
                                       reinterpret_cast<void*>(stream));
            }
            check(st, "ldpc_channel_awgn");
        },
        py::arg("llr"), py::arg("B"), py::arg("n_vars"), py::arg("sigma"), py::arg("seed"),
        py::arg("offset"), py::arg("decoding_type"), py::arg("q_bit"), py::arg("punct_start"),
        py::arg("punct_end"), py::arg("short_start"), py::arg("short_end"), py::arg("clip"),
        py::arg("stream") = 0);
    m.def(
        "channel_awgn_rows",
        [](uintptr_t rows, uintptr_t idx, int64_t n, int n_vars, double sigma, uint64_t seed,
           int64_t offset, int decoding_type, int q_bit, int ps, int pe, int ss, int se, float clip,
           uintptr_t stream) {
            check(ldpc_channel_awgn_rows(reinterpret_cast<float*>(rows), reinterpret_cast<const int64_t*>(idx),
                                         n, n_vars, sigma, seed, offset, decoding_type, q_bit, ps, pe,
                                         ss, se, clip, reinterpret_cast<void*>(stream)),
                  "ldpc_channel_awgn_rows");
        },
        py::arg("rows"), py::arg("idx"), py::arg("n"), py::arg("n_vars"), py::arg("sigma"),
        py::arg("seed"), py::arg("offset"), py::arg("decoding_type"), py::arg("q_bit"),
        py::arg("punct_start"), py::arg("punct_end"), py::arg("short_start"), py::arg("short_end"),
        py::arg("clip"), py::arg("stream") = 0);
    m.def(
        "collect_frames",
        [](uintptr_t flags, int64_t B, uint32_t mask, uint32_t want, uintptr_t idx, int64_t cap,
           uintptr_t count, uintptr_t stream) {
            check(ldpc_collect_frames(reinterpret_cast<const uint8_t*>(flags), B, mask, want,
                                      reinterpret_cast<int64_t*>(idx), cap,
                                      reinterpret_cast<int64_t*>(count),
                                      reinterpret_cast<void*>(stream)),
                  "ldpc_collect_frames");
        },
        py::arg("flags"), py::arg("B"), py::arg("mask"), py::arg("want"), py::arg("idx"),
        py::arg("cap"), py::arg("count"), py::arg("stream") = 0);
    m.def(
        "gather_rows",
        [](uintptr_t src, int64_t n_cols, uintptr_t idx, int64_t n, uintptr_t dst, uintptr_t stream) {
            check(ldpc_gather_rows(reinterpret_cast<const float*>(src), n_cols,
                                   reinterpret_cast<const int64_t*>(idx), n,
                                   reinterpret_cast<float*>(dst), reinterpret_cast<void*>(stream)),
                  "ldpc_gather_rows");
        },
        py::arg("src"), py::arg("n_cols"), py::arg("idx"), py::arg("n"), py::arg("dst"),
        py::arg("stream") = 0);
    m.def(
        "kernel_info",
        [](Ctx& c, int T, int decoding_type, int q_bit, int target_bits, int kernel, float clip) {
            ldpc_decode_params p = make_params(T, decoding_type, q_bit, target_bits, clip, kernel);
            int64_t bytes = 0;
            char name[64] = {0};
            check(ldpc_kernel_info(c.h, &p, &bytes, name, 64), "ldpc_kernel_info");
            return py::make_tuple(bytes, std::string(name));
        },
        py::arg("ctx"), py::arg("T"), py::arg("decoding_type"), py::arg("q_bit"),
        py::arg("target_bits"), py::arg("kernel"), py::arg("clip_llr") = 20.0f);
    m.def(
        "awgn_in_kernel",
        [](Ctx& c, int T, int decoding_type, int q_bit, int target_bits, int kernel, float clip,
           bool has_short, bool app) {
            ldpc_decode_params p = make_params(T, decoding_type, q_bit, target_bits, clip, kernel);
            const int r = ldpc_awgn_in_kernel(c.h, &p, has_short ? 1 : 0, app ? 1 : 0);
            check(r < 0 ? r : 0, "ldpc_awgn_in_kernel");
            return r == 1;
        },
        py::arg("ctx"), py::arg("T"), py::arg("decoding_type"), py::arg("q_bit"),
        py::arg("target_bits"), py::arg("kernel"), py::arg("clip_llr") = 20.0f,
        py::arg("has_short") = false, py::arg("app") = false);
    m.def(
        "last_kernel",
        [](Ctx& c) {
            char name[64] = {0};
            check(ldpc_ctx_last_kernel(c.h, name, 64), "ldpc_ctx_last_kernel");
            return std::string(name);
        },
        py::arg("ctx"));
    m.def(
        "last_frozen",
        [](Ctx& c) {
            const int r = ldpc_ctx_last_frozen(c.h);
            check(r < 0 ? r : 0, "ldpc_ctx_last_frozen");
            return r == 1;
        },
        py::arg("ctx"));
    m.def(
        "last_afix",
        [](Ctx& c) {
            const int r = ldpc_ctx_last_afix(c.h);
            check(r < 0 ? r : 0, "ldpc_ctx_last_afix");
            return r == 1;
        },
        py::arg("ctx"));
    m.def(
        "format_uncor_rows",
        [](py::array_t<float, py::array::c_style | py::array::forcecast> rows) {
            if (rows.ndim() != 2 || rows.shape(1) <= 0)
                throw std::invalid_argument("rows must be [n, n_cols] with n_cols > 0");
            const int64_t n = rows.shape(0), nc = rows.shape(1);
            const int64_t step = std::max<int64_t>(1, (64 << 20) / LDPC_UNCOR_ROW_BOUND(nc));
            std::string out, buf;
            out.reserve((size_t)(n * (12 + 6 * nc)));
            buf.resize((size_t)(std::min(n, step) * LDPC_UNCOR_ROW_BOUND(nc)));
            {
                py::gil_scoped_release nogil;
                for (int64_t r0 = 0; r0 < n; r0 += step) {
                    const int64_t k = std::min(step, n - r0);
                    int64_t len = 0;
                    check(ldpc_format_uncor_rows(rows.data() + r0 * nc, k, nc, buf.data(),
                                                 (int64_t)buf.size(), &len),
                          "ldpc_format_uncor_rows");
                    out.append(buf.data(), (size_t)len);
                }
            }
            return py::bytes(out);
        },
        py::arg("rows"));
}
```

ldpc_error_floor_amd/decoder.py:

```python
from __future__ import annotations

from dataclasses import dataclass
from typing import Optional

import numpy as np

from . import _native
from .code import TannerGraph
from .config import DECODING_MS, DECODING_MS_NONUDGE, DECODING_QMS, DECODING_SP, VALID_Q_BITS
from .weights import DecoderWeights

__all__ = ["NMSDecoder", "Decoder", "DecodeResult", "KERNELS"]

KERNELS = {"auto": 0, "flood": 1, "fused": 2}
Q8_GRIDS = {5: (0.5, 15), -5: (1.0, 15), 4: (1.0, 7), 3: (2.0, 3)}


@dataclass
class DecodeResult:
    app: Optional["object"] = None
    hard: Optional["object"] = None
    synd: Optional["object"] = None
    counters: Optional["object"] = None
    flags: Optional["object"] = None
# ... 401 lines not shown
        if native and isinstance(llr, torch.Tensor) and llr.device.type == "cuda":
            x = llr.to(dtype=torch.float32).contiguous()
            out = torch.empty(x.shape, dtype=torch.int8, device=x.device)
            bad = torch.zeros(1, dtype=torch.int64, device=x.device)
            if x.numel():
                with torch.cuda.device(x.device):
                    self._ext.llr_to_q8(x.data_ptr(), x.numel(), self.q_bit, self.clip, out.data_ptr(), bad.data_ptr(),
                                        torch.cuda.current_stream(x.device).cuda_stream)
            nbad = int(bad.item()) if strict else 0
        else:
            x = np.asarray(llr.cpu().numpy() if isinstance(llr, torch.Tensor) else llr, dtype=np.float32)
            g = x * np.float32(1.0 / step)
            q = np.clip(np.rint(np.nan_to_num(g, nan=0.0)), -qmax, qmax)
            lo, hi = x == np.float32(-self.clip), x == np.float32(self.clip)
            ok = q == g
            q = np.where(~ok & lo, -128, np.where(~ok & hi, 127, q)).astype(np.int8)
            nbad = int((~(ok | lo | hi)).sum())
            out = torch.from_numpy(q)
        if strict and nbad:
            raise ValueError(f"quantize_q8: {nbad} values are neither on the q_bit={self.q_bit} grid "
                             f"(multiples of {step} within +-{qmax * step}) nor +-clip_LLR")
        return out

    def dequantize_q8(self, q8):
        torch = self._torch
        step, _ = self._q8_grid()
        q = q8 if isinstance(q8, torch.Tensor) else torch.from_numpy(np.ascontiguousarray(np.asarray(q8, np.int8)))
        if q.dtype != torch.int8:
            raise ValueError("q8 must be int8")
        x = q.to(torch.float32) * step
        x = torch.where(q == -128, torch.full_like(x, -self.clip), x)
        return torch.where(q == 127, torch.full_like(x, self.clip), x)

    def _as_q8(self, q8):
        torch = self._torch
        if not isinstance(q8, torch.Tensor):
            a = np.asarray(q8)
            if a.dtype != np.int8:
                raise ValueError("q8 must be int8")
            q8 = torch.from_numpy(np.ascontiguousarray(a))
        if q8.dtype != torch.int8:
            raise ValueError("q8 must be int8 (decode() takes LLRs of any other dtype)")
        q8 = q8.to(device=self.device)
        B = q8.shape[0]
        q8 = q8.reshape(B, -1) if B else q8.reshape(0, self.n_vars)
        if q8.shape[1] != self.n_vars:
            raise ValueError(f"q8 has {q8.shape[1]} bits per codeword, graph has {self.n_vars}")
        return q8 if q8.is_contiguous() else q8.contiguous()

    def _q8_invalid_rows(self, q8):
        _, qmax = self._q8_grid()
        ok = ((q8 >= -qmax) & (q8 <= qmax)) | (q8 == -128) | (q8 == 127)
        return ~ok.all(dim=1)

    def decode_q8(self, q8, T: Optional[int] = None, counters=None, flags=False, iter_wrong: bool = False,
                  hard_last=False, word_flags: bool = False, kernel: Optional[str] = None, stream=None,
                  on_invalid: str = "raise", app: bool = False, hard: bool = False, synd: bool = False,
                  target_bits: Optional[int] = None) -> DecodeResult:
        torch = self._torch
        if on_invalid not in ("raise", "mark"):
            raise ValueError("on_invalid must be 'raise' or 'mark'")
        T = self.T if T is None else int(T)
        nt = self.target_bits if target_bits is None else int(target_bits)
        if T > self.T:
            raise ValueError(f"T={T} exceeds the {self.T} iterations the weights cover")
        word = hard_last is not False and hard_last is not None
        if word_flags and not word:
            raise ValueError("word_flags is an output of hard_last=True")
        if word and iter_wrong:
            raise ValueError("hard_last serves word_flags, counters and flags only, not iter_wrong")
        q8 = self._as_q8(q8)
        B = int(q8.shape[0])
        if app or hard or synd or not self.supports_q8(word=word, T=T, kernel=kernel):
            if on_invalid == "raise" and B:
                badrows = self._q8_invalid_rows(q8)
                if bool(badrows.any().item()):
                    first = int(badrows.nonzero()[0].item())
                    raise ValueError(f"decode_q8: frame {first} holds a byte that is no q8 value "
                                     "(on_invalid='mark' decodes it as an off-grid LLR)")
            return self.decode(self.dequantize_q8(q8), T=T, app=bool(app), hard=hard, synd=synd, counters=counters,
                               flags=flags, kernel=kernel, stream=stream, target_bits=target_bits,
                               iter_wrong=iter_wrong, hard_last=hard_last, word_flags=word_flags,
                               on_off_grid="mark")
        dev = self.device
        res = self._word_result(B, hard_last) if word else DecodeResult()
        asked = flags is not None and flags is not False
        check = on_invalid == "raise"
        self._es_outputs(res, B, T, counters, flags if asked else check, False, None)
        if word and word_flags:
            res.word_flags = torch.empty(B, dtype=torch.uint8, device=dev)
        if iter_wrong:
            res.iter_wrong = torch.empty((T, (B + 31) // 32), dtype=torch.int32, device=dev)
        if B == 0:
            return res
        ctx = self._ensure_ctx(B, T)
        if stream is None:
            stream = torch.cuda.current_stream(dev)
        ptr = lambda t: 0 if t is None else t.data_ptr()
        if word:
            self._ext.decode_q8_word(ctx, q8.data_ptr(), B, T, self.decoding_type, self.q_bit, nt, self.clip,
                                     KERNELS[kernel or self.kernel], res.hard_last.data_ptr(), ptr(res.word_flags),
                                     ptr(res.counters), ptr(res.flags), stream.cuda_stream)
        else:
            self._ext.decode_q8(ctx, q8.data_ptr(), B, T, self.decoding_type, self.q_bit, nt, self.clip,
                                KERNELS[kernel or self.kernel], ptr(res.counters), ptr(res.flags),
                                ptr(res.iter_wrong), stream.cuda_stream)
        if check:
            stream.synchronize()
            marked = (res.flags[:B] == 0x80).nonzero()
            if marked.numel():
                raise ValueError(f"decode_q8: frame {int(marked[0].item())} is the first of {int(marked.numel())} "
                                 "frames in packs holding a byte that is no q8 value; they were not decoded "
                                 "(on_invalid='mark' returns them marked)")
            if not asked:
                res.flags = None
        return res

    def awgn_q8(self, B: int, sigma: float, seed: int, offset: int = 0, punct=None, short=None,
                out=None, stream=None):
        torch = self._torch
        if self.decoding_type != DECODING_QMS or self.q_bit not in Q8_GRIDS:
            raise ValueError("awgn_q8 covers the QMS grids q_bit 5, -5, 4 and 3 only")
        punct = getattr(self, "punct", (0, 0)) if punct is None else punct
        short = getattr(self, "short", (0, 0)) if short is None else short
        if out is None:
            out = torch.empty((B, self.n_vars), dtype=torch.int8, device=self.device)
        elif (out.dtype != torch.int8 or out.device != self.device or not out.is_contiguous() or
              out.numel() < B * self.n_vars):
            raise ValueError("out must be a contiguous int8 [B, N*z] tensor on the decoder's device")
        if stream is None:
            stream = torch.cuda.current_stream(self.device)
        self._ext.channel_awgn_q8(out.data_ptr(), int(B), self.n_vars, float(sigma), int(seed), int(offset),
                                  self.q_bit, int(punct[0]), int(punct[1]), int(short[0]), int(short[1]),
                                  stream.cuda_stream)
        return out

    def generates_channel_in_kernel(self, T=None, kernel=None, app: bool = False) -> bool:
        T = self.T if T is None else T
        ctx = self._ensure_ctx(1, T)
        short = getattr(self, "short", (0, 0)) or (0, 0)
        return bool(self._ext.awgn_in_kernel(ctx, T, self.decoding_type, self.q_bit, self.target_bits,
                                             KERNELS[kernel or self.kernel], self.clip,
                                             has_short=short[0] > 0, app=app))

    def last_kernel(self) -> str:
        return "" if self._ctx is None else self._ext.last_kernel(self._ctx)

    def last_frozen(self) -> bool:
        return False if self._ctx is None else bool(self._ext.last_frozen(self._ctx))

    def last_afix(self) -> bool:
        return False if self._ctx is None else bool(self._ext.last_afix(self._ctx))

    def _empty_result(self, T, nt, hard, synd, counters, flags, app, iter_wrong=False):
        torch = self._torch
        dev = self.device
        res = DecodeResult()
        if app:
            res.app = torch.empty((T, 0, nt), dtype=torch.float32, device=dev)
        if hard:
            res.hard = torch.empty((T, 0, (self.n_vars + 31) // 32), dtype=torch.int32, device=dev)
        if synd:
            res.synd = torch.empty((T, 0, (self.n_checks + 31) // 32), dtype=torch.int32, device=dev)
        if counters is True:
            counters = torch.zeros(4, dtype=torch.int64, device=dev)
        res.counters = counters if counters is not None else None
        if isinstance(flags, torch.Tensor):
            res.flags = flags[:0]
        elif flags:
            res.flags = torch.empty(0, dtype=torch.uint8, device=dev)
        if iter_wrong:
            res.iter_wrong = torch.empty((T, 0), dtype=torch.int32, device=dev)
        return res

    def decode_awgn(self, B: int, sigma: float, seed: int, offset: int = 0, punct=None, short=None,
                    T: Optional[int] = None, app: bool = False, counters=None, flags=None,
                    kernel: Optional[str] = None, stream=None, iter_wrong: bool = False,
                    early_stop: bool = False, n_iter: bool = False, iter_hist=None,
                    hard_last=False, word_flags: bool = False, events=None) -> DecodeResult:
        want_word = hard_last is not False and hard_last is not None
        if events is not None:
            if not early_stop:
                raise ValueError("decode_awgn does not serve events without early_stop: use "
                                 "decode(awgn(...), events=buf, frame_base=offset)")
            bad = [k for k, v in dict(hard_last=want_word, app=app, iter_wrong=iter_wrong, word_flags=word_flags).items() if v]
            if bad:
                raise ValueError("events serves counters and flags (with early_stop: n_iter and iter_hist) only, "
                                 "not " + ", ".join(bad))
            T = self.T if T is None else int(T)
            if T > self.T:
                raise ValueError(f"T={T} exceeds the {self.T} iterations the weights cover")
            punct = getattr(self, "punct", (0, 0)) if punct is None else punct
            short = getattr(self, "short", (0, 0)) if short is None else short
            return self._decode_events(None, int(B), T, self.target_bits, events, 0, True, counters, flags, n_iter,
                                       iter_hist, kernel, stream, "mark",
                                       channel=(sigma, seed, offset, punct, short))
        if want_word and not early_stop:
            raise ValueError("decode_awgn does not serve hard_last: use decode(awgn(...), hard_last=True)")
        if word_flags and not want_word:
            raise ValueError("word_flags is an output of hard_last=True")
        torch = self._torch
        T = self.T if T is None else int(T)
        punct = getattr(self, "punct", (0, 0)) if punct is None else punct
        short = getattr(self, "short", (0, 0)) if short is None else short
        if early_stop:
            self._es_check_exports(app=app, iter_wrong=iter_wrong)
            if T > self.T:
                raise ValueError(f"T={T} exceeds the {self.T} iterations the weights cover")
            B = int(B)
            if want_word:
                return self._decode_es_word(None, B, T, self.target_bits, hard_last, word_flags, counters, flags,
                                            n_iter, iter_hist, kernel, stream, "mark",
                                            channel=(sigma, seed, offset, punct, short))
            res = DecodeResult()
            if B == 0:
                return self._es_outputs(res, 0, T, counters, flags, n_iter, iter_hist)
            ctx = self._ensure_ctx(B, T)
            self._es_outputs(res, B, T, counters, flags, n_iter, iter_hist)
            if stream is None:
                stream = torch.cuda.current_stream(self.device)
            ptr = lambda t: 0 if t is None else t.data_ptr()
            self._ext.decode_awgn_es(ctx, B, T, self.decoding_type, self.q_bit, self.target_bits,
                                     self.clip, KERNELS[kernel or self.kernel], float(sigma), int(seed),
                                     int(offset), int(punct[0]), int(punct[1]), int(short[0]),
                                     int(short[1]), ptr(res.counters), ptr(res.flags), ptr(res.n_iter),
                                     ptr(res.iter_hist), stream.cuda_stream)
            return res
        if n_iter or (iter_hist is not None and iter_hist is not False):
            raise ValueError("n_iter and iter_hist are outputs of early_stop=True")
        if int(B) == 0:
            return self._empty_result(T, self.target_bits, False, False, counters, flags, app, iter_wrong)
        ctx = self._ensure_ctx(int(B), T)
        dev = self.device
        res = DecodeResult()
        if app:
            res.app = torch.empty((T, B, self.target_bits), dtype=torch.float32, device=dev)
        if counters is True:
            counters = torch.zeros(4, dtype=torch.int64, device=dev)
        if counters is not None:
            if counters.dtype != torch.int64 or counters.numel() < 4 or counters.device != dev:
                raise ValueError("counters must be an int64[4] tensor on the decoder's device")
            res.counters = counters
        if isinstance(flags, torch.Tensor):
            if flags.dtype != torch.uint8 or flags.device != dev or flags.numel() < B:
                raise ValueError("flags tensor must be uint8 on the decoder's device, >= B long")
            res.flags = flags
        elif flags:
            res.flags = torch.empty(B, dtype=torch.uint8, device=dev)
        if iter_wrong:
            res.iter_wrong = torch.empty((T, (int(B) + 31) // 32), dtype=torch.int32, device=dev)
        if stream is None:
            stream = torch.cuda.current_stream(dev)
        ptr = lambda t: 0 if t is None else t.data_ptr()
        self._ext.decode_awgn(ctx, int(B), T, self.decoding_type, self.q_bit, self.target_bits,
                              self.clip, KERNELS[kernel or self.kernel], float(sigma), int(seed),
                              int(offset), int(punct[0]), int(punct[1]), int(short[0]),
                              int(short[1]), ptr(res.app), ptr(res.counters), ptr(res.flags),
                              stream.cuda_stream, ptr(res.iter_wrong))
        return res

    def _uncorrected_index(self, flags, stream):
        torch = self._torch
        B = int(flags.shape[0])
        idx = torch.empty(max(B, 1), dtype=torch.int64, device=self.device)
        cnt = torch.empty(1, dtype=torch.int64, device=self.device)
        self._ext.collect_frames(flags.data_ptr(), B, 1, 1, idx.data_ptr(), B, cnt.data_ptr(),
                                 stream.cuda_stream)
        stream.synchronize()
        n = int(cnt.item())
        return torch.sort(idx[:n]).values.contiguous()

    def collect_uncorrected(self, flags, llr, stream=None):
        torch = self._torch
        if stream is None:
            stream = torch.cuda.current_stream(self.device)
        sel = self._uncorrected_index(flags, stream)
        n = int(sel.numel())
        if n == 0:
            return np.zeros((0, self.n_vars), np.float32)
        llr = llr.reshape(llr.shape[0], -1)
        rows = torch.empty((n, self.n_vars), dtype=torch.float32, device=self.device)
        for s0 in range(0, n, 65535):
            s1 = min(n, s0 + 65535)
            self._ext.gather_rows(llr.data_ptr(), self.n_vars, sel[s0:].data_ptr(), s1 - s0,
                                  rows[s0:].data_ptr(), stream.cuda_stream)
        return rows.cpu().numpy()

    def collect_uncorrected_awgn(self, flags, sigma: float, seed: int, offset: int = 0,
                                 punct=None, short=None, stream=None):
        torch = self._torch
        if stream is None:
            stream = torch.cuda.current_stream(self.device)
        punct = getattr(self, "punct", (0, 0)) if punct is None else punct
        short = getattr(self, "short", (0, 0)) if short is None else short
        with torch.cuda.stream(stream):
            sel = self._uncorrected_index(flags, stream)
            n = int(sel.numel())
            if n == 0:
                return np.zeros((0, self.n_vars), np.float32)
            rows = torch.empty((n, self.n_vars), dtype=torch.float32, device=self.device)
            self._ext.channel_awgn_rows(rows.data_ptr(), sel.data_ptr(), n, self.n_vars, float(sigma),
                                        int(seed), int(offset), self.decoding_type, self.q_bit,
                                        int(punct[0]), int(punct[1]), int(short[0]), int(short[1]),
                                        self.clip, stream.cuda_stream)
            return rows.cpu().numpy()

# ... 42 lines not shown
```

Before: 314.9 million.

## Freeze per-iteration weight table ids into kernel to skip LUT copies

Adds a 'weights frozen' (WF) kernel variant for the frozen wman geometry. When the alpha and beta weights map to fixed table ids that are uniform across columns, the per-iteration ids are packed into LDS once at startup. The check and variable updates then use inline table selection instead of async-copying the alpha/beta LUTs from global memory every iteration. This removes per-iteration LUT copy traffic and kernarg reads, at the cost of another template instantiation and more host-side weight analysis.

Result: faster. 324.4 million (median of 6 runs) (+3.0%).

```diff
diff --git a/include/ldpc_nms.h b/include/ldpc_nms.h
--- a/include/ldpc_nms.h
+++ b/include/ldpc_nms.h
@@ -79,6 +79,8 @@
 int ldpc_ctx_last_frozen(const ldpc_ctx* c);
 
 int ldpc_ctx_last_afix(const ldpc_ctx* c);
+
+int ldpc_ctx_last_wf(const ldpc_ctx* c);
 
 int ldpc_channel_awgn(float* llr_dev, int64_t B, int32_t n_vars, double sigma, uint64_t seed,
                       int64_t offset, int32_t decoding_type, int32_t q_bit, int32_t punct_start,
diff --git a/include/ldpc_nms_debug.h b/include/ldpc_nms_debug.h
--- a/include/ldpc_nms_debug.h
+++ b/include/ldpc_nms_debug.h
@@ -23,6 +23,11 @@
 int ldpc_debug_alpha_tids(const int32_t* proto, int32_t M, int32_t N, int32_t z, int32_t T,
                           const float* alpha, const float* alpha_ucn, int32_t* ids);
 
+int ldpc_debug_bs_wf(const int32_t* proto, int32_t M, int32_t N, int32_t z, int32_t T_w,
+                     const float* alpha, const float* alpha_ucn, const float* beta, int32_t T,
+                     int32_t mode, int32_t kind, float clip, int32_t* aids, int32_t* bids,
+                     uint64_t* identity, const int32_t* alpha_tid_in);
+
 int ldpc_debug_events_out(ldpc_ctx* ctx, const uint32_t* planes_dev, const uint32_t* bad_dev, int64_t B,
                           int32_t target_bits, const uint8_t* n_iter_dev, int32_t T,
                           const ldpc_event_outputs* outputs, void* stream);
diff --git a/ldpc_error_floor_amd/csrc/ldpc_bs.hip b/ldpc_error_floor_amd/csrc/ldpc_bs.hip
--- a/ldpc_error_floor_amd/csrc/ldpc_bs.hip
+++ b/ldpc_error_floor_amd/csrc/ldpc_bs.hip
@@ -247,6 +247,25 @@
     if (bs_plan_fields(g, q) != bs_frozen_fields()) return false;
     p = q;
     return true;
+}
+
+struct BsWeightPath { bool bfix, afix, wf; };
+static BsWeightPath bs_weight_path(const DevGraph& g, const BsPlan& p, const BsReq& r, bool frozen, bool have_atid) {
+    BsWeightPath w{false, false, false};
+    if (!p.ok) return w;
+    const BsInst& k = kBsInst[p.inst];
+    w.bfix = bs_qmax(r.mode) == QMAX && !getenv("LDPC_BS_NOBFIX");
+    if (bs_loops(k) && !p.ucn && p.arows == 1 && (r.mode == MODE_Q5 || r.mode == MODE_QM5)) {
+        const char* e = getenv("LDPC_BS_AFIX");
+        w.afix = (e ? atoi(e) != 0 : true) && have_atid;
+    }
+    const char* e = getenv("LDPC_BS_WF");
+    if (!frozen || !w.bfix || !w.afix || p.bcols != 1 || (e && atoi(e) == 0)) return w;
+    const std::vector<int32_t>& wb = g.host->w_wf_beta;
+    if ((int)wb.size() < r.T) return w;
+    w.wf = true;
+    for (int t = 0; t < r.T; ++t) w.wf = w.wf && wb[(size_t)t] >= 0;
+    return w;
 }
 
 #ifndef BS_DEAL_DEFAULT
@@ -744,14 +763,13 @@
     a.blut = blut;
     a.arows = p.arows;
     a.bcols = p.bcols;
-    a.btid = (bs_qmax(r.mode) == QMAX && !getenv("LDPC_BS_NOBFIX")) ? g.beta_tid : nullptr;
+    const BsWeightPath wp = bs_weight_path(g, p, r, frozen, g.host->w_alpha_tid_dev != nullptr);
+    a.btid = wp.bfix ? g.beta_tid : nullptr;
     a.btid_n = g.N;
-    a.atid = nullptr;
-    if (bs_loops(k) && !p.ucn && p.arows == 1 && (r.mode == MODE_Q5 || r.mode == MODE_QM5)) {
-        const char* e = getenv("LDPC_BS_AFIX");
-        if (e ? atoi(e) != 0 : true) a.atid = g.host->w_alpha_tid_dev;
-    }
+    a.atid = wp.afix ? g.host->w_alpha_tid_dev : nullptr;
     ws.bs_afix = a.atid != nullptr;
+    a.wf = wp.wf && a.atid != nullptr && a.btid != nullptr;
+    ws.bs_wf = a.wf;
     a.counters = o.counters;
     a.flags = o.flags;
     a.bad = o.bad;
@@ -786,7 +804,7 @@
     const uint64_t rkey = (uint64_t)p.inst << 48 | (uint64_t)p.nw << 32 | (uint64_t)lds;
     if (ws.bs_resident_key != rkey) {
         ws.bs_resident_key = rkey;
-        std::fill(ws.bs_resident, ws.bs_resident + 7, 0);
+        std::fill(ws.bs_resident, ws.bs_resident + 9, 0);
     }
 #ifdef BS_STAMP
     static unsigned long long* dst = nullptr;
@@ -849,6 +867,7 @@
     BsPlan p = bs_route(g, r, &to_bsc);
     ws.bs_frozen = false;
     ws.bs_afix = false;
+    ws.bs_wf = false;
     if (!p.ok) return to_bsc ? bsc_decode(g, b, ws, llr, r, o, s) : LDPC_ERR_UNSUPPORTED;
     const bool frozen = bs_frozen_fit(g, p, r, o.hdx != nullptr || o.hdw != nullptr);
     return bs_run(g, b, ws, p, llr, r, o, frozen, s);
@@ -1041,6 +1060,47 @@
         names[names_len - 1] = 0;
     }
     return fz ? 1 : 0;
+}
+
+extern "C" int ldpc_debug_bs_wf(const int32_t* proto, int32_t M, int32_t N, int32_t z, int32_t T_w,
+                                const float* alpha, const float* alpha_ucn, const float* beta, int32_t T,
+                                int32_t mode, int32_t kind, float clip, int32_t* aids, int32_t* bids,
+                                uint64_t* identity, const int32_t* alpha_tid_in) {
+    using namespace ldpc;
+    using namespace ldpc::bs;
+    if (!proto || !alpha || !beta || T <= 0 || T > T_w || kind < 0 || kind > 2) return LDPC_ERR_ARG;
+    host::GraphTables h;
+    int st = host::build_graph(proto, M, N, z, h);
+    if (st != LDPC_OK) return st;
+    if (alpha_ucn && std::memcmp(alpha, alpha_ucn, (size_t)T_w * h.E * sizeof(float)) == 0) alpha_ucn = nullptr;
+    host::WeightInfo wi;
+    st = host::analyze_weights(h, T_w, alpha, alpha_ucn, beta, wi);
+    if (st != LDPC_OK) return st;
+    if (alpha_tid_in && !wi.alpha_tid.empty()) wi.alpha_tid.assign(alpha_tid_in, alpha_tid_in + T_w);
+    const bool have_atid = host::set_weight_ids(h, wi);
+    DevGraph g{};
+    g.M = h.M; g.N = h.N; g.z = h.z; g.E = h.E;
+    g.n_checks = h.M * h.z; g.n_vars = h.N * h.z; g.n_edges = h.E * h.z; g.max_cdeg = h.max_cdeg;
+    g.h_row_ptr = h.row_ptr.data();
+    g.host = &h;
+    g.w_alpha_uniform = wi.alpha_uniform;
+    g.w_alpha_pair_uniform = wi.alpha_pair_uniform;
+    g.w_beta_uniform = wi.beta_uniform;
+    g.w_beta_nonneg = wi.beta_nonneg;
+    g.w_beta_one = wi.beta_one;
+    g.w_beta_id_mask = wi.beta_id_mask;
+    g.w_ucn_iter = wi.ucn_iter_mask;
+    const BsReq r{mode, alpha_ucn != nullptr, wi.per_edge_w != 0, clip, T, kind == 1};
+    bool to_bsc;
+    BsPlan p = bs_route(g, r, &to_bsc);
+    const bool fz = bs_frozen_fit(g, p, r, kind == 2);
+    const BsWeightPath wp = bs_weight_path(g, p, r, fz, have_atid);
+    for (int t = 0; t < T; ++t) {
+        if (aids) aids[t] = wp.afix ? h.w_alpha_tid[(size_t)t] : -1;
+        if (bids) bids[t] = wp.bfix ? wi.beta_tid[(size_t)t * h.N] : -1;
+    }
+    if (identity) *identity = wi.beta_id_mask;
+    return wp.wf ? 1 : 0;
 }
 
 extern "C" int ldpc_debug_bs_bounds(const int32_t* proto, int32_t M, int32_t N, int32_t z, int32_t T,
diff --git a/ldpc_error_floor_amd/csrc/ldpc_bs_kernel.h b/ldpc_error_floor_amd/csrc/ldpc_bs_kernel.h
--- a/ldpc_error_floor_amd/csrc/ldpc_bs_kernel.h
+++ b/ldpc_error_floor_amd/csrc/ldpc_bs_kernel.h
@@ -456,6 +456,7 @@
 template <class K>
 using BsKernArgs = std::conditional_t<BS_LOOP_TU != 0, BsArgsAf<K>, K>;
 constexpr int BS_RED_NEXT = 8;
+constexpr int BS_WF_IDENT = kNBetaTab;
 #define BS_PACK_SETUP(pk)                                                                          \
     const int64_t b0 = (int64_t)(pk) * PACK;                                                       \
     const int nvalid = (int)min<int64_t>(PACK, a.B - b0);                                          \
@@ -472,7 +473,7 @@
     };
 
 template <int D, int DV, int LPC, int VPL, int CPL, bool UCN, bool BIG, bool PK, int WPE, bool XP, int LB, bool Q8,
-          bool ES = false, bool EW = false, bool FZ = false, bool L8 = false>
+          bool ES = false, bool EW = false, bool FZ = false, bool L8 = false, bool WF = false>
 __global__ void __launch_bounds__(LB) __attribute__((amdgpu_waves_per_eu(WPE)))
 k_bs(BsKernArgs<std::conditional_t<ES, std::conditional_t<EW, BsArgsEw, BsArgsEs>, std::conditional_t<XP, BsArgsXp, BsArgs>>> a) {
     static_assert(LPC == 2 || LPC == 4, "lanes per check");
@@ -504,6 +505,8 @@
     constexpr bool BKPF = !XP && VPL > 1;
     constexpr bool AFX = BS_LOOP_TU != 0;
     static_assert(!AFX || (ONE && !UCN), "fixed-set check tables: the one-chunk instances without UCN");
+    static_assert(!WF || (FZ && AFX && !BIG && !L8), "weights frozen in kind: on the geometry-frozen builds");
+    static_assert(!WF || BsFrozenWman::cn_lanes >= BsFrozenWman::NT, "weights frozen in kind: every wave holds check lanes");
     extern __shared__ __attribute__((aligned(16))) unsigned char smem[];
     if ((uint32_t)(uintptr_t)smem != 0u) __builtin_trap();
 #ifdef BS_STAMP
@@ -646,7 +649,7 @@
     BS_ST(8);
     uint32_t cs[VPL], cm[VPL][4], bg[VPL];
     int off = 0;
-    if (T0A) {
+    if (T0A && !WF) {
         copy_async((FZ ? W::off_alut : a.off_alut), a.alut, AL, wave, NT);
         copy_async((FZ ? W::off_blut : a.off_blut), a.blut, BL, wave, NT);
     }
@@ -791,8 +794,24 @@
     int bkp[VPL];
 #pragma unroll
     for (int u = 0; u < VPL; ++u) bkp[u] = -1;
+    [[maybe_unused]] int wf_bk = 0;
+    if constexpr (WF) {
+        wf_bk = (a.beta_id & 1) ? BS_WF_IDENT
+                                : __builtin_amdgcn_readfirstlane((int)((const ConstW*)a.btid)[0]);
+    }
     auto beta_lw = [&](const int u, const uint32_t bslice, const int tb, const uint32_t (&cmu)[4],
                        uint32_t (&lw)[4], const bool use_bk) __attribute__((always_inline)) {
+        if constexpr (WF) {
+            if (ABL(2) || wf_bk >= BS_WF_IDENT) {
+                PH("vn_beta_id", u);
+#pragma unroll
+                for (int i = 0; i < 4; ++i) lw[i] = cmu[i];
+            } else {
+                PH("vn_beta_fix", u);
+                beta_asm(lw, cmu, wf_bk);
+            }
+            return;
+        }
         int bk = -1;
         if constexpr (!XP) {
             if (use_bk && a.btid) {
@@ -1009,6 +1028,15 @@
 
     vn_phase(true, false, (FZ ? W::off_blut : a.off_blut), 0);
     BS_ST(12);
+    [[maybe_unused]] uint32_t wf_idw = 0u;
+    if constexpr (WF) {
+        if (tid < a.T) {
+            wf_idw = (uint32_t)kern_args<BsArgsAf<KArgs>>().atid[tid];
+            if (tid + 1 < a.T)
+                wf_idw |= (((a.beta_id >> (tid + 1)) & 1) ? (uint32_t)BS_WF_IDENT
+                                                          : (uint32_t)a.btid[(size_t)(tid + 1) * W::btid_n]) << 16;
+        }
+    }
     const int cj = lane % LPC;
     int gchunk[CPL], gdeg[CPL], gm[CPL];
     uint32_t gbase[CPL], gtab[CPL], ghd[CPL][UCN ? HDW : 1];
@@ -1042,6 +1070,9 @@
     const uint32_t tabu = (uint32_t)((FZ ? W::arows : a.arows) * LUT_W * 4);
     constexpr bool GBL = CPL == 1;
     if constexpr (GBL) lds_put((FZ ? W::off_ch : a.off_ch) + 4u * (uint32_t)tid, gbase[0]);
+    if constexpr (WF) {
+        if (tid < a.T) lds_put(W::off_alut + 4u * (uint32_t)tid, wf_idw);
+    }
     constexpr bool HDL = UCN && CPL == 1;
     if constexpr (HDL) {
 #pragma unroll
@@ -1063,7 +1094,7 @@
         const int nx = (t + 1) & 1;
         int ak = 0;
         bool afx = false;
-        if constexpr (AFX) {
+        if constexpr (AFX && !WF) {
             typedef __attribute__((address_space(4))) const BsArgsAf<KArgs> ConstAf;
             ConstAf* kq = (ConstAf*)__builtin_amdgcn_kernarg_segment_ptr();
             asm volatile("" : "+s"(kq));
@@ -1079,28 +1110,30 @@
 #pragma unroll
             for (int u = 0; u < VPL; ++u) asm volatile("" : "+v"(vv[u]));
         }
-        if (t + 1 < a.T) {
-            int cw = wave, al = AL, bl = BL, bcl = (FZ ? W::bcols : a.bcols);
-            if (!FZ && !(Q8 && VPL == 1 && CPL == 1 && !UCN))
-                asm volatile("" : "+s"(cw), "+s"(al), "+s"(bl), "+s"(bcl));
-            const uint32_t* alut_p = a.alut;
-            const uint32_t* blut_p = a.blut;
-            uint32_t off_al = (FZ ? W::off_alut : a.off_alut), off_bl = (FZ ? W::off_blut : a.off_blut);
-            if constexpr (VPL == 1 && CPL == 1 && !(Q8 && !UCN)) {
-                typedef __attribute__((address_space(4))) const BsArgs ConstArgs;
-                ConstArgs* ka = (ConstArgs*)__builtin_amdgcn_kernarg_segment_ptr();
-                asm volatile("" : "+s"(ka));
-                alut_p = ka->alut;
-                blut_p = ka->blut;
-                if constexpr (!FZ) {
-                    off_al = ka->off_alut;
-                    off_bl = ka->off_blut;
+        if constexpr (!WF) {
+            if (t + 1 < a.T) {
+                int cw = wave, al = AL, bl = BL, bcl = (FZ ? W::bcols : a.bcols);
+                if (!FZ && !(Q8 && VPL == 1 && CPL == 1 && !UCN))
+                    asm volatile("" : "+s"(cw), "+s"(al), "+s"(bl), "+s"(bcl));
+                const uint32_t* alut_p = a.alut;
+                const uint32_t* blut_p = a.blut;
+                uint32_t off_al = (FZ ? W::off_alut : a.off_alut), off_bl = (FZ ? W::off_blut : a.off_blut);
+                if constexpr (VPL == 1 && CPL == 1 && !(Q8 && !UCN)) {
+                    typedef __attribute__((address_space(4))) const BsArgs ConstArgs;
+                    ConstArgs* ka = (ConstArgs*)__builtin_amdgcn_kernarg_segment_ptr();
+                    asm volatile("" : "+s"(ka));
+                    alut_p = ka->alut;
+                    blut_p = ka->blut;
+                    if constexpr (!FZ) {
+                        off_al = ka->off_alut;
+                        off_bl = ka->off_blut;
+                    }
                 }
-            }
-            if (!(AFX && afx))
-                copy_async(off_al + 4u * (uint32_t)(nx * al), alut_p + (size_t)(t + 1) * al, al, cw, NT);
-            if (bcl > 1)
-                copy_async(off_bl + 4u * (uint32_t)(nx * bl), blut_p + (size_t)(t + 1) * bl, bl, cw, NT);
+                if (!(AFX && afx))
+                    copy_async(off_al + 4u * (uint32_t)(nx * al), alut_p + (size_t)(t + 1) * al, al, cw, NT);
+                if (bcl > 1)
+                    copy_async(off_bl + 4u * (uint32_t)(nx * bl), blut_p + (size_t)(t + 1) * bl, bl, cw, NT);
+            }
         }
         if constexpr (BKPF) {
             if (t + 1 < a.T && a.btid) {
@@ -1128,6 +1161,8 @@
                 cbase = gbase[c];
                 asm volatile("" : "+v"(cbase));
             }
+            [[maybe_unused]] uint32_t idw = 0u;
+            if constexpr (WF) idw = lds_w(W::off_alut + 4u * (uint32_t)t);
             uint32_t ctab = PKG ? (cbase >> 16) : gtab[c];
             if constexpr (PKG) cbase &= 0xFFFFu;
             int gmc = gm[c];
@@ -1216,6 +1251,12 @@
             if (LPC == 4) par ^= qperm<QP_X2>(par);
             uint32_t q1[4], q2[4];
             PH9("ck_tab", c, m1, m2, par);
+            if constexpr (WF) {
+                const uint32_t iw = (uint32_t)__builtin_amdgcn_readfirstlane((int)idw);
+                wf_bk = (int)(iw >> 16);
+                beta_asm(q1, m1, (int)(iw & 0xFFFFu));
+                beta_asm(q2, m2, (int)(iw & 0xFFFFu));
+            } else
             if (AFX && afx) {
                 beta_asm(q1, m1, ak);
                 beta_asm(q2, m2, ak);
@@ -1455,6 +1496,7 @@
     int word;
     const int32_t* atid;
     bool frozen;
+    bool wf;
     uint32_t* ticket;
 };
 
@@ -1484,11 +1526,11 @@
     return hipGetLastError() == hipSuccess ? LDPC_OK : LDPC_ERR_HIP;
 }
 
-template <int I, bool XP, bool Q8, bool FZ = false, bool L8 = false>
+template <int I, bool XP, bool Q8, bool FZ = false, bool L8 = false, bool WF = false>
 int launch_bs_x(const BsLaunch& a, int npacks, int nw, size_t lds, hipStream_t s, int grid, int* resident) {
     constexpr BsInst k = kBsInst[I];
     static_assert(bs_loops(k) == (BS_LOOP_TU != 0), "BS_LOOP_TU lists the instances of bs_loops");
-    constexpr auto fn = &k_bs<k.D, k.DV, k.LPC, k.VPL, k.CPL, k.UCN, k.BIG, k.PK, k.WPE, XP, 1024, Q8, false, false, FZ, L8>;
+    constexpr auto fn = &k_bs<k.D, k.DV, k.LPC, k.VPL, k.CPL, k.UCN, k.BIG, k.PK, k.WPE, XP, 1024, Q8, false, false, FZ, L8, WF>;
     int nblocks = npacks;
     if constexpr (bs_loops(k)) {
         if (grid < 0) {
@@ -1545,6 +1587,9 @@
                   : launch_bs_es_x<I, false, false>(a, npacks, nw, lds, s);
     } else {
         if constexpr (I == BsFrozenWman::inst) {
+            if (a.frozen && a.wf && !a.hdx)
+                return q8 ? launch_bs_x<I, false, true, true, false, true>(a, npacks, nw, lds, s, grid, resident + 8)
+                          : launch_bs_x<I, false, false, true, false, true>(a, npacks, nw, lds, s, grid, resident + 7);
             if (a.frozen && !a.hdx)
                 return q8 ? launch_bs_x<I, false, true, true>(a, npacks, nw, lds, s, grid, resident + 4)
                           : launch_bs_x<I, false, false, true>(a, npacks, nw, lds, s, grid, resident + 3);
diff --git a/ldpc_error_floor_amd/csrc/ldpc_capi.hip b/ldpc_error_floor_amd/csrc/ldpc_capi.hip
--- a/ldpc_error_floor_amd/csrc/ldpc_capi.hip
+++ b/ldpc_error_floor_amd/csrc/ldpc_capi.hip
@@ -323,8 +323,7 @@
     if (st == LDPC_OK && alpha_ucn) st = dev_alloc(&g->d_alpha_ucn, ne);
     if (st == LDPC_OK) st = dev_alloc(&g->d_beta, nn);
     if (st == LDPC_OK) st = dev_alloc(&g->d_beta_tid, nn);
-    const bool afix = !wi.alpha_tid.empty() &&
-                      std::all_of(wi.alpha_tid.begin(), wi.alpha_tid.end(), [](int32_t k) { return k >= 0; });
+    const bool afix = host::set_weight_ids(g->h, wi);
     if (st == LDPC_OK && afix) st = dev_alloc(&g->d_alpha_tid, (size_t)T);
     if (st != LDPC_OK) return st;
     bool ok = hipMemcpy(g->d_alpha, alpha, ne * sizeof(float), hipMemcpyHostToDevice) == hipSuccess;
@@ -943,6 +942,11 @@
     return (c->fused.bs_afix && std::strncmp(c->last_kernel, "bsl[", 4) == 0) ? 1 : 0;
 }
 
+int ldpc_ctx_last_wf(const ldpc_ctx* c) {
+    if (!c) return LDPC_ERR_ARG;
+    return (c->fused.bs_wf && std::strncmp(c->last_kernel, "bsl[", 4) == 0) ? 1 : 0;
+}
+
 int ldpc_ctx_last_kernel(const ldpc_ctx* c, char* name, int32_t name_len) {
     if (!c || !name || name_len <= 0) return LDPC_ERR_ARG;
     std::strncpy(name, c->last_kernel, (size_t)name_len - 1);
diff --git a/ldpc_error_floor_amd/csrc/ldpc_fused.h b/ldpc_error_floor_amd/csrc/ldpc_fused.h
--- a/ldpc_error_floor_amd/csrc/ldpc_fused.h
+++ b/ldpc_error_floor_amd/csrc/ldpc_fused.h
@@ -18,11 +18,12 @@
     size_t bs_lut_bytes = 0;
     uint32_t* bs_bad = nullptr;
     int64_t bs_bad_n = 0;
-    int bs_resident[7] = {0, 0, 0, 0, 0, 0, 0};
+    int bs_resident[9] = {0, 0, 0, 0, 0, 0, 0, 0, 0};
     uint64_t bs_resident_key = ~0ull;
     uint32_t* bs_ticket = nullptr;
     bool bs_frozen = false;
     bool bs_afix = false;
+    bool bs_wf = false;
     uint32_t* hdx = nullptr;
     int64_t hdx_elems = 0;
     bool bits_packed = false;
diff --git a/ldpc_error_floor_amd/csrc/ldpc_host.cpp b/ldpc_error_floor_amd/csrc/ldpc_host.cpp
--- a/ldpc_error_floor_amd/csrc/ldpc_host.cpp
+++ b/ldpc_error_floor_amd/csrc/ldpc_host.cpp
@@ -157,6 +157,13 @@
                 }
     w.beta_tid.resize((size_t)T * g.N);
     for (size_t x = 0; x < (size_t)T * g.N; ++x) w.beta_tid[x] = beta_table_id(beta[x]);
+    w.wf_beta.assign((size_t)T, -1);
+    for (int t = 0; t < T; ++t) {
+        int32_t k = w.beta_tid[(size_t)t * g.N];
+        for (int j = 1; j < g.N; ++j)
+            if (w.beta_tid[(size_t)t * g.N + j] != k) k = -1;
+        w.wf_beta[(size_t)t] = (t < 64 && ((w.beta_id_mask >> t) & 1)) ? kNBetaTab : k;
+    }
     for (int t = 0; t < T; ++t) {
         const float a0 = alpha[(size_t)t * g.E], b0 = beta[(size_t)t * g.N];
         for (int e = 1; e < g.E && w.alpha_uniform; ++e)
diff --git a/ldpc_error_floor_amd/csrc/ldpc_host.h b/ldpc_error_floor_amd/csrc/ldpc_host.h
--- a/ldpc_error_floor_amd/csrc/ldpc_host.h
+++ b/ldpc_error_floor_amd/csrc/ldpc_host.h
@@ -42,6 +42,7 @@
     std::vector<int32_t> device_block;
     size_t off_vn = 0;
     const int32_t* w_alpha_tid_dev = nullptr;
+    std::vector<int32_t> w_alpha_tid, w_wf_beta;
 };
 
 int build_graph(const int32_t* proto, int32_t M, int32_t N, int32_t z, GraphTables& out);
@@ -55,11 +56,19 @@
     std::vector<int32_t> row_merge;
     std::vector<int32_t> beta_tid;
     std::vector<int32_t> alpha_tid;
+    std::vector<int32_t> wf_beta;
 };
 int beta_table_id(float beta);
 int alpha_table_id(float alpha, int mode);
 int analyze_weights(const GraphTables& g, int32_t T, const float* alpha, const float* alpha_ucn,
                     const float* beta, WeightInfo& out);
+inline bool set_weight_ids(GraphTables& g, const WeightInfo& w) {
+    bool all = !w.alpha_tid.empty();
+    for (const int32_t k : w.alpha_tid) all = all && k >= 0;
+    g.w_alpha_tid = all ? w.alpha_tid : std::vector<int32_t>();
+    g.w_wf_beta = w.wf_beta;
+    return all;
+}
 
 int check_decode(const GraphTables& g, int64_t B, int64_t B_max, int32_t T_max, int32_t T_w,
                  const ldpc_decode_params* p, int* mode);
diff --git a/ldpc_error_floor_amd/csrc/pybind_module.cpp b/ldpc_error_floor_amd/csrc/pybind_module.cpp
--- a/ldpc_error_floor_amd/csrc/pybind_module.cpp
+++ b/ldpc_error_floor_amd/csrc/pybind_module.cpp
@@ -584,6 +584,14 @@
         },
         py::arg("ctx"));
     m.def(
+        "last_wf",
+        [](Ctx& c) {
+            const int r = ldpc_ctx_last_wf(c.h);
+            check(r < 0 ? r : 0, "ldpc_ctx_last_wf");
+            return r == 1;
+        },
+        py::arg("ctx"));
+    m.def(
         "format_uncor_rows",
         [](py::array_t<float, py::array::c_style | py::array::forcecast> rows) {
             if (rows.ndim() != 2 || rows.shape(1) <= 0)
diff --git a/ldpc_error_floor_amd/decoder.py b/ldpc_error_floor_amd/decoder.py
--- a/ldpc_error_floor_amd/decoder.py
+++ b/ldpc_error_floor_amd/decoder.py
@@ -577,6 +577,9 @@
     def last_afix(self) -> bool:
         return False if self._ctx is None else bool(self._ext.last_afix(self._ctx))
 
+    def last_wf(self) -> bool:
+        return False if self._ctx is None else bool(self._ext.last_wf(self._ctx))
+
     def _empty_result(self, T, nt, hard, synd, counters, flags, app, iter_wrong=False):
         torch = self._torch
         dev = self.device
```
